# ygtxr1997/MSML

Measured on AMD Instinct MI355X. Metric: images/sec (112x112) ires50-MSML+PartialFC training step, higher is better.
Workload: dtype bf16; 1 GPU; iresnet50-MSML (OSB r18 + FM x4) + 85742-id ArcFace PartialFC, 112x112, batch 256/GPU, fwd+bwd+clip+SGD; global_batch=256, parallelism=dp1+class-parallel head, launch=eager, weight gradients + OSB on side streams

## Files before the change

include/msml_hip.h:

```cpp
#ifndef MSML_HIP_H
#define MSML_HIP_H

#include <stddef.h>
#include <stdint.h>

#ifdef __cplusplus
extern "C" {
#endif

#define MSML_ABI_VERSION 1

enum { MSML_F32 = 0, MSML_BF16 = 1, MSML_BF16X3 = 2 };

enum {
  MSML_OK = 0,
  MSML_ERR_SHAPE = -1,
  MSML_ERR_DTYPE = -2,
  MSML_ERR_LAUNCH = -3,
  MSML_ERR_UNSUPPORTED = -4,
  MSML_ERR_WORKSPACE = -5
};

enum { MSML_ACT_TANH = 0, MSML_ACT_SIGMOID = 1 };
enum { MSML_ARITH_ADD = 0, MSML_ARITH_SUB = 1, MSML_ARITH_MUL = 2, MSML_ARITH_DIV = 3 };

int msml_version(void);
const char* msml_last_error(void);
long msml_stream_capture_id(void* stream);
int msml_stream_wait_stream(void* waiter, void* src);

int msml_nchw_to_nhwc(const float* src, void* dst, int N, int C, int H, int W, int Cp,
                      int dtype, void* stream);
int msml_nhwc_to_nchw(const void* src, float* dst, int N, int C, int H, int W, int Cp,
                      int dtype, void* stream);

int msml_pack_weight(const float* w, void* dst, int A, int B, int R, int S, int transpose,
                     int C1, int C1p, int C2, int C2p, int KOp, int dtype, void* stream);

int msml_fm_fuse_fwd(const void* x, const void* yf, void* z, long n, int act, int arith,
                     int dtype, void* stream);
int msml_fm_fuse_bwd(const void* dz, const void* x, const void* yf, void* dx, void* dyf,
                     long n, int act, int arith, int dtype, void* stream);

int msml_fm_act_fwd(const void* x, void* m, long n, int act, int dtype, void* stream);
int msml_fm_act_bwd(const void* dm, const void* x, void* dx, long n, int act, int dtype, void* stream);
int msml_mul_fwd(const void* a, const void* b, void* out, long n, int dtype, void* stream);
int msml_mul_bwd(const void* g, const void* a, const void* b, void* da, void* db, long n, int dtype,
                 void* stream);
int msml_axpb(const void* x, void* y, long n, float a, float b, int dtype, void* stream);
int msml_mse_fwd(const void* a, const void* b, long n, double count, float* loss, double* workspace,
                 long ws_doubles, int dtype, void* stream);
int msml_mse_bwd(const void* a, const void* b, const float* g, double count, void* da, void* db, long n,
                 int dtype, void* stream);
int msml_dropout(const void* x, void* y, long n, float p, long seed, int dtype, void* stream);
int msml_dropout_dev(const void* x, void* y, long n, float p, const long* seed, int dtype, void* stream);

int msml_conv_tile_m(int coutp);
int msml_conv_tile_n(int coutp);
int msml_conv2d(const void* in0, int c0p, const void* in1, int c1p, const void* wp, int kop,
                const float* bias, void* out, int coutp, float* stats, int N, int H, int W,
                int P, int Q, int R, int S, int stride, int pad_h, int pad_w, int transposed,
                int in_dtype, int out_dtype, void* stream);

int msml_conv2d_acc(const void* in0, int c0p, const void* in1, int c1p, const void* wp, int kop,
                    const float* bias, void* out, int coutp, double* acc, int N, int H, int W,
                    int P, int Q, int R, int S, int stride, int pad_h, int pad_w, int transposed,
                    int in_dtype, int out_dtype, void* stream);

long msml_conv_wgrad_workspace(int up, int vp, int N, int P, int Q, int R, int S);
int msml_conv_wgrad(const void* u, int up, const void* v, int vp, float* dw, int A, int Breal,
                    int Btot, int boff, int N, int H, int W, int P, int Q, int R, int S,
                    int stride, int pad_h, int pad_w, int accumulate, void* workspace,
                    long ws_bytes, int dtype, void* stream);

int msml_conv_wgrad_group_max(int up, int vp, int A, int Breal, int N, int H, int W, int P, int Q, int R, int S,
                              int stride, int pad_h, int pad_w);
int msml_conv_wgrad_group(const void* const* u, const void* const* v, float* const* dw, int group, int up, int vp,
                          int A, int Breal, int Btot, int boff, int N, int H, int W, int P, int Q, int R, int S,
                          int stride, int pad_h, int pad_w, int accumulate, void* workspace, long ws_bytes, int dtype,
                          void* stream);

int msml_conv_wgrad_kernel_is_n32(int up, int vp, int N, int H, int W, int P, int Q, int R, int S, int stride,
                                  int pad_h, int pad_w);

int msml_bn_stats_rows(long M, int C);
int msml_bn_stats(const void* x, long M, int C, float* partial, int dtype, void* stream);
int msml_bn_finalize(const float* partial, int rows, int C, double count, const float* gamma,
                     const float* beta, float* running_mean, float* running_var, float momentum,
                     float eps, float* scale, float* shift, float* save_mean, float* save_invstd,
                     void* stream);
int msml_bn_act_fwd(const void* x, const float* scale, const float* shift, const float* alpha,
                    const void* residual, int res_first, void* y, long M, int C, int dtype,
                    void* stream);
int msml_bn_act_fwd_stats_rows(long M, int C);
int msml_bn_act_fwd_stats(const void* x, const float* scale, const float* shift, const float* alpha,
                          const void* residual, int res_first, void* y, long M, int C,
                          float* stats, int dtype, void* stream);
int msml_bn_fin_act_fwd(const double* acc, double count, const float* gamma, const float* beta,
                        float* running_mean, float* running_var, float momentum, float eps, float* scale,
                        float* shift, float* save_mean, float* save_invstd, const void* x,
                        const float* alpha, const void* residual, int res_first, void* y, long M, int C,
                        double* acc_out, int dtype, void* stream);
int msml_bn_stats_acc(const void* x, long M, int C, double* acc, int dtype, void* stream);
int msml_conv2d_bnbwd_acc(const void* in0, int c0p, const void* wp, int kop, void* out, int coutp, int N,
                          int H, int W, int P, int Q, int R, int S, int stride, int pad_h, int pad_w,
                          int transposed, const void* bn_x, const float* bn_scale, const float* bn_shift,
                          const float* bn_alpha, const float* bn_mean, const float* bn_invstd, double* acc,
                          void* stream);
int msml_bn_fin_bwd_apply(const void* dy, const void* x, const float* scale, const float* shift,
                          const float* alpha, const float* save_mean, const float* save_invstd,
                          const double* acc, const void* residual_first, const void* add, int add_h,
                          int add_w, void* dx, void* dres, float* dgamma, float* dbeta, float* dalpha,
                          int accumulate, long M, int C, const void* next_x, const float* next_mean,
                          const float* next_invstd, double* next_acc, int dtype, void* stream);
int msml_bn_act_bwd_acc(const void* dy, const void* x, const float* scale, const float* shift,
                        const float* alpha, const float* save_mean, const float* save_invstd,
                        const void* residual_first, const void* add, void* dx, void* dres, float* dgamma,
                        float* dbeta, float* dalpha, int accumulate, long M, int C, double* acc, int dtype,
                        void* stream);
int msml_bn_act_bwd(const void* dy, const void* x, const float* scale, const float* shift,
                    const float* alpha, const float* save_mean, const float* save_invstd,
                    const void* residual_first, void* dx, void* dres, float* dgamma, float* dbeta,
                    float* dalpha, int accumulate, long M, int C, float* workspace, long ws_floats,
                    int dtype, void* stream);
int msml_bias_grad(const void* dy, long M, int Cp, int Creal, float* db, int accumulate,
                   float* workspace, long ws_floats, int dtype, void* stream);
int msml_add(const void* a, const void* b, void* out, long n, int dtype, void* stream);

int msml_dap_fwd(const void* x, float* seg, unsigned char* mask, int N, int H, int W, int Cp,
                 int dtype, void* stream);
int msml_dap_bwd(const float* dseg, void* dx, int N, int H, int W, int Cp, int dtype, void* stream);
int msml_seg_consensus_loss(const float* logit, const long* msk, int N, int H, int W, float alpha,
                            float beta, float* loss, float* dlogit, float* workspace,
                            long ws_floats, void* stream);
int msml_seg_consensus_loss_r(const float* logit, const long* msk, int N, int H, int W, float alpha, float beta,
                              int reduce_pixel_all, int reduce_pixel_kl_all, float* loss, float* dlogit,
                              float* workspace, long ws_floats, void* stream);

int msml_rownorm_fwd(const float* w, int R, int Rp, int E, void* dst, int ld, float* inv_norm,
                     int dtype, void* stream);
int msml_rownorm_bwd(const float* w, const float* inv_norm, const float* dy, int ldy, int R, int E,
                     float* dw, int accumulate, void* stream);
int msml_gather_target(const float* cosm, int ld, const long* label, int N, float* out,
                       void* stream);
int msml_margin_fwd(float* cosm, const long* label, int N, int C, int ld, int kind, float s,
                    float m, float a, float k, void* stream);
int msml_margin_bwd(const float* dlogit, int ldg, const long* label, const float* cos_t, int N,
                    int C, void* dcos, int ldo, int kind, float s, float m, float a, float k,
                    int dtype, void* stream);
int msml_pfc_rowstats(const float* cosm, int ld, int N, int C, const long* label, int kind, float s,
                      float m, float a, float k, float* rowmax, float* rowsum, void* stream);
int msml_pfc_grad(const float* cosm, int ld, int N, int C, const long* label, int kind, float s,
                  float m, float a, float k, const float* gmax, const float* gsum, float eps_ls,
                  float inv_n, void* dcos, int ldo, float* ptarget, int dtype, void* stream);
int msml_sgd_momentum(float* w, const float* grad, float* mom, long n, float lr, float mu, float wd,
                      int first_step, const float* clip_coef, void* stream);
int msml_grad_norm_clip(const float* grad, long n, float max_norm, float* out2, float* workspace,
                        long ws_floats, void* stream);
int msml_sgd_momentum_dev(float* w, const float* grad, float* mom, long n, const float* lr, float mu, float wd,
                          const float* coef, void* stream);
int msml_grad_norm_clip_scaled(const float* grad, long n, float max_norm, float scale, float* out2, float* workspace,
                               long ws_floats, void* stream);

long msml_gemm_splitk_workspace(int M, int coutp, int K);
int msml_gemm_splitk(const void* a, int M, int K, const void* wp, int kop, float* out, int coutp,
                     void* workspace, long ws_bytes, int dtype, void* stream);

int msml_pack_weights_batched(const long* table, int count, int dtype, void* stream);
int msml_pack_tiles(int A, int B, int R, int S);
int msml_pack_weights_tiled(const long* table, const int* tile_prefix, int count, int total_tiles,
                            int dtype, void* stream);

int msml_transpose(const void* src, int R, int C, int ld_s, void* dst, int ld_d, int dtype,
                   void* stream);

int msml_conv2d_fused(const void* in0, int c0p, const void* in1, int c1p, const void* wp, int kop,
                      const float* scale, const float* shift, const float* alpha,
                      const void* residual, int res_first, void* out, int coutp, int N, int H,
                      int W, int P, int Q, int R, int S, int stride, int pad_h, int pad_w,
                      int transposed, void* stream);

int msml_conv2d_x3(const void* in0, int c0p, const void* in1, int c1p, const void* wp, int kop,
                   const float* scale, const float* shift, const float* alpha, const void* residual,
                   int res_first, void* out, int coutp, int N, int H, int W, int P, int Q, int R, int S,
                   int stride, int pad_h, int pad_w, int transposed, void* stream);
int msml_conv2d_x3_border(const void* in0, int c0p, const void* wp, int kop, const float* scale,
                          const float* shift9, const float* alpha, const void* residual, int res_first,
                          void* out, int coutp, int N, int H, int W, void* stream);
int msml_x3_bn_act_fwd(const void* x, const float* scale, const float* shift, const float* alpha,
                       const void* residual, int res_first, void* y, long M, int C, void* stream);
int msml_x3_fm_fuse_fwd(const void* x, const void* yf, void* z, long M, int C, int act, int arith,
                        void* stream);
int msml_x3_add(const void* a, const void* b, void* out, long M, int C, void* stream);
int msml_x3_from_f32(const float* src, void* dst, long M, int C, void* stream);
int msml_x3_to_f32(const void* src, float* dst, long M, int C, void* stream);

int msml_pair_sqdist(const float* emb, int n_pairs, int E, double* dist, void* stream);
int msml_pair_sqdist_f64(const double* emb, int n_pairs, int E, double* dist, void* stream);
int msml_pair_hist(const double* dist, const unsigned char* same, int n_pairs, const double* thr, int nthr,
                   int nfolds, int* hist, void* stream);

int msml_occ_draw(long seed, long offset, int N, int H, int W, int mode, int lo, int hi, int flip, int* desc,
                  void* stream);
int msml_occ_apply(const unsigned char* src, const int* desc, float* img, long* msk, float* ori, int N, int H,
                   int W, int light, void* stream);

int msml_occ_draw_tex(long seed, long offset, int N, int H, int W, int mode, int lo, int hi, int flip,
                      const int* meta, int nsets, int* desc, void* stream);
int msml_occ_resize(const unsigned char* atlas, const int* meta, const int* dir, const int* rtab, const int* desc,
                    unsigned char* patch, long patch_stride, int N, int lds_bytes, void* stream);
int msml_occ_apply_tex(const unsigned char* src, const int* desc, const unsigned char* patch, long patch_stride,
                       float* img, long* msk, float* ori, int N, int H, int W, int light, void* stream);

int msml_occ_draw_out(long seed, long offset, int N, int H, int W, int out_h, int out_w, int mode, int lo, int hi,
                      int flip, const int* meta, int nsets, int* desc, void* stream);
int msml_occ_apply_out(const unsigned char* src, const int* desc, const unsigned char* patch, long patch_stride,
                       const int* tabw, const int* tabh, float* img, long* msk, float* ori, int N, int H, int W,
                       int out_h, int out_w, int gray, int norm, int light, void* stream);

int msml_deconv4_bwd_data(const void* dy, const void* wp0, const void* wp1, void* dx0, void* dx1, int N, int H,
                          void* stream);

int msml_conv2d_bnbwd_rows(int coutp, int N, int P, int Q);
int msml_conv2d_bnbwd(const void* in0, int c0p, const void* wp, int kop, void* out, int coutp,
                      int N, int H, int W, int P, int Q, int R, int S, int stride, int pad_h,
                      int pad_w, int transposed, const void* bn_x, const float* bn_scale,
                      const float* bn_shift, const float* bn_alpha, const float* bn_mean,
                      const float* bn_invstd, float* partial, int rows_cap, int* rows_used,
                      void* stream);
int msml_bn_act_bwd_apply(const void* dy, const void* x, const float* scale, const float* shift,
                          const float* alpha, const float* save_mean, const float* save_invstd,
                          const float* partial, int rows, const void* add, void* dx,
                          float* dgamma, float* dbeta, float* dalpha, int accumulate, long M,
                          int C, float* coef_ws, int dtype, void* stream);

int msml_bn_act_bwd_apply_s2(const void* dy, const void* x, const float* scale, const float* shift,
                             const float* alpha, const float* save_mean, const float* save_invstd,
                             const float* partial, int rows, const void* add, int H, int W, void* dx,
                             float* dgamma, float* dbeta, float* dalpha, int accumulate, long M,
                             int C, float* coef_ws, int dtype, void* stream);
int msml_bn_act_bwd_apply_next_s2(const void* dy, const void* x, const float* scale,
                                  const float* shift, const float* alpha, const float* save_mean,
                                  const float* save_invstd, const float* partial, int rows,
                                  const void* add, int H, int W, void* dx, float* dgamma, float* dbeta,
                                  float* dalpha, int accumulate, long M, int C, float* coef_ws,
                                  const void* next_x, const float* next_mean,
                                  const float* next_invstd, float* next_partial, int dtype,
                                  void* stream);

int msml_conv2d_bnin_applies(int c0p, int coutp, int N, int H, int W, int P, int Q, int R, int S,
                             int stride, int pad_h, int pad_w, int want_stats);
int msml_conv2d_bnin(const void* in0, int c0p, const float* in_scale, const float* in_shift,
                     const float* in_alpha, const void* wp, int kop, void* out, int coutp,
                     float* stats, int N, int H, int W, int P, int Q, int R, int S, int stride,
                     int pad_h, int pad_w, void* stream);
int msml_conv_wgrad_bnin_applies(int up, int vp, int A, int Breal, int N, int H, int W, int P, int Q,
                                 int R, int S, int stride, int pad_h, int pad_w);
int msml_conv_wgrad_bnin(const void* u, int up, const void* v, int vp, const float* x_scale,
                         const float* x_shift, const float* x_alpha, float* dw, int A, int Breal,
                         int Btot, int boff, int N, int H, int W, int P, int Q, int R, int S,
                         int stride, int pad_h, int pad_w, int accumulate, void* workspace,
                         long ws_bytes, void* stream);

#define MSML_KERNEL_MFM 2
const char* msml_conv2d_kernel(int c0p, int c1p, int coutp, int N, int H, int W, int P, int Q,
                               int R, int S, int stride, int pad_h, int pad_w, int transposed,
                               int in_dtype, int out_dtype, int want_stats);

int msml_stem_im2col(const float* x, void* out, int N, int C, int H, int W, int P, int Q, int R,
                     int S, int stride, int pad, int KP, int dtype, void* stream);

int msml_bn_act_bwd_apply_rows(long M, int C);
int msml_bn_act_bwd_apply_next(const void* dy, const void* x, const float* scale, const float* shift,
                               const float* alpha, const float* save_mean, const float* save_invstd,
                               const float* partial, int rows, const void* add, void* dx,
                               float* dgamma, float* dbeta, float* dalpha, int accumulate, long M,
                               int C, float* coef_ws, const void* next_x, const float* next_mean,
                               const float* next_invstd, float* next_partial, int dtype, void* stream);

int msml_conv2d_bnin_acc_applies(int c0p, int coutp, int N, int H, int W, int P, int Q, int R, int S, int stride,
                                 int pad_h, int pad_w);
int msml_conv2d_bnin_acc(const void* in0, int c0p, const double* acc_in, double count, const float* gamma,
                         const float* beta, float* running_mean, float* running_var, float momentum, float eps,
                         float* coef_out, const float* in_alpha, void* act_out, const void* wp, int kop, void* out,
                         int coutp, double* acc_out, int N, int H, int W, int P, int Q, int R, int S, int stride,
                         int pad_h, int pad_w, void* stream);

int msml_iblock_fwd_tables(int* nptr, int* nint, int* nflt);
int msml_iblock_fwd(const void* const* ptrs, const int* ints, const float* flts, void* stream);

int msml_probe_mfma(const void* seed, float* out, int wgs, int iters, void* stream);
int msml_probe_mfma_lds(const void* seed, float* out, int wgs, int iters, void* stream);


int msml_conv2d_mfm(const void* in0, int c0p, const void* wp, int kop, const float* bias, void* out, int coutp,
                    const void* residual, unsigned char* sel, int N, int H, int W, int P, int Q, int R, int S,
                    int stride, int pad_h, int pad_w, int dtype, void* stream);

int msml_mfm_bwd(const void* dy, const unsigned char* sel, void* dz, long M, int cp, int C, int czp, int dtype,
                 void* stream);

int msml_pool2_fwd(const void* x, void* y, int N, int H, int W, int cp, int dtype, void* stream);

int msml_pool2_bwd(const void* dy, const void* x, void* dx, int N, int H, int W, int cp, int dtype, void* stream);

int msml_template_pool(const float* feats, long n_rows, long ld, int E, int flip, const float* faceness,
                       const int* order, const int* media_start, const int* tmpl_media_start, const int* launch,
                       int n_templates, double* out, void* stream);
int msml_template_pair_score(const double* tn, int n_templates, int E, const int* r1, const int* r2, long n_pairs,
                             double* score, void* stream);
int msml_roc_blocks(int n);
int msml_roc_block_counts(const double* sorted, const unsigned char* label, int n, int* blk, void* stream);
int msml_roc_points(const double* sorted, const unsigned char* label, int n, const int* off, int* tps, int* fps,
                    void* stream);
int msml_roc_reduce_blocks(int n_points);
int msml_roc_reduce(const int* tps, const int* fps, int n_points, const double* target, int n_targets,
                    unsigned char* keep, unsigned long long* part, void* stream);
int msml_pair_cosdist(const float* emb, int n_pairs, int E, double* dist, void* stream);
int msml_pair_cosdist_f64(const double* emb, int n_pairs, int E, double* dist, void* stream);
int msml_rank_count(const double* sorted, int n, const double* q, int m, int strict, int* out, void* stream);

#ifdef __cplusplus
}
#endif
#endif
```

msml_amd/blocks.py:

```python
import os

import torch

from . import ops
from . import _lib
from ._lib import BF16, call
from .ops import cpad


TAP = None
FAULT = os.environ.get("MSML_FAULT", "")


def _bn_pack(bn):
    return (bn.weight, bn.bias, bn.running_mean, bn.running_var, 0.1 if bn.momentum is None else bn.momentum,
            bn.eps, bn)


def _bn_coef(x, stats, bnp):
    assert not _is_acc(stats), "accumulator-mode statistics go through _bn_fin_apply"
    c = x.shape[-1]
    m = x.numel() // c
    coef = torch.empty(4, c, dtype=torch.float32, device=x.device)
    if stats is None:
        rows = ops.bn_stats_rows(m, c)
        stats = torch.empty(rows, 2, c, dtype=torch.float32, device=x.device)
        with ops.PROFILE.rec("bn_stats", 0.0, x.numel() * x.element_size()):
            call("msml_bn_stats", x, m, c, stats, BF16)
    k = ops.rows4(coef)
    call("msml_bn_finalize", stats, stats.shape[0], c, float(m), bnp[0], bnp[1], bnp[2], bnp[3], bnp[4], bnp[5],
         k[0], k[1], k[2], k[3])
    ops.bn_counter(bnp[6])
    return coef


def _bn_apply(x, coef, alpha, residual, emit_stats=False, res_first=0):
    c = x.shape[-1]
    m = x.numel() // c
    y = torch.empty_like(x)
    coef = ops.rows4(coef)
    with ops.PROFILE.rec("bn_act_fwd", 0.0, x.numel() * x.element_size() * (3 if residual is not None else 2)):
        if emit_stats:
            ystats = torch.empty(_lib.value("msml_bn_act_fwd_stats_rows", m, c), 2, c, dtype=torch.float32,
                                 device=x.device)
            call("msml_bn_act_fwd_stats", x, coef[0], coef[1], alpha, residual, 0, y, m, c, ystats, BF16)
            return y, ystats
        call("msml_bn_act_fwd", x, coef[0], coef[1], alpha, residual, res_first, y, m, c, BF16)
    return y


def _bn_fin_apply(x, acc, bnp, alpha, residual, emit_stats=False, res_first=0):
    c = x.shape[-1]
    m = x.numel() // c
    coef = torch.empty(4, c, dtype=torch.float32, device=x.device)
    y = torch.empty_like(x)
    yacc = ops.stats_acc(c, x.device) if emit_stats else None
    k = ops.rows4(coef)
    with ops.PROFILE.rec("bn_act_fwd", 0.0, x.numel() * x.element_size() * (3 if residual is not None else 2)):
        call("msml_bn_fin_act_fwd", acc, float(m), bnp[0], bnp[1], bnp[2], bnp[3], bnp[4], bnp[5], k[0], k[1],
             k[2], k[3], x, alpha, residual, res_first, y, m, c, yacc, BF16)
    ops.bn_counter(bnp[6])
    if emit_stats:
        return y, coef, yacc
    return y, coef


def _is_acc(stats):
    return stats is not None and stats.dtype == torch.float64


def _own_stats(x, stats):
    c = x.shape[-1]
    if stats is None and ops.acc_applies(c, BF16):
        stats = ops.stats_acc(c, x.device)
        with ops.PROFILE.rec("bn_stats", 0.0, x.numel() * x.element_size()):
            call("msml_bn_stats_acc", x, x.numel() // c, c, stats, BF16)
    return stats


def _bn_fwd(x, stats, bnp, alpha, residual, emit_stats=False):
    stats = _own_stats(x, stats)
    if _is_acc(stats):
        return _bn_fin_apply(x, stats, bnp, alpha, residual, emit_stats)
    coef = _bn_coef(x, stats, bnp)
    if emit_stats:
        y, ystats = _bn_apply(x, coef, alpha, residual, True)
        return y, coef, ystats
    return _bn_apply(x, coef, alpha, residual), coef


def _conv_pack(cm):
    w = cm.weight
    return (w, tuple(w.shape), cm.stride[0], cm.padding[0], cm.padding[1])


def _conv_fwd(x, cp):
    w, (cout, cin, r, s), stride, ph, pw = cp
    wp = ops.PACKS.get(w, False, 0, cout, 0, cin, cin, 0, BF16)
    return ops.conv2d(x, None, wp, None, cpad(cout), r, s, stride, ph, pw, False, want_stats=True,
                      real=(cin, cout))


def _bn_conv_fwd(x, stats, bnp, alpha, cp):
    if not (ops.FUSE_BN_IN and stats is None):
        stats = _own_stats(x, stats)
    if _is_acc(stats):
        w, (cout, cin, r, s), stride, ph, pw = cp
        n, h, wd, cp_in = x.shape
        if ph == pw and ops.bnin_acc_applies(n, h, wd, cp_in, cpad(cout), r, s, stride, ph):
            wp = ops.PACKS.get(w, False, 0, cout, 0, cin, cin, 0, BF16)
            o, coef, y, st = ops.conv2d_bnin_acc(x, stats, bnp, alpha, wp, cpad(cout), real=(cin, cout))
            ops.bn_counter(bnp[6])
            return o, coef, y, st
        o, coef = _bn_fin_apply(x, stats, bnp, alpha, None)
        y, st = _conv_fwd(o, cp)
        return o, coef, y, st
    coef = _bn_coef(x, stats, bnp)
    w, (cout, cin, r, s), stride, ph, pw = cp
    n, h, wd, cp_in = x.shape
    if r == 3 and s == 3 and stride == 1 and ph == 1 and pw == 1 and \
            ops.bnin_applies(n, h, wd, cp_in, cpad(cout), cout, cin):
        wp = ops.PACKS.get(w, False, 0, cout, 0, cin, cin, 0, BF16)
        y, st = ops.conv2d_bnin(x, coef, alpha, wp, cpad(cout), real=(cin, cout))
        return None, coef, y, st
    o = _bn_apply(x, coef, alpha, None)
    y, st = _conv_fwd(o, cp)
    return o, coef, y, st


def _wgrad(dy, x, cp, xin=None):
    wparam, (cout, cin, r, s), stride, ph, pw = cp
    inplace = ops.inplace(wparam)
    dw = wparam.grad.view(wparam.shape) if inplace else torch.empty_like(wparam)
    side = ops.WGRAD_STREAM if inplace else None
    if side is not None:
        _lib.stream_wait_current(side)
        dy.record_stream(side)
        x.record_stream(side)
        if xin is not None:
            xin[0].record_stream(side)
    if xin is not None:
        ops.conv_wgrad_bnin(dy, x, xin[0], xin[1], dw, cout, cin, cin, 0, accumulate=inplace, stream=side)
    elif inplace and r == 3 and s == 3 and stride == 1 and ph == 1 and pw == 1:
        ops.conv_wgrad_queued(dy, x, dw, cout, cin, cin, 0, side, wparam)
        return None
    else:
        ops.conv_wgrad(dy, x, dw, cout, cin, cin, 0, r, s, stride, ph, pw, accumulate=inplace, stream=side)
    if inplace:
        ops.grad_ready(wparam)
        return None
    return dw


def _dgrad(dy, cp, h, w, bn_x=None, coef=None, alpha=None):
    wparam, (cout, cin, r, s), stride, ph, pw = cp
    wp = ops.PACKS.get(wparam, True, 0, cout, 0, cin, cout, 0, BF16)
    if bn_x is not None and ops.FUSE_BN_BWD:
        got = ops.conv_dgrad_bnbwd(dy, wp, cpad(cin), r, s, stride, ph, pw, h, w, bn_x, coef, alpha,
                                   real=(cout, cin))
        if got is not None:
            return got
    dx, _ = ops.conv2d(dy, None, wp, None, cpad(cin), r, s, stride, ph, pw, True, p=h, q=w, real=(cout, cin))
    return dx, None


def _dgrad_plus(dy, cp, h, w, other):
    wparam, (cout, cin, r, s), stride, ph, pw = cp
    cinp = cpad(cin)
    if stride != 1 or other.shape[-1] != cinp:
        dx, _ = _dgrad(dy, cp, h, w)
        call("msml_add", dx, other, dx, dx.numel(), BF16)
        return dx
    wp = ops.PACKS.get(wparam, True, 0, cout, 0, cin, cout, 0, BF16)
    unit = ops.unit_coef(cinp, dy.device)
    n, p, q, c0p = dy.shape
    out = torch.empty(n, h, w, cinp, dtype=torch.bfloat16, device=dy.device)
    name = "conv_igemm"
    if ops.PROFILE.on:
        name = ops.conv_label("T+add", c0p, 0, cinp, n, p, q, h, w, r, s, stride, ph, pw, 1, BF16, BF16, False)
    with ops.PROFILE.rec(name, 2.0 * n * p * q * cout * cin * r * s):
        call("msml_conv2d_fused", dy, c0p, None, 0, wp, wp.shape[0], unit[0], unit[1], None, other, 0, out, cinp,
             n, p, q, h, w, r, s, stride, ph, pw, 1)
    return out


def _dgrad_1x1_compact(dy, cp):
    wparam, (cout, cin, _, _), _, _, _ = cp
    wp = ops.PACKS.get(wparam, True, 0, cout, 0, cin, cout, 0, BF16)
    dxc, _ = ops.conv2d(dy, None, wp, None, cpad(cin), 1, 1, 1, 0, 0, True, p=dy.shape[1], q=dy.shape[2],
                        real=(cout, cin))
    return dxc


class _ParamGrads:

    def __init__(self, params, c, dev):
        self.params = params
        self.want = [p is not None and p.requires_grad for p in params]
        self.inplace = all((not w) or ops.inplace(p) for w, p in zip(self.want, params))
        if self.inplace:
            self.tg = [p.grad if w else None for w, p in zip(self.want, params)]
        else:
            pg = torch.empty(3, c, dtype=torch.float32, device=dev)
            self.tg = [pg[i] if p is not None else None for i, p in enumerate(params)]

    def done(self):
        if self.inplace:
            ops.grad_ready(*[p for w, p in zip(self.want, self.params) if w])

    def out(self, i):
        return self.tg[i] if (self.want[i] and not self.inplace) else None


def _bn_bwd(dy, x, coef, alpha, pgr, partial=None, add=None, nxt=None, add_s2=False):
    c = x.shape[-1]
    m = x.numel() // c
    dx = torch.empty_like(x)
    coef = ops.rows4(coef)
    if nxt:
        nxt = (nxt[0], ops.rows4(nxt[1])) + tuple(nxt[2:])
    s2 = (add, x.shape[1], x.shape[2]) if add_s2 else (add,)
    sfx = "_s2" if add_s2 else ""
    if partial is None and ops.acc_applies(c, BF16):
        assert not add_s2, "a compact stride-2 `add` needs the producer-side sums (docstring)"
        with ops.PROFILE.rec("bn_act_bwd", 0.0, x.numel() * x.element_size() * 5):
            call("msml_bn_act_bwd_acc", dy, x, coef[0], coef[1], alpha, coef[2], coef[3], None, add, dx, None,
                 pgr.tg[0], pgr.tg[1], pgr.tg[2], int(pgr.inplace), m, c, ops.stats_acc(c, x.device, 3), BF16)
    elif partial is None:
        rows = ops.bn_stats_rows(m, c)
        ws = ops.workspace((rows * 3 * c + 2 * c) * 4, x.device)
        with ops.PROFILE.rec("bn_act_bwd", 0.0, x.numel() * x.element_size() * 5):
            call("msml_bn_act_bwd", dy, x, coef[0], coef[1], alpha, coef[2], coef[3], None, dx, None,
                 pgr.tg[0], pgr.tg[1], pgr.tg[2], int(pgr.inplace), m, c, ws, ws.numel() // 4, BF16)
        if add is not None:
            call("msml_add", dx, add, dx, dx.numel(), BF16)
    elif partial.dtype == torch.float64:
        ah, aw = (x.shape[1], x.shape[2]) if add_s2 else (0, 0)
        if nxt is not None and 256 % (c // 8) == 0:
            nacc = ops.stats_acc(c, x.device, 3)
            with ops.PROFILE.rec("bn_act_bwd_apply", 0.0, x.numel() * x.element_size() * (5 if add is not None else 4)):
                call("msml_bn_fin_bwd_apply", dy, x, coef[0], coef[1], alpha, coef[2], coef[3], partial, None, add, ah, aw,
                     dx, None, pgr.tg[0], pgr.tg[1], pgr.tg[2], int(pgr.inplace), m, c, nxt[0], nxt[1][2], nxt[1][3],
                     nacc, BF16)
            pgr.done()
            return dx, nacc
        with ops.PROFILE.rec("bn_act_bwd_apply", 0.0, x.numel() * x.element_size() * (4 if add is not None else 3)):
            call("msml_bn_fin_bwd_apply", dy, x, coef[0], coef[1], alpha, coef[2], coef[3], partial, None, add, ah, aw,
                 dx, None, pgr.tg[0], pgr.tg[1], pgr.tg[2], int(pgr.inplace), m, c, None, None, None, None, BF16)
    else:
        cw = torch.empty(98 * c, dtype=torch.float32, device=x.device)
        if nxt is not None and 256 % (c // 8) == 0:
            npart = torch.empty(_lib.value("msml_bn_act_bwd_apply_rows", m, c), 3, c, dtype=torch.float32,
                                device=x.device)
            with ops.PROFILE.rec("bn_act_bwd_apply", 0.0, x.numel() * x.element_size() * (5 if add is not None else 4)):
                call("msml_bn_act_bwd_apply_next" + sfx, dy, x, coef[0], coef[1], alpha, coef[2], coef[3], partial,
                     partial.shape[0], *s2, dx, pgr.tg[0], pgr.tg[1], pgr.tg[2], int(pgr.inplace), m, c, cw,
                     nxt[0], nxt[1][2], nxt[1][3], npart, BF16)
            pgr.done()
            return dx, npart
        with ops.PROFILE.rec("bn_act_bwd_apply", 0.0, x.numel() * x.element_size() * (4 if add is not None else 3)):
            call("msml_bn_act_bwd_apply" + sfx, dy, x, coef[0], coef[1], alpha, coef[2], coef[3], partial,
                 partial.shape[0], *s2, dx, pgr.tg[0], pgr.tg[1], pgr.tg[2], int(pgr.inplace), m, c, cw, BF16)
    pgr.done()
    if nxt is not None:
        return dx, None
    return dx


def _block_pack(blk):
    ds = blk.downsample
    return {
        "bn1": _bn_pack(blk.bn1), "bn2": _bn_pack(blk.bn2), "bn3": _bn_pack(blk.bn3),
        "c1": _conv_pack(blk.conv1), "c2": _conv_pack(blk.conv2), "alpha": blk.prelu.weight,
        "ds": None if ds is None else (_conv_pack(ds[0]), _bn_pack(ds[1])),
        "emit_stats": bool(getattr(blk, "emit_stats", False)),
    }


(_IB_X, _IB_XACC, _IB_BN1_G, _IB_BN1_B, _IB_BN1_RM, _IB_BN1_RV, _IB_COEF1, _IB_O1, _IB_WP1, _IB_C1, _IB_ACC1,
 _IB_BN2_G, _IB_BN2_B, _IB_BN2_RM, _IB_BN2_RV, _IB_COEF2, _IB_ALPHA, _IB_O2, _IB_WP2, _IB_C2, _IB_ACC2,
 _IB_WPD, _IB_D, _IB_ACCD, _IB_BND_G, _IB_BND_B, _IB_BND_RM, _IB_BND_RV, _IB_COEFD, _IB_IDN,
 _IB_BN3_G, _IB_BN3_B, _IB_BN3_RM, _IB_BN3_RV, _IB_COEF3, _IB_OUT, _IB_ACC_OUT, _IB_NPTR) = range(38)
(_II_N, _II_H, _II_W, _II_CINP, _II_COUTP, _II_KOP1, _II_KOP2, _II_KOPD, _II_STRIDE, _II_P, _II_Q, _II_HAS_DS,
 _II_DS_STRIDE, _II_NINT) = range(14)
_IF_NFLT = 8
_TABLES_OK = []


def _tables_checked():
    if not _TABLES_OK:
        import ctypes
        a, b, c = ctypes.c_int(), ctypes.c_int(), ctypes.c_int()
        call("msml_iblock_fwd_tables", ctypes.byref(a), ctypes.byref(b), ctypes.byref(c))
        if (a.value, b.value, c.value) != (_IB_NPTR, _II_NINT, _IF_NFLT):
            raise RuntimeError("msml_iblock_fwd: table layout of the library (%d, %d, %d) differs from blocks.py"
                               % (a.value, b.value, c.value))
        _TABLES_OK.append(True)
    return True


def _iblock_fwd_applies(x, bp):
    if not (ops.BLOCK_C_ENTRY and ops.ACC_STATS and not ops.PROFILE.on and not ops.FUSE_BN_IN and x.dtype == torch.bfloat16):
        return False
    cout = cpad(bp["c1"][1][0])
    return ops.acc_applies(x.shape[-1], BF16) and ops.acc_applies(cout, BF16) and x.shape[-1] == bp["c1"][1][1]


def _iblock_fwd_fast(x, bp, xstats):
    import ctypes
    _tables_checked()
    tab = bp.get("_fwd_tab")
    if tab is None:
        tab = bp["_fwd_tab"] = ((ctypes.c_void_p * _IB_NPTR)(), (ctypes.c_int * _II_NINT)(), (ctypes.c_float * _IF_NFLT)())
    pt, it, ft = tab
    dev = x.device
    n, h, w, cinp = x.shape
    bn1, bn2, bn3, ds = bp["bn1"], bp["bn2"], bp["bn3"], bp["ds"]
    w1, (cout, cin, _, _), _, _, _ = bp["c1"]
    w2, _, stride, _, _ = bp["c2"]
    coutp = cpad(cout)
    p_, q_ = ops.conv_out_size(h, 3, stride, 1, False), ops.conv_out_size(w, 3, stride, 1, False)
    if xstats is None:
        xstats = _own_stats(x, None)
    bf = torch.bfloat16
    o1 = torch.empty_like(x)
    c1 = torch.empty(n, h, w, coutp, dtype=bf, device=dev)
    o2 = torch.empty_like(c1)
    c2 = torch.empty(n, p_, q_, coutp, dtype=bf, device=dev)
    out = torch.empty_like(c2)
    k1 = torch.empty(4, cinp, dtype=torch.float32, device=dev)
    k2 = torch.empty(4, coutp, dtype=torch.float32, device=dev)
    k3 = torch.empty(4, coutp, dtype=torch.float32, device=dev)
    acc1, acc2 = ops.stats_acc(coutp, dev), ops.stats_acc(coutp, dev)
    wp1 = ops.PACKS.get(w1, False, 0, cout, 0, cin, cin, 0, BF16)
    wp2 = ops.PACKS.get(w2, False, 0, cout, 0, cout, cout, 0, BF16)
    emit = bp["emit_stats"] and 256 % (coutp // 8) == 0
    ostats = ops.stats_acc(coutp, dev) if emit else None
    pt[_IB_X], pt[_IB_XACC] = x.data_ptr(), xstats.data_ptr()
    pt[_IB_BN1_G], pt[_IB_BN1_B], pt[_IB_BN1_RM], pt[_IB_BN1_RV] = (bn1[0].data_ptr(), bn1[1].data_ptr(),
                                                                    bn1[2].data_ptr(), bn1[3].data_ptr())
    pt[_IB_COEF1], pt[_IB_O1], pt[_IB_WP1], pt[_IB_C1], pt[_IB_ACC1] = (k1.data_ptr(), o1.data_ptr(), wp1.data_ptr(),
                                                                       c1.data_ptr(), acc1.data_ptr())
    pt[_IB_BN2_G], pt[_IB_BN2_B], pt[_IB_BN2_RM], pt[_IB_BN2_RV] = (bn2[0].data_ptr(), bn2[1].data_ptr(),
                                                                    bn2[2].data_ptr(), bn2[3].data_ptr())
    pt[_IB_COEF2], pt[_IB_ALPHA], pt[_IB_O2], pt[_IB_WP2], pt[_IB_C2], pt[_IB_ACC2] = (
        k2.data_ptr(), bp["alpha"].data_ptr(), o2.data_ptr(), wp2.data_ptr(), c2.data_ptr(), acc2.data_ptr())
    d = kd = None
    it[_II_HAS_DS] = 0
    if ds is not None:
        wd, (_, _, dr, dsz), dstride, dph, dpw = ds[0]
        if dr != 1 or dsz != 1 or dph != 0 or dpw != 0:
            return None
        dbn = ds[1]
        d = torch.empty_like(c2)
        idn = torch.empty_like(c2)
        kd = torch.empty(4, coutp, dtype=torch.float32, device=dev)
        accd = ops.stats_acc(coutp, dev)
        wpd = ops.PACKS.get(wd, False, 0, cout, 0, cin, cin, 0, BF16)
        pt[_IB_WPD], pt[_IB_D], pt[_IB_ACCD] = wpd.data_ptr(), d.data_ptr(), accd.data_ptr()
        pt[_IB_BND_G], pt[_IB_BND_B], pt[_IB_BND_RM], pt[_IB_BND_RV] = (dbn[0].data_ptr(), dbn[1].data_ptr(),
                                                                        dbn[2].data_ptr(), dbn[3].data_ptr())
        pt[_IB_COEFD], pt[_IB_IDN] = kd.data_ptr(), idn.data_ptr()
        it[_II_HAS_DS], it[_II_KOPD], it[_II_DS_STRIDE] = 1, wpd.shape[0], dstride
        ft[6], ft[7] = dbn[4], dbn[5]
    pt[_IB_BN3_G], pt[_IB_BN3_B], pt[_IB_BN3_RM], pt[_IB_BN3_RV] = (bn3[0].data_ptr(), bn3[1].data_ptr(),
                                                                    bn3[2].data_ptr(), bn3[3].data_ptr())
    pt[_IB_COEF3], pt[_IB_OUT] = k3.data_ptr(), out.data_ptr()
    pt[_IB_ACC_OUT] = ostats.data_ptr() if emit else None
    (it[_II_N], it[_II_H], it[_II_W], it[_II_CINP], it[_II_COUTP], it[_II_KOP1], it[_II_KOP2], it[_II_STRIDE], it[_II_P],
     it[_II_Q]) = n, h, w, cinp, coutp, wp1.shape[0], wp2.shape[0], stride, p_, q_
    ft[0], ft[1], ft[2], ft[3], ft[4], ft[5] = bn1[4], bn1[5], bn2[4], bn2[5], bn3[4], bn3[5]
    call("msml_iblock_fwd", pt, it, ft)
    for b in ((bn1, bn2, bn3) if ds is None else (bn1, bn2, ds[1], bn3)):
        ops.bn_counter(b[6])
    return o1, c1, o2, c2, d, k1, k2, k3, kd, out, ostats


class _IBlock(torch.autograd.Function):
    @staticmethod
    def forward(ctx, x, bp, xstats, pc2, pk3, *params):
        if _iblock_fwd_applies(x, bp):
            fast = _iblock_fwd_fast(x, bp, xstats)
            if fast is not None:
                o1, c1, o2, c2, d, k1, k2, k3, kd, out, ostats = fast
                if ostats is None:
                    ostats = out.new_empty(0)
                ctx.bp = bp
                ctx.set_materialize_grads(False)
                bp["_last_bn3"] = (c2, k3) if bp["emit_stats"] else None
                ctx.save_for_backward(x, o1, c1, o2, c2, d, k1, k2, k3, kd, pc2, pk3)
                ctx.mark_non_differentiable(ostats)
                return out, ostats
        ds = bp["ds"]
        o1, k1, c1, st1 = _bn_conv_fwd(x, xstats, bp["bn1"], None, bp["c1"])
        o2, k2, c2, st2 = _bn_conv_fwd(c1, st1, bp["bn2"], bp["alpha"], bp["c2"])
        if ds is not None:
            d, std = _conv_fwd(x, ds[0])
            idn, kd = _bn_fwd(d, std, ds[1], None, None)
        else:
            d, kd, idn = None, None, x
        if bp["emit_stats"] and 256 % (c2.shape[-1] // 8) == 0:
            out, k3, ostats = _bn_fwd(c2, st2, bp["bn3"], None, idn, emit_stats=True)
        else:
            out, k3 = _bn_fwd(c2, st2, bp["bn3"], None, idn)
            ostats = out.new_empty(0)
        ctx.bp = bp
        ctx.set_materialize_grads(False)
        bp["_last_bn3"] = (c2, k3) if bp["emit_stats"] else None
        ctx.save_for_backward(x, o1, c1, o2, c2, d, k1, k2, k3, kd, pc2, pk3)
        ctx.mark_non_differentiable(ostats)
        return out, ostats

    @staticmethod
    def backward(ctx, dout, _dstats):
        x, o1, c1, o2, c2, d, k1, k2, k3, kd, pc2, pk3 = ctx.saved_tensors
        bp = ctx.bp
        ds = bp["ds"]
        dev = x.device
        dout = dout.contiguous()
        n, h, w, _ = x.shape
        bn1, bn2, bn3, alpha = bp["bn1"], bp["bn2"], bp["bn3"], bp["alpha"]
        g3 = _ParamGrads((bn3[0], bn3[1], None), c2.shape[-1], dev)
        part3 = dout.__dict__.pop("_msml_bn3_partial", None) if bp["emit_stats"] else None
        if part3 is not None:
            ops.COUNTERS["bn3_partial_hits"] += 1
        dc2 = _bn_bwd(dout, c2, k3, None, g3, part3)
        dw2 = _wgrad(dc2, o2, bp["c2"]) if o2 is not None else _wgrad(dc2, c1, bp["c2"], (k2, alpha))
        do2, part2 = _dgrad(dc2, bp["c2"], c1.shape[1], c1.shape[2], c1, k2, alpha)
        g2 = _ParamGrads((bn2[0], bn2[1], alpha), c1.shape[-1], dev)
        dc1 = _bn_bwd(do2, c1, k2, alpha, g2, part2)
        dw1 = _wgrad(dc1, o1, bp["c1"]) if o1 is not None else _wgrad(dc1, x, bp["c1"], (k1, None))
        do1, part1 = _dgrad(dc1, bp["c1"], h, w, x, k1, None)
        dwd, gd = None, None
        if ds is not None:
            gd = _ParamGrads((ds[1][0], ds[1][1], None), d.shape[-1], dev)
            dd = _bn_bwd(dout, d, kd, None, gd)
            dwd = _wgrad(dd, x, ds[0])
            (_, (_, _, dr, dsz), dstride, dph, dpw) = ds[0]
            join_s2 = (ops.SPARSE_DOWNSAMPLE_GRAD and part1 is not None and dr == 1 and dsz == 1 and dstride == 2
                       and dph == 0 and dpw == 0 and n * h * w < (1 << 24))
            if join_s2:
                join = _dgrad_1x1_compact(dd, ds[0])
            else:
                join, _ = _dgrad(dd, ds[0], h, w)
        else:
            join, join_s2 = (None if FAULT == "skip_join" else dout), False
        g1 = _ParamGrads((bn1[0], bn1[1], None), x.shape[-1], dev)
        if pc2 is not None and part1 is not None and ops.FUSE_BN_BWD:
            dx, pprev = _bn_bwd(do1, x, k1, None, g1, part1, add=join, nxt=(pc2, pk3), add_s2=join_s2)
            if pprev is not None:
                dx._msml_bn3_partial = pprev
        else:
            dx = _bn_bwd(do1, x, k1, None, g1, part1, add=join, add_s2=join_s2)
        if TAP is not None:
            TAP("iblock", bp, {"x": x, "dout": dout, "dx": dx, "k1": k1, "k2": k2, "k3": k3, "kd": kd})
        grads = [dw1, dw2] + ([dwd] if ds is not None else [])
        grads += [g1.out(0), g1.out(1), g2.out(0), g2.out(1), g2.out(2), g3.out(0), g3.out(1)]
        if ds is not None:
            grads += [gd.out(0), gd.out(1)]
        return (dx, None, None, None, None) + tuple(grads)


def iblock(blk, x):
    bp = blk.__dict__.get("_msml_pack")
    if bp is None or bp["bn1"][2] is not blk.bn1._buffers["running_mean"]:
        bp = _block_pack(blk)
        ds = blk.downsample
        params = [blk.conv1.weight, blk.conv2.weight] + ([ds[0].weight] if ds is not None else [])
        params += [blk.bn1.weight, blk.bn1.bias, blk.bn2.weight, blk.bn2.bias, blk.prelu.weight,
                   blk.bn3.weight, blk.bn3.bias]
        if ds is not None:
            params += [ds[1].weight, ds[1].bias]
        bp["params"] = tuple(params)
        blk.__dict__["_msml_pack"] = bp
    xd = x.__dict__ if hasattr(x, "__dict__") else {}
    xstats, prev = xd.get("_msml_stats"), xd.get("_msml_bn3")
    out, ostats = _IBlock.apply(x, bp, xstats, prev[0] if prev else None, prev[1] if prev else None, *bp["params"])
    last = bp.pop("_last_bn3", None)
    if ostats.numel():
        out._msml_stats = ostats
        out._msml_bn3 = last
    return out


def _bottle_pack(blk):
    return {
        "bn1": _bn_pack(blk.bn1), "bn2": _bn_pack(blk.bn2), "bn3": _bn_pack(blk.bn3),
        "c1": _conv_pack(blk.conv1), "c2": _conv_pack(blk.conv2), "c3": _conv_pack(blk.conv3),
        "a1": blk.prelu1.weight, "a2": blk.prelu2.weight, "a3": blk.prelu3.weight,
    }


class _Bottle(torch.autograd.Function):
    @staticmethod
    def forward(ctx, x, bp, *params):
        c1, st1 = _conv_fwd(x, bp["c1"])
        o1, k1 = _bn_fwd(c1, st1, bp["bn1"], bp["a1"], None)
        c2, st2 = _conv_fwd(o1, bp["c2"])
        o2, k2 = _bn_fwd(c2, st2, bp["bn2"], bp["a2"], None)
        c3, st3 = _conv_fwd(o2, bp["c3"])
        if _is_acc(st3):
            out, k3 = _bn_fin_apply(c3, st3, bp["bn3"], bp["a3"], x, res_first=1)
        else:
            k3 = _bn_coef(c3, st3, bp["bn3"])
            out = _bn_apply(c3, k3, bp["a3"], x, res_first=1)
        ctx.bp = bp
        ctx.set_materialize_grads(False)
        ctx.save_for_backward(x, c1, o1, c2, o2, c3, k1, k2, k3)
        return out

    @staticmethod
    def backward(ctx, dout):
        x, c1, o1, c2, o2, c3, k1, k2, k3 = ctx.saved_tensors
        bp = ctx.bp
        dev = x.device
        dout = dout.contiguous()
        n, h, w, _ = x.shape
        bn1, bn2, bn3 = bp["bn1"], bp["bn2"], bp["bn3"]
        g3 = _ParamGrads((bn3[0], bn3[1], bp["a3"]), c3.shape[-1], dev)
        c = c3.shape[-1]
        m = c3.numel() // c
        dc3, dres = torch.empty_like(c3), torch.empty_like(x)
        r3 = ops.rows4(k3)
        with ops.PROFILE.rec("bn_act_bwd", 0.0, c3.numel() * c3.element_size() * 7):
            if ops.acc_applies(c, BF16):
                call("msml_bn_act_bwd_acc", dout, c3, r3[0], r3[1], bp["a3"], r3[2], r3[3], x, None, dc3, dres,
                     g3.tg[0], g3.tg[1], g3.tg[2], int(g3.inplace), m, c, ops.stats_acc(c, dev, 3), BF16)
            else:
                rows = ops.bn_stats_rows(m, c)
                ws = ops.workspace((rows * 3 * c + 2 * c) * 4, dev)
                call("msml_bn_act_bwd", dout, c3, r3[0], r3[1], bp["a3"], r3[2], r3[3], x, dc3, dres,
                     g3.tg[0], g3.tg[1], g3.tg[2], int(g3.inplace), m, c, ws, ws.numel() // 4, BF16)
        g3.done()
        dw3 = _wgrad(dc3, o2, bp["c3"])
        do2, part2 = _dgrad(dc3, bp["c3"], h, w, c2, k2, bp["a2"])
        g2 = _ParamGrads((bn2[0], bn2[1], bp["a2"]), c2.shape[-1], dev)
        dc2 = _bn_bwd(do2, c2, k2, bp["a2"], g2, part2)
        dw2 = _wgrad(dc2, o1, bp["c2"])
        do1, part1 = _dgrad(dc2, bp["c2"], h, w, c1, k1, bp["a1"])
        g1 = _ParamGrads((bn1[0], bn1[1], bp["a1"]), c1.shape[-1], dev)
        dc1 = _bn_bwd(do1, c1, k1, bp["a1"], g1, part1)
        dw1 = _wgrad(dc1, x, bp["c1"])
        dx = _dgrad_plus(dc1, bp["c1"], h, w, dres)
        if TAP is not None:
            TAP("bottle", bp, {"x": x, "dout": dout, "dx": dx, "k1": k1, "k2": k2, "k3": k3})
        return (dx, None, dw1, dw2, dw3, g1.out(0), g1.out(1), g1.out(2), g2.out(0), g2.out(1), g2.out(2),
                g3.out(0), g3.out(1), g3.out(2))


def bottleneck(blk, x):
    bp = blk.__dict__.get("_msml_pack")
    if bp is None or bp["bn1"][2] is not blk.bn1._buffers["running_mean"]:
        bp = _bottle_pack(blk)
        bp["params"] = (blk.conv1.weight, blk.conv2.weight, blk.conv3.weight,
                        blk.bn1.weight, blk.bn1.bias, blk.prelu1.weight,
                        blk.bn2.weight, blk.bn2.bias, blk.prelu2.weight,
                        blk.bn3.weight, blk.bn3.bias, blk.prelu3.weight)
        blk.__dict__["_msml_pack"] = bp
    return _Bottle.apply(x, bp, *bp["params"])
```

msml_amd/csrc/bn.hip:

```cpp
#include <stdlib.h>

#include "common.h"

#define RED_ROWS_MAX 1024

template <int NQ, bool PIPE, typename L, typename F>
__device__ __forceinline__ void slab_reduce(long M, int C, float* __restrict__ partial, L ld, F f, int acc_mode = 0) {
  extern __shared__ __attribute__((aligned(16))) char smem_raw[];
  float* red = reinterpret_cast<float*>(smem_raw);
  const int C8 = C / 8;
  const int PY = 256 / C8 > 0 ? 256 / C8 : 1;
  MSML_LDS_REGION(red, PY * NQ * C * 4);
  const int t = threadIdx.x;
  const int cx = t % C8, py = t / C8;
  float q[NQ][8];
#pragma unroll
  for (int a = 0; a < NQ; a++)
#pragma unroll
    for (int j = 0; j < 8; j++) q[a][j] = 0.f;
  const long per = (M + gridDim.x - 1) / gridDim.x;
  const long beg = blockIdx.x * per;
  long end = beg + per;
  if (end > M) end = M;
  if (py < PY) {
    long pix = beg + py;
    if (PIPE)
    for (; pix + 3 * PY < end; pix += 4 * PY) {
      auto d0 = ld(pix, cx), d1 = ld(pix + PY, cx), d2 = ld(pix + 2 * PY, cx), d3 = ld(pix + 3 * PY, cx);
      f(d0, q);
      f(d1, q);
      f(d2, q);
      f(d3, q);
    }
    for (; pix < end; pix += PY) f(ld(pix, cx), q);
  }
  if (py < PY) {
#pragma unroll
    for (int a = 0; a < NQ; a++)
#pragma unroll
      for (int j = 0; j < 8; j++) red[(py * NQ + a) * C + cx * 8 + j] = q[a][j];
  }
  __syncthreads();
  for (int i = t; i < NQ * C; i += blockDim.x) {
    float s = 0.f;
    for (int y = 0; y < PY; y++) s += red[y * NQ * C + i];
    if (acc_mode)
      unsafeAtomicAdd(reinterpret_cast<double*>(partial) + (long)(blockIdx.x & (MSML_ACC_ROWS - 1)) * NQ * C + i, (double)s);
    else
      partial[(long)blockIdx.x * NQ * C + i] = s;
  }
}

static inline int red_rows(long M, int C) {
  int py = 256 / (C / 8) > 0 ? 256 / (C / 8) : 1;
  static const long ppt = getenv("MSML_RED_PPT") ? atol(getenv("MSML_RED_PPT")) : 16;
  long rows = (M + (long)py * ppt - 1) / ((long)py * ppt);
  if (rows < 1) rows = 1;
  if (rows > RED_ROWS_MAX) rows = RED_ROWS_MAX;
  return (int)rows;
}
static inline size_t red_lds(int NQ, int C) {
  int py = 256 / (C / 8) > 0 ? 256 / (C / 8) : 1;
  return (size_t)py * NQ * C * sizeof(float);
}

#define RED_PIPE_MAX_ROWS 512
template <typename T, bool PIPE>
__global__ void __launch_bounds__(256) k_bn_stats(const T* __restrict__ x, long M, int C,
                                                  float* __restrict__ partial, int acc_mode) {
  slab_reduce<2, PIPE>(M, C, partial, [&](long pix, int c8) { return load8<T>(x + pix * C + c8 * 8); },
                 [&](const Vec8& v, float(&q)[2][8]) {
#pragma unroll
    for (int j = 0; j < 8; j++) {
      q[0][j] += v.v[j];
      q[1][j] += v.v[j] * v.v[j];
    }
  }, acc_mode);
}

extern "C" int msml_bn_stats_rows(long M, int C) { return red_rows(M, C); }

extern "C" int msml_bn_stats(const void* x, long M, int C, float* partial, int dtype, void* stream) {
  MSML_CHECK(x && partial && M > 0 && C > 0 && C % 8 == 0 && C <= 2048, MSML_ERR_SHAPE,
             "bn_stats: bad shape M=%ld C=%d", M, C);
  int rows = red_rows(M, C);
  MSML_DISPATCH_DTYPE(dtype, "bn_stats",
                      if (rows <= RED_PIPE_MAX_ROWS)
                        (k_bn_stats<DT, true>)<<<rows, 256, red_lds(2, C), (hipStream_t)stream>>>((const DT*)x, M, C, partial, msml_tl_stats_acc);
                      else
                        (k_bn_stats<DT, false>)<<<rows, 256, red_lds(2, C), (hipStream_t)stream>>>((const DT*)x, M, C, partial, msml_tl_stats_acc);)
  MSML_LAUNCH_OK("bn_stats");
  return MSML_OK;
}

extern "C" int msml_bn_stats_acc(const void* x, long M, int C, double* acc, int dtype, void* stream) {
  MSML_CHECK(acc, MSML_ERR_SHAPE, "bn_stats_acc: null accumulator");
  msml_tl_stats_acc = 1;
  const int rc = msml_bn_stats(x, M, C, reinterpret_cast<float*>(acc), dtype, stream);
  msml_tl_stats_acc = 0;
  return rc;
}

#define FIN_CPB 8
#define FIN_LANES (1024 / FIN_CPB)
template <int NQ>
__device__ __forceinline__ void fin_reduce(const float* __restrict__ partial, int rows, int C, int c,
                                           bool cok, double (&out)[NQ]) {
  __shared__ double red[FIN_LANES][NQ][FIN_CPB + 1];
  __shared__ double red2[16][NQ][FIN_CPB + 1];
  const int cx = threadIdx.x & (FIN_CPB - 1), ry = threadIdx.x / FIN_CPB;
  double acc[NQ];
#pragma unroll
  for (int q = 0; q < NQ; q++) acc[q] = 0.0;
  if (cok) {
    double a1[NQ], a2[NQ], a3[NQ];
#pragma unroll
    for (int q = 0; q < NQ; q++) a1[q] = a2[q] = a3[q] = 0.0;
    int r = ry;
    for (; r + 3 * FIN_LANES < rows; r += 4 * FIN_LANES)
#pragma unroll
      for (int q = 0; q < NQ; q++) {
        acc[q] += (double)partial[((long)r * NQ + q) * C + c];
        a1[q] += (double)partial[((long)(r + FIN_LANES) * NQ + q) * C + c];
        a2[q] += (double)partial[((long)(r + 2 * FIN_LANES) * NQ + q) * C + c];
        a3[q] += (double)partial[((long)(r + 3 * FIN_LANES) * NQ + q) * C + c];
      }
    for (; r < rows; r += FIN_LANES)
#pragma unroll
      for (int q = 0; q < NQ; q++) acc[q] += (double)partial[((long)r * NQ + q) * C + c];
#pragma unroll
    for (int q = 0; q < NQ; q++) acc[q] = (acc[q] + a1[q]) + (a2[q] + a3[q]);
  }
#pragma unroll
  for (int q = 0; q < NQ; q++) red[ry][q][cx] = acc[q];
  __syncthreads();
  if (ry < 16) {
#pragma unroll
    for (int q = 0; q < NQ; q++) {
      double s = 0.0;
#pragma unroll
      for (int y = 0; y < FIN_LANES / 16; y++) s += red[ry * (FIN_LANES / 16) + y][q][cx];
      red2[ry][q][cx] = s;
    }
  }
  __syncthreads();
#pragma unroll
  for (int q = 0; q < NQ; q++) {
    double s = 0.0;
    if (ry == 0)
#pragma unroll
      for (int y = 0; y < 16; y++) s += red2[y][q][cx];
    out[q] = s;
  }
}

__global__ void __launch_bounds__(1024) k_bn_finalize(const float* __restrict__ partial, int rows, int C, double count,
                              const float* __restrict__ gamma, const float* __restrict__ beta,
                              float* __restrict__ rmean, float* __restrict__ rvar, float momentum,
                              float eps, float* __restrict__ scale, float* __restrict__ shift,
                              float* __restrict__ save_mean, float* __restrict__ save_invstd) {
  const int c = blockIdx.x * FIN_CPB + (threadIdx.x & (FIN_CPB - 1));
  const bool cok = c < C;
  float mean = 0.f, invstd = 1.f;
  if (rows > 0) {
    double s[2];
    fin_reduce<2>(partial, rows, C, c, cok, s);
    if (threadIdx.x >= FIN_CPB || !cok) return;
    double m = s[0] / count;
    double var = s[1] / count - m * m;
    if (var < 0.0) var = 0.0;
    mean = (float)m;
    invstd = (float)(1.0 / sqrt(var + (double)eps));
    if (rmean) {
      double unbiased = count > 1.0 ? var * count / (count - 1.0) : var;
      rmean[c] = (1.f - momentum) * rmean[c] + momentum * mean;
      rvar[c] = (1.f - momentum) * rvar[c] + momentum * (float)unbiased;
    }
  } else {
    if (threadIdx.x >= FIN_CPB || !cok) return;
    mean = rmean[c];
    invstd = 1.0f / sqrtf(rvar[c] + eps);
  }
  float g = gamma ? gamma[c] : 1.f, b = beta ? beta[c] : 0.f;
  scale[c] = g * invstd;
  shift[c] = b - mean * g * invstd;
  if (save_mean) {
    save_mean[c] = mean;
    save_invstd[c] = invstd;
  }
}

extern "C" int msml_bn_finalize(const float* partial, int rows, int C, double count,
                                const float* gamma, const float* beta, float* running_mean,
                                float* running_var, float momentum, float eps, float* scale,
                                float* shift, float* save_mean, float* save_invstd, void* stream) {
  MSML_CHECK(C > 0 && scale && shift && rows >= 0, MSML_ERR_SHAPE, "bn_finalize: bad args");
  MSML_CHECK(rows > 0 ? (partial && count > 0) : (running_mean && running_var), MSML_ERR_SHAPE,
             "bn_finalize: train needs partials, eval needs running stats");
  k_bn_finalize<<<cdiv(C, FIN_CPB), 1024, 0, (hipStream_t)stream>>>(
      partial, rows, C, count, gamma, beta, running_mean, running_var, momentum, eps, scale, shift,
      save_mean, save_invstd);
  MSML_LAUNCH_OK("bn_finalize");
  return MSML_OK;
}

struct Coef8 {
  float v[8];
};
__device__ __forceinline__ Coef8 ldc8(const float* p, int c0, float dflt) {
  Coef8 r;
  if (p) {
    f32x4 a = *reinterpret_cast<const f32x4*>(p + c0);
    f32x4 b = *reinterpret_cast<const f32x4*>(p + c0 + 4);
#pragma unroll
    for (int i = 0; i < 4; i++) { r.v[i] = a[i]; r.v[4 + i] = b[i]; }
  } else {
#pragma unroll
    for (int i = 0; i < 8; i++) r.v[i] = dflt;
  }
  return r;
}

template <typename T, bool STATS>
__global__ void __launch_bounds__(256) k_bn_act_fwd(const T* __restrict__ x, const float* __restrict__ scale,
                                                    const float* __restrict__ shift,
                                                    const float* __restrict__ alpha,
                                                    const T* __restrict__ residual, int res_first,
                                                    T* __restrict__ y, long n8, int C8, float* __restrict__ stats) {
  const long tid = blockIdx.x * (long)blockDim.x + threadIdx.x;
  const int c0 = (int)(tid % C8) * 8;
  const Coef8 sc = ldc8(scale, c0, 1.f), sh = ldc8(shift, c0, 0.f), al = ldc8(alpha, c0, 1.f);
  float q1[8], q2[8];
#pragma unroll
  for (int j = 0; j < 8; j++) q1[j] = q2[j] = 0.f;
  for (long i = tid; i < n8; i += (long)gridDim.x * blockDim.x) {
    Vec8 v = load8<T>(x + i * 8);
    Vec8 r;
    if (residual) r = load8<T>(residual + i * 8);
#pragma unroll
    for (int j = 0; j < 8; j++) {
      float z = v.v[j] * sc.v[j] + sh.v[j];
      if (residual && res_first) z += r.v[j];
      if (alpha) z = z > 0.f ? z : z * al.v[j];
      if (residual && !res_first) z += r.v[j];
      v.v[j] = z;
    }
    store8<T>(y + i * 8, v);
    if (STATS) {
      const Vec8 vr = round8<T>(v);
#pragma unroll
      for (int j = 0; j < 8; j++) {
        q1[j] += vr.v[j];
        q2[j] += vr.v[j] * vr.v[j];
      }
    }
  }
  if (STATS) {
    __shared__ float red[2][256][9];
    const int t = threadIdx.x, C = C8 * 8;
#pragma unroll
    for (int j = 0; j < 8; j++) {
      red[0][t][j] = q1[j];
      red[1][t][j] = q2[j];
    }
    __syncthreads();
    for (int i = t; i < 2 * C; i += 256) {
      const int which = i / C, c = i % C, cx = c >> 3, j = c & 7;
      float sum = 0.f;
      for (int k = cx; k < 256; k += C8) sum += red[which][k][j];
      stats[((long)blockIdx.x * 2 + which) * C + c] = sum;
    }
  }
}

static inline int ew_grid(long n8) {
  static const long cap = getenv("MSML_EW_GRID") ? atol(getenv("MSML_EW_GRID")) : 768;
  long b = (n8 + 255) / 256;
  return (int)(b < cap ? b : cap);
}
static inline int ew_grid_c(long n8, int C8) {
  int g = ew_grid(n8);
  if (C8 > 256) {
    int m = C8 / 256;
    g = (g + m - 1) / m * m;
  }
  return g;
}

extern "C" int msml_bn_act_fwd(const void* x, const float* scale, const float* shift,
                               const float* alpha, const void* residual, int res_first, void* y,
                               long M, int C, int dtype, void* stream) {
  MSML_CHECK(x && y && scale && shift && M > 0 && C > 0 && C % 8 == 0, MSML_ERR_SHAPE,
             "bn_act_fwd: bad shape M=%ld C=%d", M, C);
  MSML_CHECK(256 % (C / 8) == 0 || (C / 8) % 256 == 0, MSML_ERR_UNSUPPORTED,
             "bn_act_fwd: C/8 = %d must divide 256 or be a multiple of it", C / 8);
  long n8 = M * (C / 8);
  MSML_DISPATCH_DTYPE(dtype, "bn_act_fwd",
                      (k_bn_act_fwd<DT, false>)<<<ew_grid_c(n8, C / 8), 256, 0, (hipStream_t)stream>>>(
                          (const DT*)x, scale, shift, alpha, (const DT*)residual, res_first, (DT*)y, n8,
                          C / 8, nullptr);)
  MSML_LAUNCH_OK("bn_act_fwd");
  return MSML_OK;
}

extern "C" int msml_bn_act_fwd_stats_rows(long M, int C) { return ew_grid_c(M * (C / 8), C / 8); }

extern "C" int msml_bn_act_fwd_stats(const void* x, const float* scale, const float* shift, const float* alpha,
                                     const void* residual, int res_first, void* y, long M, int C,
                                     float* stats, int dtype, void* stream) {
  MSML_CHECK(x && y && scale && shift && stats && M > 0 && C > 0 && C % 8 == 0, MSML_ERR_SHAPE,
             "bn_act_fwd_stats: bad shape M=%ld C=%d", M, C);
  MSML_CHECK(256 % (C / 8) == 0, MSML_ERR_UNSUPPORTED, "bn_act_fwd_stats: C/8 = %d must divide 256", C / 8);
  long n8 = M * (C / 8);
  MSML_DISPATCH_DTYPE(dtype, "bn_act_fwd_stats",
                      (k_bn_act_fwd<DT, true>)<<<ew_grid_c(n8, C / 8), 256, 0, (hipStream_t)stream>>>(
                          (const DT*)x, scale, shift, alpha, (const DT*)residual, res_first, (DT*)y, n8,
                          C / 8, stats);)
  MSML_LAUNCH_OK("bn_act_fwd_stats");
  return MSML_OK;
}

template <typename T, bool STATS>
__global__ void __launch_bounds__(256) k_bn_fin_act_fwd(const double* __restrict__ acc, double count,
                                                        const float* __restrict__ gamma, const float* __restrict__ beta,
                                                        float* __restrict__ rmean, float* __restrict__ rvar, float momentum,
                                                        float eps, float* __restrict__ scale, float* __restrict__ shift,
                                                        float* __restrict__ save_mean, float* __restrict__ save_invstd,
                                                        const T* __restrict__ x, const float* __restrict__ alpha,
                                                        const T* __restrict__ residual, int res_first,
                                                        T* __restrict__ y, long n8, int C8, double* __restrict__ acc_out) {
  extern __shared__ float cs[];
  const int C = C8 * 8, t = threadIdx.x;
  MSML_LDS_REGION(cs, 2 * C * 4);
  for (int c = t; c < C; c += 256) {
    double s = 0.0, ss = 0.0;
#pragma unroll
    for (int r = 0; r < MSML_ACC_ROWS; r++) {
      s += acc[(r * 2 + 0) * C + c];
      ss += acc[(r * 2 + 1) * C + c];
    }
    const double m = s / count;
    double var = ss / count - m * m;
    if (var < 0.0) var = 0.0;
    const float mean = (float)m;
    const float invstd = (float)(1.0 / sqrt(var + (double)eps));
    const float g = gamma ? gamma[c] : 1.f, b = beta ? beta[c] : 0.f;
    const float sc = g * invstd, sh = b - mean * g * invstd;
    cs[c] = sc;
    cs[C + c] = sh;
    if (blockIdx.x == 0) {
      scale[c] = sc;
      shift[c] = sh;
      save_mean[c] = mean;
      save_invstd[c] = invstd;
      if (rmean) {
        const double unbiased = count > 1.0 ? var * count / (count - 1.0) : var;
        rmean[c] = (1.f - momentum) * rmean[c] + momentum * mean;
        rvar[c] = (1.f - momentum) * rvar[c] + momentum * (float)unbiased;
      }
    }
  }
  __syncthreads();
  const long tid = blockIdx.x * (long)blockDim.x + t;
  const int c0 = (int)(tid % C8) * 8;
  Coef8 sc, sh;
#pragma unroll
  for (int j = 0; j < 8; j++) {
    sc.v[j] = cs[c0 + j];
    sh.v[j] = cs[C + c0 + j];
  }
  const Coef8 al = ldc8(alpha, c0, 1.f);
  float q1[8], q2[8];
#pragma unroll
  for (int j = 0; j < 8; j++) q1[j] = q2[j] = 0.f;
  for (long i = tid; i < n8; i += (long)gridDim.x * blockDim.x) {
    Vec8 v = load8<T>(x + i * 8);
    Vec8 r;
    if (residual) r = load8<T>(residual + i * 8);
#pragma unroll
    for (int j = 0; j < 8; j++) {
      float z = v.v[j] * sc.v[j] + sh.v[j];
      if (residual && res_first) z += r.v[j];
      if (alpha) z = z > 0.f ? z : z * al.v[j];
      if (residual && !res_first) z += r.v[j];
      v.v[j] = z;
    }
    store8<T>(y + i * 8, v);
    if (STATS) {
      const Vec8 vr = round8<T>(v);
#pragma unroll
      for (int j = 0; j < 8; j++) {
        q1[j] += vr.v[j];
        q2[j] += vr.v[j] * vr.v[j];
      }
    }
  }
  if (STATS) {
    __shared__ float red[2][256][9];
#pragma unroll
    for (int j = 0; j < 8; j++) {
      red[0][t][j] = q1[j];
      red[1][t][j] = q2[j];
    }
    __syncthreads();
    for (int i = t; i < 2 * C; i += 256) {
      const int which = i / C, c = i % C, cx = c >> 3, j = c & 7;
      float sum = 0.f;
      for (int k = cx; k < 256; k += C8) sum += red[which][k][j];
      stats_emit(reinterpret_cast<float*>(acc_out), 1, blockIdx.x, which, C, c, sum);
    }
  }
}

extern "C" int msml_bn_fin_act_fwd(const double* acc, double count, const float* gamma, const float* beta,
                                   float* running_mean, float* running_var, float momentum, float eps, float* scale,
                                   float* shift, float* save_mean, float* save_invstd, const void* x,
                                   const float* alpha, const void* residual, int res_first, void* y, long M, int C,
                                   double* acc_out, int dtype, void* stream) {
  MSML_CHECK(acc && x && y && scale && shift && save_mean && save_invstd && M > 0 && C > 0 && C % 8 == 0 && count > 0,
             MSML_ERR_SHAPE, "bn_fin_act_fwd: bad arguments M=%ld C=%d", M, C);
  MSML_CHECK(256 % (C / 8) == 0, MSML_ERR_UNSUPPORTED, "bn_fin_act_fwd: C/8 = %d must divide 256", C / 8);
  const long n8 = M * (C / 8);
  const size_t lds = (size_t)2 * C * sizeof(float);
  hipStream_t st = (hipStream_t)stream;
  if (acc_out) {
    MSML_DISPATCH_DTYPE(dtype, "bn_fin_act_fwd",
                        (k_bn_fin_act_fwd<DT, true>)<<<ew_grid_c(n8, C / 8), 256, lds, st>>>(
                            acc, count, gamma, beta, running_mean, running_var, momentum, eps, scale, shift, save_mean,
                            save_invstd, (const DT*)x, alpha, (const DT*)residual, res_first, (DT*)y, n8, C / 8, acc_out);)
  } else {
    MSML_DISPATCH_DTYPE(dtype, "bn_fin_act_fwd",
                        (k_bn_fin_act_fwd<DT, false>)<<<ew_grid_c(n8, C / 8), 256, lds, st>>>(
                            acc, count, gamma, beta, running_mean, running_var, momentum, eps, scale, shift, save_mean,
                            save_invstd, (const DT*)x, alpha, (const DT*)residual, res_first, (DT*)y, n8, C / 8, nullptr);)
  }
  MSML_LAUNCH_OK("bn_fin_act_fwd");
  return MSML_OK;
}

template <typename T, bool PIPE>
__global__ void __launch_bounds__(256) k_bn_bwd_reduce(const T* __restrict__ dy, const T* __restrict__ x,
                                                       const float* __restrict__ scale,
                                                       const float* __restrict__ shift,
                                                       const float* __restrict__ alpha,
                                                       const float* __restrict__ mean,
                                                       const float* __restrict__ invstd,
                                                       const T* __restrict__ res, long M, int C,
                                                       float* __restrict__ partial, int acc_mode) {
  const int c0h = (threadIdx.x % (C / 8)) * 8;
  const Coef8 sc = ldc8(scale, c0h, 1.f), sh = ldc8(shift, c0h, 0.f), al = ldc8(alpha, c0h, 1.f);
  const Coef8 mu = ldc8(mean, c0h, 0.f), is = ldc8(invstd, c0h, 1.f);
  struct Px {
    Vec8 g, v, rr;
  };
  slab_reduce<3, PIPE>(M, C, partial, [&](long pix, int c8) {
    Px d;
    d.g = load8<T>(dy + pix * C + c8 * 8);
    d.v = load8<T>(x + pix * C + c8 * 8);
    if (res) d.rr = load8<T>(res + pix * C + c8 * 8);
    return d;
  }, [&](const Px& d, float(&q)[3][8]) {
    const Vec8 &g = d.g, &v = d.v, &rr = d.rr;
#pragma unroll
    for (int j = 0; j < 8; j++) {
      float gg = g.v[j];
      if (alpha) {
        float z = v.v[j] * sc.v[j] + sh.v[j];
        if (res) z += rr.v[j];
        if (z <= 0.f) {
          q[2][j] += gg * z;
          gg *= al.v[j];
        }
      }
      float xh = (v.v[j] - mu.v[j]) * is.v[j];
      q[0][j] += gg;
      q[1][j] += gg * xh;
    }
  }, acc_mode);
}

#define FOLD_ROWS 32
#define FOLD_MIN_ROWS 512
template <int NQ>
__global__ void __launch_bounds__(1024) k_fold_rows(const float* __restrict__ partial, int rows, int C,
                                                    float* __restrict__ out) {
  const int c = blockIdx.x * FIN_CPB + (threadIdx.x & (FIN_CPB - 1));
  const bool cok = c < C;
  const int chunk = (rows + FOLD_ROWS - 1) / FOLD_ROWS;
  const int r0 = blockIdx.y * chunk;
  int nr = rows - r0;
  if (nr > chunk) nr = chunk;
  if (nr < 0) nr = 0;
  double s[NQ];
  fin_reduce<NQ>(partial + (long)r0 * NQ * C, nr, C, c, cok, s);
  if (threadIdx.x >= FIN_CPB || !cok) return;
#pragma unroll
  for (int q = 0; q < NQ; q++) out[((long)blockIdx.y * NQ + q) * C + c] = (float)s[q];
}

__global__ void __launch_bounds__(1024) k_bn_bwd_finalize(const float* __restrict__ partial, int rows, int C, double count,
                                  float* __restrict__ dgamma, float* __restrict__ dbeta,
                                  float* __restrict__ dalpha, float* __restrict__ coef, int accumulate) {
  const int c = blockIdx.x * FIN_CPB + (threadIdx.x & (FIN_CPB - 1));
  const bool cok = c < C;
  double s[3];
  fin_reduce<3>(partial, rows, C, c, cok, s);
  if (threadIdx.x >= FIN_CPB || !cok) return;
  if (dbeta) dbeta[c] = (accumulate ? dbeta[c] : 0.f) + (float)s[0];
  if (dgamma) dgamma[c] = (accumulate ? dgamma[c] : 0.f) + (float)s[1];
  if (dalpha) dalpha[c] = (accumulate ? dalpha[c] : 0.f) + (float)s[2];
  coef[c] = (float)(s[0] / count);
  coef[C + c] = (float)(s[1] / count);
}

template <typename T, bool NEXT, bool ADD_S2 = false>
__global__ void __launch_bounds__(256) k_bn_bwd_apply(const T* __restrict__ dy, const T* __restrict__ x,
                                                      const float* __restrict__ scale,
                                                      const float* __restrict__ shift,
                                                      const float* __restrict__ alpha,
                                                      const float* __restrict__ mean,
                                                      const float* __restrict__ invstd,
                                                      const float* __restrict__ coef,
                                                      const T* __restrict__ res, const T* __restrict__ add,
                                                      T* __restrict__ dx, T* __restrict__ dres, long n8,
                                                      int C8, const T* __restrict__ nx,
                                                      const float* __restrict__ nmean,
                                                      const float* __restrict__ ninvstd,
                                                      float* __restrict__ npartial, int aH, int aW) {
  const int C = C8 * 8;
  const long tid = blockIdx.x * (long)blockDim.x + threadIdx.x;
  const int c0 = (int)(tid % C8) * 8;
  const Coef8 sc = ldc8(scale, c0, 1.f), sh = ldc8(shift, c0, 0.f), al = ldc8(alpha, c0, 1.f);
  const Coef8 mu = ldc8(mean, c0, 0.f), is = ldc8(invstd, c0, 1.f);
  const Coef8 k1 = ldc8(coef, c0, 0.f), k2 = ldc8(coef + C, c0, 0.f);
  const float rcpW = ADD_S2 ? 1.0f / (float)aW : 0.f, rcpH = ADD_S2 ? 1.0f / (float)aH : 0.f;
  const int aPw = (aW + 1) >> 1, aPh = (aH + 1) >> 1;
  const Coef8 nmu = ldc8(NEXT ? nmean : nullptr, c0, 0.f), nis = ldc8(NEXT ? ninvstd : nullptr, c0, 1.f);
  float nq0[8], nq1[8];
#pragma unroll
  for (int j = 0; j < 8; j++) nq0[j] = nq1[j] = 0.f;
  for (long i = tid; i < n8; i += (long)gridDim.x * blockDim.x) {
    Vec8 g = load8<T>(dy + i * 8);
    Vec8 v = load8<T>(x + i * 8);
    Vec8 rr, ad;
    if (res) rr = load8<T>(res + i * 8);
    bool has_add = add != nullptr;
    if (ADD_S2) {
      const int pix = (int)(i / C8);
      int row = (int)((float)pix * rcpW), xx = pix - row * aW;
      if (xx < 0) { row--; xx += aW; } else if (xx >= aW) { row++; xx -= aW; }
      int nn = (int)((float)row * rcpH), yy = row - nn * aH;
      if (yy < 0) { nn--; yy += aH; } else if (yy >= aH) { nn++; yy -= aH; }
      has_add = !((xx | yy) & 1);
      if (has_add) ad = load8<T>(add + (((long)nn * aPh + (yy >> 1)) * aPw + (xx >> 1)) * C + c0);
    } else if (add) {
      ad = load8<T>(add + i * 8);
    }
#pragma unroll
    for (int j = 0; j < 8; j++) {
      float gg = g.v[j];
      if (alpha) {
        float z = v.v[j] * sc.v[j] + sh.v[j];
        if (res) z += rr.v[j];
        if (z <= 0.f) gg *= al.v[j];
      }
      float xh = (v.v[j] - mu.v[j]) * is.v[j];
      v.v[j] = sc.v[j] * (gg - k1.v[j] - xh * k2.v[j]);
      if (has_add) v.v[j] += ad.v[j];
      g.v[j] = gg;
    }
    store8<T>(dx + i * 8, v);
    if (dres) store8<T>(dres + i * 8, g);
    if (NEXT) {
      const Vec8 o = round8<T>(v), xn = load8<T>(nx + i * 8);
#pragma unroll
      for (int j = 0; j < 8; j++) {
        nq0[j] += o.v[j];
        nq1[j] += o.v[j] * ((xn.v[j] - nmu.v[j]) * nis.v[j]);
      }
    }
  }
  if (NEXT) {
    __shared__ float red[2][256][9];
    const int t = threadIdx.x;
#pragma unroll
    for (int j = 0; j < 8; j++) {
      red[0][t][j] = nq0[j];
      red[1][t][j] = nq1[j];
    }
    __syncthreads();
    for (int i = t; i < 3 * C; i += 256) {
      const int q = i / C, c = i % C, cx = c >> 3, j = c & 7;
      float sum = 0.f;
      if (q < 2)
        for (int k = cx; k < 256; k += C8) sum += red[q][k][j];
      npartial[((long)blockIdx.x * 3 + q) * C + c] = sum;
    }
  }
}

extern "C" int msml_bn_act_bwd(const void* dy, const void* x, const float* scale, const float* shift,
                               const float* alpha, const float* save_mean, const float* save_invstd,
                               const void* residual_first, void* dx, void* dres, float* dgamma,
                               float* dbeta, float* dalpha, int accumulate, long M, int C,
                               float* workspace, long ws_floats, int dtype, void* stream) {
  MSML_CHECK(dy && x && dx && scale && shift && save_mean && save_invstd && workspace && M > 0 &&
                 C > 0 && C % 8 == 0 && C <= 2048,
             MSML_ERR_SHAPE, "bn_act_bwd: bad args M=%ld C=%d", M, C);
  MSML_CHECK(256 % (C / 8) == 0, MSML_ERR_UNSUPPORTED, "bn_act_bwd: C/8 = %d must divide 256", C / 8);
  int rows = red_rows(M, C);
  long need = (long)rows * 3 * C + 2 * C;
  MSML_CHECK(ws_floats >= need, MSML_ERR_WORKSPACE, "bn_act_bwd: workspace %ld < %ld floats", ws_floats, need);
  float* partial = workspace;
  float* coef = workspace + (long)rows * 3 * C;
  hipStream_t st = (hipStream_t)stream;
  long n8 = M * (C / 8);
  MSML_DISPATCH_DTYPE(
      dtype, "bn_act_bwd",
      if (rows <= RED_PIPE_MAX_ROWS)
        (k_bn_bwd_reduce<DT, true>)<<<rows, 256, red_lds(3, C), st>>>((const DT*)dy, (const DT*)x, scale, shift, alpha,
                                                                      save_mean, save_invstd,
                                                                      (const DT*)residual_first, M, C, partial, 0);
      else
        (k_bn_bwd_reduce<DT, false>)<<<rows, 256, red_lds(3, C), st>>>((const DT*)dy, (const DT*)x, scale, shift, alpha,
                                                                       save_mean, save_invstd,
                                                                       (const DT*)residual_first, M, C, partial, 0);
      MSML_LAUNCH_OK("bn_bwd_reduce");
      k_bn_bwd_finalize<<<cdiv(C, FIN_CPB), 1024, 0, st>>>(partial, rows, C, (double)M, dgamma, dbeta, dalpha, coef, accumulate);
      MSML_LAUNCH_OK("bn_bwd_finalize");
      (k_bn_bwd_apply<DT, false>)<<<ew_grid_c(n8, C / 8), 256, 0, st>>>(
          (const DT*)dy, (const DT*)x, scale, shift, alpha, save_mean, save_invstd, coef,
          (const DT*)residual_first, (const DT*)nullptr, (DT*)dx, (DT*)dres, n8, C / 8, (const DT*)nullptr,
          nullptr, nullptr, nullptr, 0, 0);)
  MSML_LAUNCH_OK("bn_bwd_apply");
  return MSML_OK;
}

template <typename T, bool NEXT, bool ADD_S2>
__global__ void __launch_bounds__(256) k_bn_fin_bwd_apply(const T* __restrict__ dy, const T* __restrict__ x,
                                                          const float* __restrict__ scale, const float* __restrict__ shift,
                                                          const float* __restrict__ alpha, const float* __restrict__ mean,
                                                          const float* __restrict__ invstd, const double* __restrict__ acc,
                                                          double count, float* __restrict__ dgamma,
                                                          float* __restrict__ dbeta, float* __restrict__ dalpha,
                                                          int accumulate, const T* __restrict__ res,
                                                          const T* __restrict__ add, T* __restrict__ dx,
                                                          T* __restrict__ dres, long n8, int C8,
                                                          const T* __restrict__ nx, const float* __restrict__ nmean,
                                                          const float* __restrict__ ninvstd, double* __restrict__ nacc,
                                                          int aH, int aW) {
  extern __shared__ float ck[];
  const int C = C8 * 8, t = threadIdx.x;
  MSML_LDS_REGION(ck, 2 * C * 4);
  for (int c = t; c < C; c += 256) {
    double s0 = 0.0, s1 = 0.0, s2 = 0.0;
#pragma unroll
    for (int r = 0; r < MSML_ACC_ROWS; r++) {
      s0 += acc[(r * 3 + 0) * C + c];
      s1 += acc[(r * 3 + 1) * C + c];
      s2 += acc[(r * 3 + 2) * C + c];
    }
    ck[c] = (float)(s0 / count);
    ck[C + c] = (float)(s1 / count);
    if (blockIdx.x == 0) {
      if (dbeta) dbeta[c] = (accumulate ? dbeta[c] : 0.f) + (float)s0;
      if (dgamma) dgamma[c] = (accumulate ? dgamma[c] : 0.f) + (float)s1;
      if (dalpha) dalpha[c] = (accumulate ? dalpha[c] : 0.f) + (float)s2;
    }
  }
  __syncthreads();
  const long tid = blockIdx.x * (long)blockDim.x + t;
  const int c0 = (int)(tid % C8) * 8;
  const Coef8 sc = ldc8(scale, c0, 1.f), sh = ldc8(shift, c0, 0.f), al = ldc8(alpha, c0, 1.f);
  const Coef8 mu = ldc8(mean, c0, 0.f), is = ldc8(invstd, c0, 1.f);
  Coef8 k1, k2;
#pragma unroll
  for (int j = 0; j < 8; j++) {
    k1.v[j] = ck[c0 + j];
    k2.v[j] = ck[C + c0 + j];
  }
  const float rcpW = ADD_S2 ? 1.0f / (float)aW : 0.f, rcpH = ADD_S2 ? 1.0f / (float)aH : 0.f;
  const int aPw = (aW + 1) >> 1, aPh = (aH + 1) >> 1;
  const Coef8 nmu = ldc8(NEXT ? nmean : nullptr, c0, 0.f), nis = ldc8(NEXT ? ninvstd : nullptr, c0, 1.f);
  float nq0[8], nq1[8];
#pragma unroll
  for (int j = 0; j < 8; j++) nq0[j] = nq1[j] = 0.f;
  for (long i = tid; i < n8; i += (long)gridDim.x * blockDim.x) {
    Vec8 g = load8<T>(dy + i * 8);
    Vec8 v = load8<T>(x + i * 8);
    Vec8 rr, ad;
    if (res) rr = load8<T>(res + i * 8);
    bool has_add = add != nullptr;
    if (ADD_S2) {
      const int pix = (int)(i / C8);
      int row = (int)((float)pix * rcpW), xx = pix - row * aW;
      if (xx < 0) { row--; xx += aW; } else if (xx >= aW) { row++; xx -= aW; }
      int nn = (int)((float)row * rcpH), yy = row - nn * aH;
      if (yy < 0) { nn--; yy += aH; } else if (yy >= aH) { nn++; yy -= aH; }
      has_add = !((xx | yy) & 1);
      if (has_add) ad = load8<T>(add + (((long)nn * aPh + (yy >> 1)) * aPw + (xx >> 1)) * C + c0);
    } else if (add) {
      ad = load8<T>(add + i * 8);
    }
#pragma unroll
    for (int j = 0; j < 8; j++) {
      float gg = g.v[j];
      if (alpha) {
        float z = v.v[j] * sc.v[j] + sh.v[j];
        if (res) z += rr.v[j];
        if (z <= 0.f) gg *= al.v[j];
      }
      float xh = (v.v[j] - mu.v[j]) * is.v[j];
      v.v[j] = sc.v[j] * (gg - k1.v[j] - xh * k2.v[j]);
      if (has_add) v.v[j] += ad.v[j];
      g.v[j] = gg;
    }
    store8<T>(dx + i * 8, v);
    if (dres) store8<T>(dres + i * 8, g);
    if (NEXT) {
      const Vec8 o = round8<T>(v), xn = load8<T>(nx + i * 8);
#pragma unroll
      for (int j = 0; j < 8; j++) {
        const float gn = o.v[j];
        nq0[j] += gn;
        nq1[j] += gn * ((xn.v[j] - nmu.v[j]) * nis.v[j]);
      }
    }
  }
  if (NEXT) {
    __shared__ float red[2][256][9];
#pragma unroll
    for (int j = 0; j < 8; j++) {
      red[0][t][j] = nq0[j];
      red[1][t][j] = nq1[j];
    }
    __syncthreads();
    for (int i = t; i < 2 * C; i += 256) {
      const int q = i / C, c = i % C, cx = c >> 3, j = c & 7;
      float sum = 0.f;
      for (int k = cx; k < 256; k += C8) sum += red[q][k][j];
      bnb_emit(reinterpret_cast<float*>(nacc), 1, blockIdx.x, q, C, c, sum);
    }
  }
}

extern "C" int msml_bn_fin_bwd_apply(const void* dy, const void* x, const float* scale, const float* shift,
                                     const float* alpha, const float* save_mean, const float* save_invstd,
                                     const double* acc, const void* residual_first, const void* add, int add_h,
                                     int add_w, void* dx, void* dres, float* dgamma, float* dbeta, float* dalpha,
                                     int accumulate, long M, int C, const void* next_x, const float* next_mean,
                                     const float* next_invstd, double* next_acc, int dtype, void* stream) {
  MSML_CHECK(dy && x && dx && scale && shift && save_mean && save_invstd && acc && M > 0 && C > 0 && C % 8 == 0,
             MSML_ERR_SHAPE, "bn_fin_bwd_apply: bad args M=%ld C=%d", M, C);
  MSML_CHECK(256 % (C / 8) == 0, MSML_ERR_UNSUPPORTED, "bn_fin_bwd_apply: C/8 = %d must divide 256", C / 8);
  const bool s2 = add_h > 0;
  MSML_CHECK(!s2 || (add && add_w > 0 && M % ((long)add_h * add_w) == 0 && M < (1L << 24)), MSML_ERR_SHAPE,
             "bn_fin_bwd_apply: stride-2 add needs M = N*H*W < 2^24 (M=%ld H=%d W=%d)", M, add_h, add_w);
  MSML_CHECK(!next_acc || (next_x && next_mean && next_invstd), MSML_ERR_SHAPE, "bn_fin_bwd_apply: next_* incomplete");
  hipStream_t st = (hipStream_t)stream;
  const long n8 = M * (C / 8);
  const size_t lds = (size_t)2 * C * sizeof(float);
#define BN_FIN_LAUNCH(NEXT_, S2_)                                                                                   \
  (k_bn_fin_bwd_apply<DT, NEXT_, S2_>)<<<ew_grid_c(n8, C / 8), 256, lds, st>>>(                                     \
      (const DT*)dy, (const DT*)x, scale, shift, alpha, save_mean, save_invstd, acc, (double)M, dgamma, dbeta, dalpha, \
      accumulate, (const DT*)residual_first, (const DT*)add, (DT*)dx, (DT*)dres, n8, C / 8, (const DT*)next_x,      \
      next_mean, next_invstd, next_acc, add_h, add_w);
  MSML_DISPATCH_DTYPE(dtype, "bn_fin_bwd_apply",
                      if (next_acc) { if (s2) { BN_FIN_LAUNCH(true, true) } else { BN_FIN_LAUNCH(true, false) } }
                      else { if (s2) { BN_FIN_LAUNCH(false, true) } else { BN_FIN_LAUNCH(false, false) } })
#undef BN_FIN_LAUNCH
  MSML_LAUNCH_OK("bn_fin_bwd_apply");
  return MSML_OK;
}

extern "C" int msml_bn_act_bwd_acc(const void* dy, const void* x, const float* scale, const float* shift,
                                   const float* alpha, const float* save_mean, const float* save_invstd,
                                   const void* residual_first, const void* add, void* dx, void* dres, float* dgamma,
                                   float* dbeta, float* dalpha, int accumulate, long M, int C, double* acc, int dtype,
                                   void* stream) {
  MSML_CHECK(dy && x && dx && scale && shift && save_mean && save_invstd && acc && M > 0 && C > 0 && C % 8 == 0 &&
                 C <= 2048, MSML_ERR_SHAPE, "bn_act_bwd_acc: bad args M=%ld C=%d", M, C);
  MSML_CHECK(256 % (C / 8) == 0, MSML_ERR_UNSUPPORTED, "bn_act_bwd_acc: C/8 = %d must divide 256", C / 8);
  const int rows = red_rows(M, C);
  hipStream_t st = (hipStream_t)stream;
  MSML_DISPATCH_DTYPE(
      dtype, "bn_act_bwd_acc",
      if (rows <= RED_PIPE_MAX_ROWS)
        (k_bn_bwd_reduce<DT, true>)<<<rows, 256, red_lds(3, C), st>>>((const DT*)dy, (const DT*)x, scale, shift, alpha,
                                                                      save_mean, save_invstd, (const DT*)residual_first,
                                                                      M, C, reinterpret_cast<float*>(acc), 1);
      else
        (k_bn_bwd_reduce<DT, false>)<<<rows, 256, red_lds(3, C), st>>>((const DT*)dy, (const DT*)x, scale, shift, alpha,
                                                                       save_mean, save_invstd, (const DT*)residual_first,
                                                                       M, C, reinterpret_cast<float*>(acc), 1);)
  MSML_LAUNCH_OK("bn_bwd_reduce(acc)");
  return msml_bn_fin_bwd_apply(dy, x, scale, shift, alpha, save_mean, save_invstd, acc, residual_first, add, 0, 0,
                               dx, dres, dgamma, dbeta, dalpha, accumulate, M, C, nullptr, nullptr, nullptr, nullptr,
                               dtype, stream);
}

static int bn_bwd_apply_impl(const void* dy, const void* x, const float* scale, const float* shift,
                             const float* alpha, const float* save_mean, const float* save_invstd,
                             const float* partial, int rows, const void* add, void* dx, float* dgamma,
                             float* dbeta, float* dalpha, int accumulate, long M, int C, float* coef_ws,
                             const void* next_x, const float* next_mean, const float* next_invstd,
                             float* next_partial, int dtype, void* stream, int add_h = 0, int add_w = 0) {
  MSML_CHECK(dy && x && dx && scale && shift && save_mean && save_invstd && partial && coef_ws && rows > 0 &&
                 M > 0 && C > 0 && C % 8 == 0 && C <= 2048,
             MSML_ERR_SHAPE, "bn_act_bwd_apply: bad args M=%ld C=%d rows=%d", M, C, rows);
  MSML_CHECK(256 % (C / 8) == 0, MSML_ERR_UNSUPPORTED, "bn_act_bwd_apply: C/8 = %d must divide 256", C / 8);
  const bool s2 = add_h > 0;
  MSML_CHECK(!s2 || (add && add_w > 0 && M % ((long)add_h * add_w) == 0 && M < (1L << 24)), MSML_ERR_SHAPE,
             "bn_act_bwd_apply: stride-2 add needs M = N*H*W < 2^24 (M=%ld H=%d W=%d)", M, add_h, add_w);
  hipStream_t st = (hipStream_t)stream;
  long n8 = M * (C / 8);
  if (rows > FOLD_MIN_ROWS) {
    float* folded = coef_ws + 2 * C;
    k_fold_rows<3><<<dim3(cdiv(C, FIN_CPB), FOLD_ROWS), 1024, 0, st>>>(partial, rows, C, folded);
    MSML_LAUNCH_OK("bn_bwd_fold");
    partial = folded;
    rows = FOLD_ROWS;
  }
  k_bn_bwd_finalize<<<cdiv(C, FIN_CPB), 1024, 0, st>>>(partial, rows, C, (double)M, dgamma, dbeta, dalpha, coef_ws, accumulate);
  MSML_LAUNCH_OK("bn_bwd_finalize");
#define BN_APPLY_LAUNCH(NEXT_, S2_, NX, NM, NI, NP)                                                          \
  (k_bn_bwd_apply<DT, NEXT_, S2_>)<<<ew_grid_c(n8, C / 8), 256, 0, st>>>(                                    \
      (const DT*)dy, (const DT*)x, scale, shift, alpha, save_mean, save_invstd, coef_ws, (const DT*)nullptr, \
      (const DT*)add, (DT*)dx, (DT*)nullptr, n8, C / 8, (const DT*)(NX), NM, NI, NP, add_h, add_w);
  if (next_partial) {
    MSML_CHECK(next_x && next_mean && next_invstd && 256 % (C / 8) == 0, MSML_ERR_SHAPE,
               "bn_act_bwd_apply_next: bad args C=%d", C);
    MSML_DISPATCH_DTYPE(dtype, "bn_act_bwd_apply_next",
                        if (s2) { BN_APPLY_LAUNCH(true, true, next_x, next_mean, next_invstd, next_partial) }
                        else { BN_APPLY_LAUNCH(true, false, next_x, next_mean, next_invstd, next_partial) })
  } else {
    MSML_DISPATCH_DTYPE(dtype, "bn_act_bwd_apply",
                        if (s2) { BN_APPLY_LAUNCH(false, true, nullptr, nullptr, nullptr, nullptr) }
                        else { BN_APPLY_LAUNCH(false, false, nullptr, nullptr, nullptr, nullptr) })
  }
#undef BN_APPLY_LAUNCH
  MSML_LAUNCH_OK("bn_bwd_apply");
  return MSML_OK;
}

extern "C" int msml_bn_act_bwd_apply(const void* dy, const void* x, const float* scale, const float* shift,
                                     const float* alpha, const float* save_mean, const float* save_invstd,
                                     const float* partial, int rows, const void* add, void* dx,
                                     float* dgamma, float* dbeta, float* dalpha, int accumulate, long M,
                                     int C, float* coef_ws, int dtype, void* stream) {
  return bn_bwd_apply_impl(dy, x, scale, shift, alpha, save_mean, save_invstd, partial, rows, add, dx, dgamma,
                           dbeta, dalpha, accumulate, M, C, coef_ws, nullptr, nullptr, nullptr, nullptr, dtype,
                           stream);
}

extern "C" int msml_bn_act_bwd_apply_rows(long M, int C) { return ew_grid_c(M * (C / 8), C / 8); }

extern "C" int msml_bn_act_bwd_apply_next(const void* dy, const void* x, const float* scale, const float* shift,
                                          const float* alpha, const float* save_mean, const float* save_invstd,
                                          const float* partial, int rows, const void* add, void* dx,
                                          float* dgamma, float* dbeta, float* dalpha, int accumulate, long M,
                                          int C, float* coef_ws, const void* next_x, const float* next_mean,
                                          const float* next_invstd, float* next_partial, int dtype,
                                          void* stream) {
  MSML_CHECK(next_partial, MSML_ERR_SHAPE, "bn_act_bwd_apply_next: next_partial is null");
  return bn_bwd_apply_impl(dy, x, scale, shift, alpha, save_mean, save_invstd, partial, rows, add, dx, dgamma,
                           dbeta, dalpha, accumulate, M, C, coef_ws, next_x, next_mean, next_invstd,
                           next_partial, dtype, stream);
}

extern "C" int msml_bn_act_bwd_apply_s2(const void* dy, const void* x, const float* scale, const float* shift,
                                        const float* alpha, const float* save_mean, const float* save_invstd,
                                        const float* partial, int rows, const void* add, int H, int W, void* dx,
                                        float* dgamma, float* dbeta, float* dalpha, int accumulate, long M,
                                        int C, float* coef_ws, int dtype, void* stream) {
  MSML_CHECK(add && H > 0 && W > 0, MSML_ERR_SHAPE, "bn_act_bwd_apply_s2: bad add H=%d W=%d", H, W);
  return bn_bwd_apply_impl(dy, x, scale, shift, alpha, save_mean, save_invstd, partial, rows, add, dx, dgamma,
                           dbeta, dalpha, accumulate, M, C, coef_ws, nullptr, nullptr, nullptr, nullptr, dtype,
                           stream, H, W);
}

extern "C" int msml_bn_act_bwd_apply_next_s2(const void* dy, const void* x, const float* scale,
                                             const float* shift, const float* alpha, const float* save_mean,
                                             const float* save_invstd, const float* partial, int rows,
                                             const void* add, int H, int W, void* dx, float* dgamma, float* dbeta,
                                             float* dalpha, int accumulate, long M, int C, float* coef_ws,
                                             const void* next_x, const float* next_mean,
                                             const float* next_invstd, float* next_partial, int dtype,
                                             void* stream) {
  MSML_CHECK(add && H > 0 && W > 0 && next_partial, MSML_ERR_SHAPE, "bn_act_bwd_apply_next_s2: bad args");
  return bn_bwd_apply_impl(dy, x, scale, shift, alpha, save_mean, save_invstd, partial, rows, add, dx, dgamma,
                           dbeta, dalpha, accumulate, M, C, coef_ws, next_x, next_mean, next_invstd,
                           next_partial, dtype, stream, H, W);
}

__global__ void __launch_bounds__(1024) k_colsum_finalize(const float* __restrict__ partial, int rows, int C,
                                                          int stride_q, float* __restrict__ out, int Creal,
                                                          int accumulate) {
  constexpr int CS_LANES = 32;
  __shared__ double red[CS_LANES][33];
  const int cx = threadIdx.x & 31, ry = threadIdx.x >> 5;
  const int c = blockIdx.x * 32 + cx;
  double acc = 0.0;
  if (c < Creal)
    for (int r = ry; r < rows; r += CS_LANES) acc += (double)partial[(long)r * stride_q * C + c];
  red[ry][cx] = acc;
  __syncthreads();
  if (ry == 0 && c < Creal) {
    double s = 0.0;
    for (int y = 0; y < CS_LANES; y++) s += red[y][cx];
    out[c] = (accumulate ? out[c] : 0.f) + (float)s;
  }
}

extern "C" int msml_bias_grad(const void* dy, long M, int Cp, int Creal, float* db, int accumulate,
                              float* workspace, long ws_floats, int dtype, void* stream) {
  MSML_CHECK(dy && db && workspace && M > 0 && Cp > 0 && Cp % 8 == 0 && Cp <= 2048 && Creal <= Cp, MSML_ERR_SHAPE,
             "bias_grad: bad args");
  int rows = red_rows(M, Cp);
  MSML_CHECK(ws_floats >= (long)rows * 2 * Cp, MSML_ERR_WORKSPACE, "bias_grad: workspace too small");
  hipStream_t st = (hipStream_t)stream;
  MSML_DISPATCH_DTYPE(dtype, "bias_grad",
                      if (rows <= RED_PIPE_MAX_ROWS)
                        (k_bn_stats<DT, true>)<<<rows, 256, red_lds(2, Cp), st>>>((const DT*)dy, M, Cp, workspace, 0);
                      else
                        (k_bn_stats<DT, false>)<<<rows, 256, red_lds(2, Cp), st>>>((const DT*)dy, M, Cp, workspace, 0);)
  MSML_LAUNCH_OK("bias_grad");
  k_colsum_finalize<<<cdiv(Creal, 32), 1024, 0, st>>>(workspace, rows, Cp, 2, db, Creal, accumulate);
  MSML_LAUNCH_OK("bias_grad_finalize");
  return MSML_OK;
}

template <typename T>
__global__ void __launch_bounds__(256) k_add(const T* __restrict__ a, const T* __restrict__ b,
                                             T* __restrict__ o, long n8) {
  for (long i = blockIdx.x * (long)blockDim.x + threadIdx.x; i < n8;
       i += (long)gridDim.x * blockDim.x) {
    Vec8 x = load8<T>(a + i * 8), y = load8<T>(b + i * 8);
#pragma unroll
    for (int j = 0; j < 8; j++) x.v[j] += y.v[j];
    store8<T>(o + i * 8, x);
  }
}

extern "C" int msml_add(const void* a, const void* b, void* out, long n, int dtype, void* stream) {
  MSML_CHECK(a && b && out && n > 0 && n % 8 == 0, MSML_ERR_SHAPE, "add: n=%ld", n);
  MSML_DISPATCH_DTYPE(dtype, "add",
                      k_add<DT><<<ew_grid(n / 8), 256, 0, (hipStream_t)stream>>>(
                          (const DT*)a, (const DT*)b, (DT*)out, n / 8);)
  MSML_LAUNCH_OK("add");
  return MSML_OK;
}
```

msml_amd/functional.py:

```python
import os
import torch

from . import _lib, ops
from ._lib import BF16, DTYPE_OF, F32, TORCH_DTYPE, call
from .ops import cpad


class _ToNHWC(torch.autograd.Function):

    @staticmethod
    def forward(ctx, x, dtype):
        return ops.to_nhwc(x.float(), dtype)

    @staticmethod
    def backward(ctx, g):
        return None, None


def to_nhwc(x, dtype):
    return _ToNHWC.apply(x, dtype)


def _slice_w(w, deconv, off, n):
    if deconv:
        return w[off:off + n]
    return w[:, off:off + n].contiguous()


class _Conv(torch.autograd.Function):

    @staticmethod
    def forward(ctx, x0, x1, weight, bias, cfg, wp):
        deconv = cfg["deconv"]
        c0, c1 = cfg["c0"], cfg["c1"]
        cout = cfg["cout"]
        r, s = weight.shape[2], weight.shape[3]
        dtype = DTYPE_OF[x0.dtype]
        if wp is None:
            wp = ops.PACKS.get(weight, deconv, 0, weight.shape[0], 0, weight.shape[1], c0, c1, dtype)
        bp = None
        if bias is not None:
            bp = ops.padded_bias(bias, cpad(cout))
        y, stats = ops.conv2d(x0, x1, wp, bp, cpad(cout), r, s, cfg["stride"], cfg["pad_h"],
                              cfg["pad_w"], deconv, out_dtype=cfg.get("out_dtype"),
                              want_stats=cfg.get("want_stats", False), real=(c0 + c1, cout))
        ctx.cfg = cfg
        ctx.set_materialize_grads(False)
        ctx.has_bias = bias is not None
        ctx.wparam = cfg.get("grad_param", weight)
        ctx.wobj = weight
        ctx.bparam = bias
        ctx.save_for_backward(x0, x1, weight)
        if stats is None:
            stats = x0.new_empty(0)
        ctx.mark_non_differentiable(stats)
        return y, stats

    @staticmethod
    def backward(ctx, dy, _dstats):
        return _Conv._bwd(ctx, dy, ctx.needs_input_grad)

    @staticmethod
    def _bwd(ctx, dy, need):
        x0, x1, weight = ctx.saved_tensors
        cfg = ctx.cfg
        if dy is None:
            return None, None, None, None, None, None
        deconv, c0, c1, cout = cfg["deconv"], cfg["c0"], cfg["c1"], cfg["cout"]
        stride, ph, pw = cfg["stride"], cfg["pad_h"], cfg["pad_w"]
        r, s = weight.shape[2], weight.shape[3]
        dy = dy.contiguous()
        if DTYPE_OF[dy.dtype] != DTYPE_OF[x0.dtype]:
            dy = dy.to(x0.dtype)
        dtype = DTYPE_OF[x0.dtype]
        w = weight.detach()
        n, h, wd, _ = x0.shape
        grads = [None, None]
        if (deconv and x1 is not None and need[0] and need[1] and dtype == BF16
                and r == 4 and s == 4 and stride == 2 and ph == 1 and pw == 1 and x0.shape[3] == 32 and x1.shape[3] == 32
                and dy.shape[3] == 32 and h == wd and h in (14, 28, 56)):
            wp0 = ops.PACKS.get(w, False, 0, c0, 0, cout, cout, 0, dtype, owner=ctx.wobj)
            wp1 = ops.PACKS.get(w, False, c0, c1, 0, cout, cout, 0, dtype, owner=ctx.wobj)
            g0, g1 = torch.empty_like(x0), torch.empty_like(x1)
            name = "conv_igemm"
            if ops.PROFILE.on:
                name = "conv N c32+0->32+32 %dx%d k4x4 s2 n%d [k_deconv4_bwd<both segments>]" % (2 * h, 2 * h, n)
            with ops.PROFILE.rec(name, 2.0 * n * h * wd * (c0 + c1) * cout * 16):
                rc = _lib.try_call("msml_deconv4_bwd_data", dy, wp0, wp1, g0, g1, n, h)
            if rc == 0:
                grads = [g0, g1]
        for i, (x, off, ci) in enumerate(((x0, 0, c0), (x1, c0, c1))):
            if grads[i] is not None:
                continue
            if x is None or not need[i]:
                continue
            if deconv:
                wp = ops.PACKS.get(w, False, off, ci, 0, cout, cout, 0, dtype, owner=ctx.wobj)
                grads[i], _ = ops.conv2d(dy, None, wp, None, cpad(ci), r, s, stride, ph, pw, False,
                                         p=h, q=wd, real=(cout, ci))
            else:
                wp = ops.PACKS.get(w, True, 0, cout, off, ci, cout, 0, dtype, owner=ctx.wobj)
                grads[i], _ = ops.conv2d(dy, None, wp, None, cpad(ci), r, s, stride, ph, pw, True,
                                         p=h, q=wd, real=(cout, ci))
        dw = None
        if need[2]:
            inplace = ops.inplace(ctx.wparam)
            dw = ctx.wparam.grad.view(w.shape) if inplace else torch.empty_like(w)
            side = ops.WGRAD_STREAM if inplace else None
            if side is not None:
                _lib.stream_wait_current(side)
                dy.record_stream(side)
                for xs in (x0, x1):
                    if xs is not None:
                        xs.record_stream(side)
            for x, off, ci in ((x0, 0, c0), (x1, c0, c1)):
                if x is None:
                    continue
                if deconv:
                    ops.conv_wgrad(x, dy, dw[off:off + ci], ci, cout, cout, 0, r, s, stride, ph, pw,
                                   accumulate=inplace, stream=side)
                else:
                    ops.conv_wgrad(dy, x, dw, cout, ci, c0 + c1, off, r, s, stride, ph, pw,
                                   accumulate=inplace, stream=side)
            if inplace:
                dw = None
                ops.grad_ready(ctx.wparam)
        db = None
        if ctx.has_bias and need[3]:
            m = dy.numel() // dy.shape[-1]
            cp = dy.shape[-1]
            rows = ops.bn_stats_rows(m, cp)
            wsb = ops.workspace(rows * 2 * cp * 4, dy.device)
            binplace = ops.inplace(ctx.bparam)
            db = ctx.bparam.grad if binplace else torch.empty(cout, dtype=torch.float32, device=dy.device)
            call("msml_bias_grad", dy, m, cp, cout, db, int(binplace), wsb, wsb.numel() // 4, dtype)
            if binplace:
                db = None
                ops.grad_ready(ctx.bparam)
        return grads[0], grads[1], dw, db, None, None


def conv(x0, x1, weight, bias, cfg, wp=None):
    y, stats = _Conv.apply(x0, x1, weight, bias, cfg, wp)
    return y, (stats if stats.numel() else None)


FAULT = ""


class _ConvTee(torch.autograd.Function):

    @staticmethod
    def forward(ctx, x0, x1, weight, bias, cfg, wp):
        y, stats = _Conv.forward(ctx, x0, x1, weight, bias, cfg, wp)
        ctx.mark_non_differentiable(stats)
        return y, stats, x0.view_as(x0)

    @staticmethod
    def backward(ctx, dy, _dstats, dtee):
        cfg = ctx.cfg
        x0, x1, weight = ctx.saved_tensors
        if FAULT == "skip_tee":
            dtee = None
        fused = None
        if (dy is not None and dtee is not None and ctx.needs_input_grad[0] and not cfg["deconv"] and cfg["stride"] == 1
                and dy.dtype == torch.bfloat16 and dtee.dtype == torch.bfloat16 and dtee.shape == x0.shape):
            c0, cout = cfg["c0"], cfg["cout"]
            r, s = weight.shape[2], weight.shape[3]
            dyc = dy.contiguous()
            wp = ops.PACKS.get(weight.detach(), True, 0, cout, 0, c0, cout, 0, BF16, owner=ctx.wobj)
            n, h, wd, c0p = x0.shape
            unit = _unit_coef(c0p, dy.device)
            fused = torch.empty_like(x0)
            name = "conv_igemm"
            if ops.PROFILE.on:
                name = ops.conv_label("T+add", dyc.shape[3], 0, c0p, n, dyc.shape[1], dyc.shape[2], h, wd, r, s, 1,
                                      cfg["pad_h"], cfg["pad_w"], 1, BF16, BF16, False)
            with ops.PROFILE.rec(name, 2.0 * n * h * wd * cout * c0 * r * s):
                call("msml_conv2d_fused", dyc, dyc.shape[3], None, 0, wp, wp.shape[0], unit[0], unit[1], None,
                     dtee.contiguous(), 0, fused, c0p, n, dyc.shape[1], dyc.shape[2], h, wd, r, s, 1, cfg["pad_h"],
                     cfg["pad_w"], 1)
        if fused is not None:
            g = _Conv._bwd(ctx, dy, (False,) + tuple(ctx.needs_input_grad[1:]))
            return (fused,) + tuple(g[1:])
        g = _Conv._bwd(ctx, dy, ctx.needs_input_grad)
        if dtee is not None and g[0] is not None:
            g0 = torch.empty_like(g[0])
            call("msml_add", g[0], dtee.contiguous(), g0, g0.numel(), DTYPE_OF[g0.dtype])
            return (g0,) + tuple(g[1:])
        return ((dtee if g[0] is None else g[0]),) + tuple(g[1:])


def _unit_coef(cp, device):
    return ops.unit_coef(cp, device)


def conv_tee(x0, x1, weight, bias, cfg, wp=None):
    y, stats, x0b = _ConvTee.apply(x0, x1, weight, bias, cfg, wp)
    return y, (stats if stats.numel() else None), x0b


class _BnAct(torch.autograd.Function):

    @staticmethod
    def forward(ctx, x, stats, gamma, beta, alpha, residual, rmean, rvar, training, momentum, eps,
                res_first, emit=False):
        c = x.shape[-1]
        m = x.numel() // c
        dtype = DTYPE_OF[x.dtype]
        dev = x.device
        coef = torch.empty(4, c, dtype=torch.float32, device=dev)
        if training and stats is None and ops.acc_applies(c, dtype):
            stats = ops.stats_acc(c, dev)
            with ops.PROFILE.rec("bn_stats", 0.0, x.numel() * x.element_size()):
                call("msml_bn_stats_acc", x, m, c, stats, dtype)
        if training and stats is not None and stats.dtype == torch.float64:
            y = torch.empty_like(x)
            yacc = ops.stats_acc(c, dev) if emit else None
            with ops.PROFILE.rec("bn_act_fwd", 0.0, x.numel() * x.element_size() * (3 if residual is not None else 2)):
                call("msml_bn_fin_act_fwd", stats, float(m), gamma, beta, rmean, rvar, momentum, eps, coef[0], coef[1],
                     coef[2], coef[3], x, alpha, residual, int(res_first), y, m, c, yacc, dtype)
            ctx.training = training
            ctx.has = (gamma is not None, beta is not None, alpha is not None, residual is not None)
            ctx.res_first = bool(res_first) and residual is not None and alpha is not None
            ctx.params = (gamma, beta, alpha)
            ctx.save_for_backward(x, coef, alpha, residual if ctx.res_first else None)
            if emit:
                ctx.mark_non_differentiable(yacc)
                return y, yacc
            return y
        if training:
            if stats is None:
                rows = ops.bn_stats_rows(m, c)
                stats = torch.empty(rows, 2, c, dtype=torch.float32, device=dev)
                with ops.PROFILE.rec("bn_stats", 0.0, x.numel() * x.element_size()):
                    call("msml_bn_stats", x, m, c, stats, dtype)
            call("msml_bn_finalize", stats, stats.shape[0], c, float(m), gamma, beta, rmean, rvar,
                 momentum, eps, coef[0], coef[1], coef[2], coef[3])
        else:
            call("msml_bn_finalize", None, 0, c, 0.0, gamma, beta, rmean, rvar, momentum, eps,
                 coef[0], coef[1], coef[2], coef[3])
        y = torch.empty_like(x)
        with ops.PROFILE.rec("bn_act_fwd", 0.0, x.numel() * x.element_size() * (3 if residual is not None else 2)):
            call("msml_bn_act_fwd", x, coef[0], coef[1], alpha, residual, int(res_first), y, m, c, dtype)
        ctx.training = training
        ctx.has = (gamma is not None, beta is not None, alpha is not None, residual is not None)
        ctx.res_first = bool(res_first) and residual is not None and alpha is not None
        ctx.params = (gamma, beta, alpha)
        ctx.save_for_backward(x, coef, alpha, residual if ctx.res_first else None)
        return y

    @staticmethod
    def backward(ctx, dy, *_dacc):
        x, coef, alpha, res = ctx.saved_tensors
        if not ctx.training:
            raise RuntimeError("msml_amd: backward through eval-mode BatchNorm is not supported")
        c = x.shape[-1]
        m = x.numel() // c
        dtype = DTYPE_OF[x.dtype]
        dy = dy.contiguous()
        dx = torch.empty_like(x)
        pg = torch.empty(3, c, dtype=torch.float32, device=x.device)
        rows = ops.bn_stats_rows(m, c)
        need = (rows * 3 * c + 2 * c) * 4
        ws = ops.workspace(need, x.device)
        dres = torch.empty_like(x) if ctx.res_first else None
        has_g, has_b, has_a, has_r = ctx.has
        gamma, beta, alpha_p = ctx.params
        want = (has_g and ctx.needs_input_grad[2], has_b and ctx.needs_input_grad[3],
                has_a and ctx.needs_input_grad[4])
        inplace = all((not w) or ops.inplace(prm) for w, prm in zip(want, (gamma, beta, alpha_p)))
        if inplace:
            tg = [prm.grad if w else None for w, prm in zip(want, (gamma, beta, alpha_p))]
        else:
            tg = [pg[0], pg[1], pg[2] if alpha is not None else None]
        with ops.PROFILE.rec("bn_act_bwd", 0.0, x.numel() * x.element_size() * (5 + (3 if ctx.res_first else 0))):
            if ops.acc_applies(c, dtype):
                call("msml_bn_act_bwd_acc", dy, x, coef[0], coef[1], alpha, coef[2], coef[3], res, None, dx, dres,
                     tg[0], tg[1], tg[2], int(inplace), m, c, ops.stats_acc(c, x.device, 3), dtype)
            else:
                call("msml_bn_act_bwd", dy, x, coef[0], coef[1], alpha, coef[2], coef[3], res, dx, dres,
                     tg[0], tg[1], tg[2], int(inplace), m, c, ws, ws.numel() // 4, dtype)
        if ctx.res_first:
            dy = dres
        if inplace:
            ops.grad_ready(*[prm for w, prm in zip(want, (gamma, beta, alpha_p)) if w])
        return (dx, None,
                pg[0] if want[0] and not inplace else None,
                pg[1] if want[1] and not inplace else None,
                pg[2] if want[2] and not inplace else None,
                dy if has_r else None, None, None, None, None, None, None, None)


def bn_act(x, stats, bn, prelu=None, residual=None, res_first=False, emit_stats=False):
    if isinstance(x, SplitT):
        return bn_act_x3(x, bn, prelu, residual, res_first)
    training = bn.training
    if training:
        ops.bn_counter(bn)
    c = x.shape[-1]
    if bn.num_features != c:
        return _bn_act_padded(x, stats, bn, prelu, residual, res_first, training)
    emit = bool(emit_stats and training and ops.EMIT_STEM_STATS and x.dtype == torch.bfloat16 and ops.acc_applies(c, BF16)
                and (stats is None or stats.dtype == torch.float64) and 256 % (c // 8) == 0)
    out = _BnAct.apply(x, stats, bn.weight, bn.bias, prelu.weight if prelu is not None else None,
                       residual, bn.running_mean, bn.running_var, training,
                       0.1 if bn.momentum is None else bn.momentum, bn.eps, res_first, emit)
    if emit:
        y, yacc = out
        y._msml_stats = yacc
        return y
    return out


def _bn_act_padded(x, stats, bn, prelu, residual, res_first, training):
    import torch.nn.functional as F
    c, cr = x.shape[-1], bn.num_features
    assert cr < c and bn.weight is not None
    pad = (0, c - cr)
    rm = F.pad(bn.running_mean, pad)
    rv = F.pad(bn.running_var, pad, value=1.0)
    out = _BnAct.apply(x, stats, F.pad(bn.weight, pad), F.pad(bn.bias, pad),
                       F.pad(prelu.weight, pad) if prelu is not None else None, residual, rm, rv, training,
                       0.1 if bn.momentum is None else bn.momentum, bn.eps, res_first, False)
    if training:
        with torch.no_grad():
            bn.running_mean.copy_(rm[:cr])
            bn.running_var.copy_(rv[:cr])
    return out


class _FmFuse(torch.autograd.Function):
    @staticmethod
    def forward(ctx, x, yf, act, arith):
        z = torch.empty_like(yf)
        with ops.PROFILE.rec("fm_fuse_fwd", 0.0, 3 * x.numel() * x.element_size()):
            call("msml_fm_fuse_fwd", x, yf, z, x.numel(), act, arith, DTYPE_OF[x.dtype])
        ctx.save_for_backward(x, yf)
        ctx.mode = (act, arith)
        return z

    @staticmethod
    def backward(ctx, dz):
        x, yf = ctx.saved_tensors
        dz = dz.contiguous()
        dx, dyf = torch.empty_like(x), torch.empty_like(yf)
        with ops.PROFILE.rec("fm_fuse_bwd", 0.0, 5 * x.numel() * x.element_size()):
            call("msml_fm_fuse_bwd", dz, x, yf, dx, dyf, x.numel(), ctx.mode[0], ctx.mode[1],
                 DTYPE_OF[x.dtype])
        return dx, dyf, None, None


ACTS = {"tanh": 0, "sigmoid": 1}
ARITHS = {"add": 0, "sub": 1, "mul": 2, "div": 3}


def fm_fuse(x, yf, act, arith):
    if isinstance(x, SplitT):
        return fm_fuse_x3(x, yf, act, arith)
    return _FmFuse.apply(x, yf, ACTS[act], ARITHS[arith])


class _Add(torch.autograd.Function):
    @staticmethod
    def forward(ctx, a, b):
        out = torch.empty_like(a)
        call("msml_add", a, b, out, a.numel(), DTYPE_OF[a.dtype])
        return out

    @staticmethod
    def backward(ctx, g):
        return g, g


def add(a, b):
    if isinstance(a, SplitT):
        return add_x3(a, b)
    return _Add.apply(a, b)


class _FanOut2(torch.autograd.Function):

    @staticmethod
    def forward(ctx, x):
        return x.view_as(x), x.view_as(x)

    @staticmethod
    def backward(ctx, ga, gb):
        if ga is None or gb is None:
            return ga if gb is None else gb
        ga, gb = ga.contiguous(), gb.contiguous()
        out = torch.empty_like(ga)
        call("msml_add", ga, gb, out, out.numel(), DTYPE_OF[ga.dtype])
        return out


def fanout2(x):
    if (torch.is_grad_enabled() and isinstance(x, torch.Tensor) and x.requires_grad and x.is_cuda
            and x.dtype in DTYPE_OF):
        a, b = _FanOut2.apply(x)
        if "_msml_stats" in x.__dict__:
            a.__dict__["_msml_stats"] = x.__dict__["_msml_stats"]
        return a, b
    return x, x


class _Dap(torch.autograd.Function):

    @staticmethod
    def forward(ctx, x):
        n, h, w, cp = x.shape
        seg = torch.empty(n, 2, h, w, dtype=torch.float32, device=x.device)
        call("msml_dap_fwd", x, seg, None, n, h, w, cp, DTYPE_OF[x.dtype])
        ctx.meta = (x.shape, x.dtype)
        return seg

    @staticmethod
    def backward(ctx, dseg):
        shape, dt = ctx.meta
        dx = torch.empty(shape, dtype=dt, device=dseg.device)
        dseg = dseg.contiguous().float()
        dseg.record_stream(_lib.current_stream())
        call("msml_dap_bwd", dseg, dx, shape[0], shape[1], shape[2], shape[3], DTYPE_OF[dt])
        return dx


def dap(x):
    if isinstance(x, SplitT):
        x = x3_to_f32(x)
    return _Dap.apply(x)


def mask_index(final_seg):
    n, _, h, w = final_seg.shape
    a, b = final_seg[:, 0], final_seg[:, 1]
    return (b > a).to(torch.uint8)


class _ToVec(torch.autograd.Function):

    @staticmethod
    def forward(ctx, x, c):
        ctx.meta = (x.shape, x.dtype)
        return x.reshape(x.shape[0], -1)[:, :c].float()

    @staticmethod
    def backward(ctx, g):
        shape, dt = ctx.meta
        out = torch.zeros(shape, dtype=dt, device=g.device)
        out.reshape(shape[0], -1)[:, :g.shape[1]] = g.to(dt)
        return out, None


def to_vec(x, c):
    return _ToVec.apply(x, c)


class _SegLoss(torch.autograd.Function):

    @staticmethod
    def forward(ctx, logit, msk, alpha, beta, mean_all=False, kl_all=False):
        n, c, h, w = logit.shape
        assert c == 2
        logit = logit.contiguous().float()
        msk = msk.to(device=logit.device, dtype=torch.int64).contiguous()
        loss = torch.empty(1, dtype=torch.float32, device=logit.device)
        dlogit = torch.empty_like(logit)
        ws = torch.empty(20 * n, dtype=torch.float32, device=logit.device)
        call("msml_seg_consensus_loss_r", logit, msk, n, h, w, alpha, beta, int(mean_all), int(kl_all), loss, dlogit, ws,
             ws.numel())
        ctx.save_for_backward(dlogit)
        return loss[0]

    @staticmethod
    def backward(ctx, g):
        (dlogit,) = ctx.saved_tensors
        return dlogit * g, None, None, None, None, None


def seg_consensus_loss(logit, msk, alpha=10.0, beta=5.0, reduce_pixel="idx", reduce_pixel_kl="idx"):
    return _SegLoss.apply(logit, msk, alpha, beta, reduce_pixel == "all", reduce_pixel_kl == "all")


HEAD_KIND = {"arc": 0, "cos": 1}


class _CosMarginHead(torch.autograd.Function):

    @staticmethod
    def forward(ctx, emb, weight, label, kind, s, m, a, k, dtype):
        b, e = emb.shape
        c = weight.shape[0]
        dev = emb.device
        tdt = TORCH_DTYPE[dtype]
        cp = cpad(c)
        kop = (cp + ops.tile_n(cp) - 1) // ops.tile_n(cp) * ops.tile_n(cp)
        xn = torch.empty(b, 1, 1, e, dtype=tdt, device=dev)
        inv_x = torch.empty(b, dtype=torch.float32, device=dev)
        call("msml_rownorm_fwd", emb.detach().contiguous(), b, b, e, xn, e, inv_x, dtype)
        wn = torch.empty(kop, e, dtype=tdt, device=dev)
        inv_w = torch.empty(c, dtype=torch.float32, device=dev)
        call("msml_rownorm_fwd", weight.detach(), c, kop, e, wn, e, inv_w, dtype)
        cosm, _ = ops.conv2d(xn, None, wn, None, cp, 1, 1, 1, 0, 0, False, out_dtype=F32)
        cosm = cosm.reshape(b, cp)
        label = label.to(device=dev, dtype=torch.int64).contiguous()
        cos_t = torch.empty(b, dtype=torch.float32, device=dev)
        call("msml_gather_target", cosm, cp, label, b, cos_t)
        call("msml_margin_fwd", cosm, label, b, c, cp, kind, s, m, a, k)
        ctx.save_for_backward(emb, weight, label, xn, wn, inv_x, inv_w, cos_t)
        ctx.prm = (kind, s, m, a, k, dtype)
        return cosm[:, :c]

    @staticmethod
    def backward(ctx, dlogit):
        emb, weight, label, xn, wn, inv_x, inv_w, cos_t = ctx.saved_tensors
        kind, s, m, a, k, dtype = ctx.prm
        b, e = emb.shape
        c = weight.shape[0]
        dev = emb.device
        tdt = TORCH_DTYPE[dtype]
        cp = cpad(c)
        dlogit = dlogit.contiguous().float()
        dcos = torch.empty(b, 1, 1, cp, dtype=tdt, device=dev)
        call("msml_margin_bwd", dlogit, dlogit.shape[1], label, cos_t, b, c, dcos, cp, kind, s, m,
             a, k, dtype)
        demb = dw = None
        if ctx.needs_input_grad[0]:
            wnt = torch.empty(e, ops.kpad(cp), dtype=tdt, device=dev)
            call("msml_transpose", wn, c, e, e, wnt, ops.kpad(cp), dtype)
            dxn, _ = ops.conv2d(dcos, None, wnt, None, e, 1, 1, 1, 0, 0, False, out_dtype=F32)
            demb = torch.empty_like(emb)
            call("msml_rownorm_bwd", emb.detach().contiguous(), inv_x, dxn.reshape(b, e), e, b, e,
                 demb, 0)
        if ctx.needs_input_grad[1]:
            dwn = torch.empty(c, e, dtype=torch.float32, device=dev)
            ops.conv_wgrad(dcos, xn, dwn, c, e, e, 0, 1, 1, 1, 0, 0)
            dw = torch.empty_like(weight)
            call("msml_rownorm_bwd", weight.detach(), inv_w, dwn, e, c, e, dw, 0)
        return demb, dw, None, None, None, None, None, None, None


def cos_margin_head(emb, weight, label, kind, s, m, a, k, dtype):
    return _CosMarginHead.apply(emb, weight, label, HEAD_KIND[kind], s, m, a, k, dtype)


class _Linear(torch.autograd.Function):

    @staticmethod
    def forward(ctx, emb, weight, bias, dtype):
        b, e = emb.shape
        c = weight.shape[0]
        tdt = TORCH_DTYPE[dtype]
        x = emb.detach().to(tdt).reshape(b, 1, 1, e).contiguous()
        wp = ops.pack_weight(weight.detach().reshape(c, e, 1, 1), False, e, 0, dtype)
        bp = torch.zeros(cpad(c), dtype=torch.float32, device=emb.device)
        bp[:c] = bias.detach()
        y, _ = ops.conv2d(x, None, wp, bp, cpad(c), 1, 1, 1, 0, 0, False, out_dtype=F32)
        ctx.save_for_backward(x, weight)
        ctx.dtype = dtype
        return y.reshape(b, -1)[:, :c]

    @staticmethod
    def backward(ctx, dy):
        x, weight = ctx.saved_tensors
        dtype = ctx.dtype
        tdt = TORCH_DTYPE[dtype]
        b, e = x.shape[0], x.shape[3]
        c = weight.shape[0]
        cp = cpad(c)
        g = torch.zeros(b, 1, 1, cp, dtype=tdt, device=dy.device)
        g.reshape(b, cp)[:, :c] = dy.to(tdt)
        wt = ops.pack_weight(weight.detach().reshape(c, e, 1, 1), True, c, 0, dtype)
        dx, _ = ops.conv2d(g, None, wt, None, e, 1, 1, 1, 0, 0, False, out_dtype=F32)
        dw = torch.empty_like(weight)
        ops.conv_wgrad(g, x, dw, c, e, e, 0, 1, 1, 1, 0, 0)
        db = dy.float().sum(0)
        return dx.reshape(b, e), dw, db, None


def linear(emb, weight, bias, dtype):
    return _Linear.apply(emb, weight, bias, dtype)


class _Normalize(torch.autograd.Function):

    @staticmethod
    def forward(ctx, x):
        b, e = x.shape
        x = x.contiguous().float()
        y = torch.empty_like(x)
        inv = torch.empty(b, dtype=torch.float32, device=x.device)
        call("msml_rownorm_fwd", x, b, b, e, y, e, inv, F32)
        ctx.save_for_backward(x, inv)
        return y

    @staticmethod
    def backward(ctx, dy):
        x, inv = ctx.saved_tensors
        b, e = x.shape
        dx = torch.empty_like(x)
        call("msml_rownorm_bwd", x, inv, dy.contiguous().float(), e, b, e, dx, 0)
        return dx


def normalize(x):
    return _Normalize.apply(x)


class _FlatFc(torch.autograd.Function):

    @staticmethod
    def forward(ctx, x, weight, bias, grad_param):
        n, h, w, c = x.shape
# ... 694 lines not shown
```

msml_amd/ops.py:

```python
import ctypes
import os
import weakref

import torch

from . import _lib
from ._lib import BF16, DTYPE_OF, F32, TORCH_DTYPE, call, try_call


class _Profile:

    def __init__(self):
        self.on = False
        self.recs = []
        self.by_size = bool(os.environ.get("MSML_PROFILE_BY_SIZE"))

    def start(self):
        self.recs = []
        self.on = True

    def rec(self, name, flops=0.0, nbytes=0.0):
        if not self.on:
            return _NO_REC
        if nbytes and not flops and self.by_size:
# ... 52 lines not shown
def cpad(c):
    cp = (c + 31) // 32 * 32
    if 64 < cp < 256 and cp & (cp - 1):
        cp = 128 if cp < 128 else 256
    return cp


def kpad(k):
    return (k + 31) // 32 * 32


def tile_n(coutp):
    return 32 if coutp <= 32 else (64 if coutp <= 64 else 128)


def tile_m(coutp):
    return 256 if coutp <= 64 else 128


def to_nhwc(x, dtype, cp=None):
    n, c, h, w = x.shape
    cp = cp or cpad(c)
    out = torch.empty(n, h, w, cp, dtype=TORCH_DTYPE[dtype], device=x.device)
    call("msml_nchw_to_nhwc", x.contiguous(), out, n, c, h, w, cp, dtype)
    return out


def to_nchw(t, c):
    n, h, w, cp = t.shape
    out = torch.empty(n, c, h, w, dtype=torch.float32, device=t.device)
    call("msml_nhwc_to_nchw", t, out, n, c, h, w, cp, DTYPE_OF[t.dtype])
    return out


def pack_weight(w, transpose, c1, c2, dtype, stored=False):
    a, b, r, s = w.shape
    ko = b if transpose else a
    kop = (cpad(ko) + tile_n(cpad(ko)) - 1) // tile_n(cpad(ko)) * tile_n(cpad(ko))
    c1p, c2p = (c1, c2) if stored else (cpad(c1), cpad(c2) if c2 else 0)
    ktot = kpad(r * s * c1p) + (kpad(r * s * c2p) if c2 else 0)
    wp = torch.empty(kop, ktot, dtype=TORCH_DTYPE[dtype], device=w.device)
    call("msml_pack_weight", w.contiguous(), wp, a, b, r, s, int(transpose), c1, c1p, c2, c2p, kop,
         dtype)
    return wp


def bn_stats_rows(m, c):
    return _lib.value("msml_bn_stats_rows", m, c)


ACC_STATS = os.environ.get("MSML_NO_ACC_STATS") is None
ACC_ROWS = 8


class _AccArena:
    CHUNK = 1 << 20

    def __init__(self):
        self.chunks = {}

    def get(self, c, device, nq=2):
        n = ACC_ROWS * nq * c
        raw = _lib.raw_stream()
        cap = _lib.value("msml_stream_capture_id", raw) if torch.cuda.is_current_stream_capturing() else 0
        if cap < 0:
            raise RuntimeError("msml_stream_capture_id failed: %s" % _lib.load().msml_last_error().decode())
        key = (device.index, raw, cap != 0)
        ent = self.chunks.get(key)
        if ent is None or ent[1] + n > ent[0].numel() or ent[2] != cap:
            ent = [torch.zeros(max(self.CHUNK, n), dtype=torch.float64, device=device), 0, cap]
            self.chunks[key] = ent
        out = ent[0][ent[1]:ent[1] + n].view(ACC_ROWS, nq, c)
        ent[1] += n
        return out


ACC_ARENA = _AccArena()


def acc_applies(c, dtype):
    return ACC_STATS and dtype == BF16 and c % 8 == 0 and 256 % (c // 8) == 0


def stats_acc(c, device, nq=2):
    return ACC_ARENA.get(c, device, nq)


def rows4(t):
    assert t.dtype is torch.float32
    p = t.data_ptr()
    s = t.stride(0) * 4
    return (p, p + s, p + s + s, p + 3 * s)


_UNIT_COEF = {}


def unit_coef(cp, device):
    key = (cp, device)
    u = _UNIT_COEF.get(key)
    if u is None:
        if torch.cuda.is_current_stream_capturing():
            return (torch.ones(cp, dtype=torch.float32, device=device), torch.zeros(cp, dtype=torch.float32, device=device))
        u = _UNIT_COEF[key] = (torch.ones(cp, dtype=torch.float32).to(device), torch.zeros(cp, dtype=torch.float32).to(device))
        torch.cuda.current_stream(device).synchronize()
    return u


def conv_out_size(h, r, stride, pad, transposed, out_pad=0):
    if transposed:
        return (h - 1) * stride - 2 * pad + r + out_pad
    return (h + 2 * pad - r) // stride + 1


def stem_im2col(x, r, s, stride, pad, kp=32, dtype=BF16):
    n, c, h, w = x.shape
    p = conv_out_size(h, r, stride, pad, False)
    q = conv_out_size(w, s, stride, pad, False)
    out = torch.empty(n, p, q, kp, dtype=TORCH_DTYPE[dtype], device=x.device)
    with PROFILE.rec("stem_im2col", 0.0, x.numel() * 4 + out.numel() * out.element_size()):
        call("msml_stem_im2col", x.contiguous(), out, n, c, h, w, p, q, r, s, stride, pad, kp, dtype)
    return out


def conv_label(kind, c0p, c1p, coutp, n, h, w, p, q, r, s, stride, pad_h, pad_w, transposed, in_dtype, out_dtype,
               want_stats):
    kern = _lib.value("msml_conv2d_kernel", c0p, c1p, coutp, n, h, w, p, q, r, s, stride, pad_h, pad_w,
                      int(transposed), in_dtype, out_dtype, int(bool(want_stats))).decode()
    return "conv %s c%d+%d->%d %dx%d k%dx%d s%d n%d [%s]" % (kind, c0p, c1p, coutp, h, w, r, s, stride, n, kern)


def conv2d(x0, x1, wp, bias, coutp, r, s, stride, pad_h, pad_w, transposed, p=None, q=None,
           out_dtype=None, want_stats=False, real=None):
    n, h, w, c0p = x0.shape
    c1p = x1.shape[3] if x1 is not None else 0
    if p is None:
        p = conv_out_size(h, r, stride, pad_h, transposed)
        q = conv_out_size(w, s, stride, pad_w, transposed)
    in_dtype = DTYPE_OF[x0.dtype]
    out_dtype = in_dtype if out_dtype is None else out_dtype
    out = torch.empty(n, p, q, coutp, dtype=TORCH_DTYPE[out_dtype], device=x0.device)
    stats = None
    acc = want_stats and out_dtype == BF16 and acc_applies(coutp, in_dtype)
    if acc:
        stats = stats_acc(coutp, x0.device)
    elif want_stats:
        tiles = (n * p * q + tile_m(coutp) - 1) // tile_m(coutp)
        stats = torch.empty(tiles, 2, coutp, dtype=torch.float32, device=x0.device)
    cin, cout = real if real is not None else (c0p + c1p, coutp)
    pix = n * h * w if transposed else n * p * q
    name = "conv_igemm"
    if PROFILE.on:
        name = conv_label("T" if transposed else "N", c0p, c1p, coutp, n, h, w, p, q, r, s, stride, pad_h, pad_w,
                          transposed, in_dtype, out_dtype, want_stats)
    with PROFILE.rec(name, 2.0 * pix * cin * cout * r * s):
        call("msml_conv2d_acc" if acc else "msml_conv2d", x0, c0p, x1, c1p, wp, wp.shape[0], bias, out, coutp, stats,
             n, h, w, p, q, r, s, stride, pad_h, pad_w, int(transposed), in_dtype, out_dtype)
    return out, stats


FUSE_BN_IN = os.environ.get("MSML_FUSE_BN_IN") is not None
_BNIN_OK = {}


def bnin_applies(n, h, w, cin_p, cout_p, a_real, b_real):
    key = (n, h, w, cin_p, cout_p, a_real, b_real)
    ok = _BNIN_OK.get(key)
    if ok is None:
        ok = bool(FUSE_BN_IN and
                  _lib.value("msml_conv2d_bnin_applies", cin_p, cout_p, n, h, w, h, w, 3, 3, 1, 1, 1, 1) and
                  _lib.value("msml_conv_wgrad_bnin_applies", cout_p, cin_p, a_real, b_real, n, h, w, h, w,
                             3, 3, 1, 1, 1))
        _BNIN_OK[key] = ok
    return ok


BNIN_ACC = os.environ.get("MSML_NO_BNIN_ACC") is None
BNIN_ACC_MIN_C = int(os.environ.get("MSML_BNIN_ACC_MIN_C", "256"))
_BNIN_ACC_OK = {}


def bnin_acc_applies(n, h, w, cin_p, cout_p, r, s, stride, pad):
    key = (n, h, w, cin_p, cout_p, r, s, stride, pad)
    ok = _BNIN_ACC_OK.get(key)
    if ok is None:
        ok = False
        if BNIN_ACC and ACC_STATS and r == 3 and s == 3 and stride == 1 and pad == 1 and acc_applies(cin_p, BF16) and \
                acc_applies(cout_p, BF16):
            kind = _lib.value("msml_conv2d_bnin_acc_applies", cin_p, cout_p, n, h, w, h, w, 3, 3, 1, 1, 1)
            ok = (kind == 1 and cin_p >= BNIN_ACC_MIN_C) or kind == 3
        _BNIN_ACC_OK[key] = ok
    return ok


def conv2d_bnin_acc(x, acc_in, bnp, alpha, wp, coutp, real=None):
    n, h, w, c0p = x.shape
    act = torch.empty_like(x)
    out = torch.empty(n, h, w, coutp, dtype=torch.bfloat16, device=x.device)
    coef = torch.empty(4, c0p, dtype=torch.float32, device=x.device)
    acc_out = stats_acc(coutp, x.device)
    cin, cout = real if real is not None else (c0p, coutp)
    name = "conv_igemm"
    if PROFILE.on:
        name = conv_label("N+bn", c0p, 0, coutp, n, h, w, h, w, 3, 3, 1, 1, 1, 0, BF16, BF16, True)
    with PROFILE.rec(name, 2.0 * n * h * w * cin * cout * 9):
        call("msml_conv2d_bnin_acc", x, c0p, acc_in, float(n * h * w), bnp[0], bnp[1], bnp[2], bnp[3], bnp[4], bnp[5], coef,
             alpha, act, wp, wp.shape[0], out, coutp, acc_out, n, h, w, h, w, 3, 3, 1, 1, 1)
    return act, coef, out, acc_out


def conv2d_bnin(x, coef, alpha, wp, coutp, real=None):
    n, h, w, c0p = x.shape
    out = torch.empty(n, h, w, coutp, dtype=torch.bfloat16, device=x.device)
    tiles = (n * h * w + tile_m(coutp) - 1) // tile_m(coutp)
    stats = torch.empty(tiles, 2, coutp, dtype=torch.float32, device=x.device)
    cin, cout = real if real is not None else (c0p, coutp)
    name = "conv_igemm"
    if PROFILE.on:
        name = conv_label("N+bnin", c0p, 0, coutp, n, h, w, h, w, 3, 3, 1, 1, 1, 0, BF16, BF16, True)
    with PROFILE.rec(name, 2.0 * n * h * w * cin * cout * 9):
        coef = rows4(coef)
        call("msml_conv2d_bnin", x, c0p, coef[0], coef[1], alpha, wp, wp.shape[0], out, coutp, stats, n, h, w,
             h, w, 3, 3, 1, 1, 1)
    return out, stats


def conv_wgrad_bnin(u, v, coef, alpha, dw, a, breal, btot, boff, accumulate=False, stream=None):
    n, p, q, up = u.shape
    _, h, w, vp = v.shape
    key = (up, vp, n, p, q, 3, 3)
    need = _WGRAD_WS_NEED.get(key)
    if need is None:
        need = _WGRAD_WS_NEED[key] = _lib.value("msml_conv_wgrad_workspace", *key)
    raw = stream.cuda_stream if stream is not None else _lib.raw_stream()
    ws = workspace(need, u.device, "wgrad", stream)
    coef = rows4(coef)
    if PROFILE.on and stream is None:
        name = "wgrad+bnin u%d v%d %dx%d k3x3 s1 n%d" % (up, vp, p, q, n)
        with PROFILE.rec(name, 2.0 * n * p * q * a * breal * 9):
            call("msml_conv_wgrad_bnin", u, up, v, vp, coef[0], coef[1], alpha, dw, a, breal, btot, boff, n, h, w,
                 p, q, 3, 3, 1, 1, 1, int(accumulate), ws, ws.numel(), raw)
        return dw
    call("msml_conv_wgrad_bnin", u, up, v, vp, coef[0], coef[1], alpha, dw, a, breal, btot, boff, n, h, w,
         p, q, 3, 3, 1, 1, 1, int(accumulate), ws, ws.numel(), raw)
    return dw


def conv_dgrad_bnbwd(dy, wp, coutp, r, s, stride, pad_h, pad_w, p, q, bn_x, coef, alpha, real=None):
    n, h, w, c0p = dy.shape
    if dy.dtype != torch.bfloat16:
        return None
    out = torch.empty(n, p, q, coutp, dtype=torch.bfloat16, device=dy.device)
    cin, cout = real if real is not None else (c0p, coutp)
    coef = rows4(coef)
    name = "conv_igemm"
    if PROFILE.on:
        name = conv_label("T+bnb", c0p, 0, coutp, n, h, w, p, q, r, s, stride, pad_h, pad_w, 1, BF16, BF16, False)
    if acc_applies(coutp, BF16):
        acc = stats_acc(coutp, dy.device, 3)
        with PROFILE.rec(name, 2.0 * n * h * w * cin * cout * r * s):
            rc = try_call("msml_conv2d_bnbwd_acc", dy, c0p, wp, wp.shape[0], out, coutp, n, h, w, p, q, r, s, stride,
                          pad_h, pad_w, 1, bn_x, coef[0], coef[1], alpha, coef[2], coef[3], acc)
        return (out, acc) if rc == 0 else None
    cap = _lib.value("msml_conv2d_bnbwd_rows", coutp, n, p, q)
    partial = torch.empty(cap, 3, coutp, dtype=torch.float32, device=dy.device)
    used = ctypes.c_int(0)
    with PROFILE.rec(name, 2.0 * n * h * w * cin * cout * r * s):
        rc = try_call("msml_conv2d_bnbwd", dy, c0p, wp, wp.shape[0], out, coutp, n, h, w, p, q, r, s, stride,
                      pad_h, pad_w, 1, bn_x, coef[0], coef[1], alpha, coef[2], coef[3], partial, cap,
                      ctypes.byref(used))
    if rc != 0:
        return None
    return out, partial[:used.value]


_WS = {}


def workspace(nbytes, device, tag="main", stream=None):
    key = (device, tag, stream.cuda_stream if stream is not None else _lib.raw_stream())
    buf = _WS.get(key)
    if buf is None or buf.numel() < nbytes:
        if stream is not None:
            with torch.cuda.stream(stream):
                buf = torch.empty(max(nbytes, 1 << 20), dtype=torch.uint8, device=device)
        else:
            buf = torch.empty(max(nbytes, 1 << 20), dtype=torch.uint8, device=device)
        _WS[key] = buf
    return buf


WGRAD_STREAM = None
OSB_STREAM = None


BLOCK_FUNCTION = os.environ.get("MSML_NO_BLOCK_FUNCTION") is None
BOTTLE_FUNCTION = os.environ.get("MSML_NO_BOTTLE_FUNCTION") is None
FUSE_BN_BWD = os.environ.get("MSML_NO_FUSE_BN_BWD") is None
BLOCK_C_ENTRY = os.environ.get("MSML_BLOCK_C_ENTRY") is not None
EMIT_STEM_STATS = os.environ.get("MSML_NO_EMIT_STEM_STATS") is None
FM_TEE = os.environ.get("MSML_NO_FM_TEE") is None
GCM_TEE = os.environ.get("MSML_NO_GCM_TEE") is None
SPARSE_DOWNSAMPLE_GRAD = os.environ.get("MSML_NO_SPARSE_DOWNSAMPLE_GRAD") is None

COUNTERS = {"bn3_partial_hits": 0}

DEFER_BN_COUNTERS = False
_PENDING_COUNTERS = []


def bn_counter(bn):
    if bn.num_batches_tracked is None:
        return
    if DEFER_BN_COUNTERS:
        _PENDING_COUNTERS.append(bn.num_batches_tracked)
    else:
        bn.num_batches_tracked += 1


def flush_bn_counters():
    if _PENDING_COUNTERS:
        torch._foreach_add_(_PENDING_COUNTERS, 1)
        _PENDING_COUNTERS.clear()


def grad_ready(*params):
    for p in params:
        if p is not None:
            cb = getattr(p, "_msml_ready", None)
            if cb is not None:
                cb(p)


def wgrad_stream_join():
    wgrad_flush()
    if OSB_STREAM is None and WGRAD_STREAM is None:
        return
    cur = torch.cuda.current_stream()
    if OSB_STREAM is not None:
        cur.wait_stream(OSB_STREAM)
        if WGRAD_STREAM is not None:
            WGRAD_STREAM.wait_stream(OSB_STREAM)
    if WGRAD_STREAM is not None:
        cur.wait_stream(WGRAD_STREAM)


_WGRAD_WS_NEED = {}


def conv_wgrad(u, v, dw, a, breal, btot, boff, r, s, stride, pad_h, pad_w, accumulate=False, stream=None):
    n, p, q, up = u.shape
    _, h, w, vp = v.shape
    key = (up, vp, n, p, q, r, s)
    need = _WGRAD_WS_NEED.get(key)
    if need is None:
        need = _WGRAD_WS_NEED[key] = _lib.value("msml_conv_wgrad_workspace", *key)
    raw = stream.cuda_stream if stream is not None else _lib.raw_stream()
    ws = workspace(need, u.device, "wgrad", stream)
    name = "conv_wgrad"
    if PROFILE.on and stream is None:
        name = "wgrad u%d v%d %dx%d k%dx%d s%d n%d" % (up, vp, p, q, r, s, stride, n)
        with PROFILE.rec(name, 2.0 * n * p * q * a * breal * r * s):
            call("msml_conv_wgrad", u, up, v, vp, dw, a, breal, btot, boff, n, h, w, p, q, r, s, stride,
                 pad_h, pad_w, int(accumulate), ws, ws.numel(), DTYPE_OF[u.dtype], raw)
        return dw
    call("msml_conv_wgrad", u, up, v, vp, dw, a, breal, btot, boff, n, h, w, p, q, r, s, stride,
         pad_h, pad_w, int(accumulate), ws, ws.numel(), DTYPE_OF[u.dtype], raw)
    return dw


WGRAD_GROUP = int(os.environ.get("MSML_WGRAD_GROUP", "4"))
WGRAD_GROUP_MAX_HW = int(os.environ.get("MSML_WGRAD_GROUP_MAX_HW", "1000"))
_GROUP_MAX = {}


class _WgradQueue:
    def __init__(self):
        self.key = None
        self.items = []
        self.stream = None


_WQ = _WgradQueue()


def wgrad_drop():
    _WQ.items, _WQ.key, _WQ.stream = [], None, None


def wgrad_flush():
    q = _WQ
    if not q.items:
        return
    items, key, stream = q.items, q.key, q.stream
    q.items, q.key, q.stream = [], None, None
    up, vp, n, h, w, a, breal, btot, boff, raw = key
    if stream is None and raw != _lib.raw_stream():
        stream = torch.cuda.ExternalStream(raw)
    g = len(items)
    need = _WGRAD_WS_NEED.get((up, vp, n, h, w, 3, 3))
    if need is None:
        need = _WGRAD_WS_NEED[(up, vp, n, h, w, 3, 3)] = _lib.value("msml_conv_wgrad_workspace", up, vp, n, h, w, 3, 3)
    ws = workspace(need, items[0][0].device, "wgrad", stream)
    arr = ctypes.c_void_p * g
    us, vs, dws = arr(*[it[0].data_ptr() for it in items]), arr(*[it[1].data_ptr() for it in items]), \
        arr(*[it[2].data_ptr() for it in items])
    if g == 1:
        u, v, dw = items[0][:3]
        conv_wgrad(u, v, dw, a, breal, btot, boff, 3, 3, 1, 1, 1, accumulate=True, stream=stream)
    elif PROFILE.on and stream is None:
        with PROFILE.rec("wgrad u%d v%d %dx%d k3x3 s1 n%d x%d" % (up, vp, h, w, n, g), 2.0 * n * h * w * a * breal * 9 * g):
            call("msml_conv_wgrad_group", us, vs, dws, g, up, vp, a, breal, btot, boff, n, h, w, h, w, 3, 3, 1, 1, 1, 1,
                 ws, ws.numel(), BF16, raw)
    else:
        call("msml_conv_wgrad_group", us, vs, dws, g, up, vp, a, breal, btot, boff, n, h, w, h, w, 3, 3, 1, 1, 1, 1,
             ws, ws.numel(), BF16, raw)
    for it in items:
        if it[3] is not None:
            grad_ready(it[3])


def conv_wgrad_queued(u, v, dw, a, breal, btot, boff, stream, param):
    n, p, q, up = u.shape
    vp = v.shape[3]
    skey = (up, vp, n, p, q, a, breal, btot, boff)
    gmax = _GROUP_MAX.get(skey)
    if gmax is None:
        gmax = _GROUP_MAX[skey] = min(WGRAD_GROUP, _lib.value("msml_conv_wgrad_group_max", up, vp, a, breal, n, p, q, p, q,
                                                              3, 3, 1, 1, 1)) if WGRAD_GROUP > 1 else 1
    if gmax <= 1 or u.dtype != torch.bfloat16 or p > WGRAD_GROUP_MAX_HW:
        conv_wgrad(u, v, dw, a, breal, btot, boff, 3, 3, 1, 1, 1, accumulate=True, stream=stream)
        grad_ready(param)
        return
    wq = _WQ
    key = skey + (stream.cuda_stream if stream is not None else _lib.raw_stream(),)
    if wq.items and wq.key != key:
        wgrad_flush()
    if not wq.items:
        torch.autograd.Variable._execution_engine.queue_callback(wgrad_flush)
    wq.key, wq.stream = key, stream
    wq.items.append((u, v, dw, param))
    if len(wq.items) >= gmax:
        wgrad_flush()


def gemm_splitk(a, wp, coutp):
    m, k = a.shape
    need = _lib.value("msml_gemm_splitk_workspace", m, coutp, k)
    ws = workspace(need, a.device)
    out = torch.empty(m, coutp, dtype=torch.float32, device=a.device)
    with PROFILE.rec("gemm_splitk", 2.0 * m * k * coutp):
        call("msml_gemm_splitk", a, m, k, wp, wp.shape[0], out, coutp, ws, ws.numel(), DTYPE_OF[a.dtype])
    return out


class PackCache:

    def __init__(self):
        self.entries = {}
        self.stale_log = None
        self.table = None
        self.order = []
        self.last_epoch = -1

    def clear(self):
        self.__init__()

    @staticmethod
    def _stamp(w):
        return (w._version, WEIGHT_EPOCH, w.data_ptr())

    def _evict(self, key):
        def cb(_ref):
            self.entries.pop(key, None)
            self.table = None
        return cb

    def get(self, w, transpose, a_off, a_n, b_off, b_n, c1, c2, dtype, owner=None):
        own = w if owner is None else owner
        afull, bfull, r, s = w.shape
        key = (id(own), (afull, bfull, r, s), transpose, a_off, a_n, b_off, b_n, c1, c2, dtype)
        e = self.entries.get(key)
        if e is not None and e["ref"]() is not own:
            e = None
        if e is None:
            ko = b_n if transpose else a_n
            kop = (cpad(ko) + tile_n(cpad(ko)) - 1) // tile_n(cpad(ko)) * tile_n(cpad(ko))
            c1p, c2p = cpad(c1), cpad(c2) if c2 else 0
            ktot = kpad(r * s * c1p) + (kpad(r * s * c2p) if c2 else 0)
            dst = torch.zeros(kop, ktot, dtype=TORCH_DTYPE[dtype], device=w.device)
            desc = [0, dst.data_ptr(), afull, bfull, a_off, a_n, b_off, b_n, r, s, int(transpose), c1,
                    c1p, c2, c2p, kop]
            e = {"desc": desc, "dst": dst, "stamp": None, "ref": weakref.ref(own, self._evict(key))}
            self.entries[key] = e
            self.table = None
        st = self._stamp(own)
        if e["stamp"] != st:
            if self.stale_log is not None:
                self.stale_log.append((tuple(w.shape), transpose, e["stamp"], st))
            e["desc"][0] = own.data_ptr()
            t = torch.tensor([e["desc"]], dtype=torch.int64, device=w.device)
            call("msml_pack_weights_batched", t, 1, dtype)
            e["stamp"] = st
        return e["dst"]

    def refresh_if_stale(self):
        if self.entries and self.last_epoch != WEIGHT_EPOCH:
            self.refresh()

    def refresh(self):
        self.last_epoch = WEIGHT_EPOCH
        live = [(e, e["ref"]()) for e in list(self.entries.values())]
        live = [(e, w) for e, w in live if w is not None]
        if not live:
            return
        ents = [e for e, _ in live]
        ptrs = tuple(w.data_ptr() for _, w in live)
        dtype = DTYPE_OF[ents[0]["dst"].dtype]
        if self.table is None or self.order != ptrs:
            for e, w in live:
                e["desc"][0] = w.data_ptr()
            dev = ents[0]["dst"].device
            self.table = torch.tensor([e["desc"] for e in ents], dtype=torch.int64, device=dev)
            tiles = [_lib.value("msml_pack_tiles", e["desc"][5], e["desc"][7], e["desc"][8], e["desc"][9]) for e in ents]
            pre = [0]
            for n_ in tiles[:-1]:
                pre.append(pre[-1] + n_)
            self.total_tiles = pre[-1] + tiles[-1]
            tmap = [i for i, n_ in enumerate(tiles) for _ in range(n_)]
            self.prefix = torch.tensor(pre + [-1] + tmap, dtype=torch.int32, device=dev)
            self.order = ptrs
        if any(DTYPE_OF[e["dst"].dtype] != dtype for e in ents):
            for e in ents:
                e["stamp"] = None
            return
        if max(e["desc"][8] * e["desc"][9] for e in ents) <= 49:
            call("msml_pack_weights_tiled", self.table, self.prefix, len(ents), self.total_tiles, dtype)
        else:
            call("msml_pack_weights_batched", self.table, len(ents), dtype)
        for e, w in live:
            e["stamp"] = self._stamp(w)


WEIGHT_EPOCH = 0


def padded_bias(bias, cp):
    b = bias.detach()
    if b.numel() == cp and b.dtype == torch.float32 and b.is_contiguous():
        return b
    stamp = (bias._version, WEIGHT_EPOCH, bias.data_ptr(), cp)
    hit = getattr(bias, "_msml_bias_pad", None)
    if hit is None or hit[0] != stamp:
        buf = hit[1] if hit is not None and hit[1].numel() == cp and hit[1].device == b.device else \
            torch.zeros(cp, dtype=torch.float32, device=b.device)
        buf[:b.numel()].copy_(b)
        bias._msml_bias_pad = hit = (stamp, buf)
    return hit[1]
PACKS = PackCache()
```

Before: 8717 images/sec.

## Fuse downsample and bn3 backward into dual kernels and pass stem BN sums forward

```diff
diff --git a/include/msml_hip.h b/include/msml_hip.h
--- a/include/msml_hip.h
+++ b/include/msml_hip.h
@@ -118,6 +118,24 @@
                         const void* residual_first, const void* add, void* dx, void* dres, float* dgamma,
                         float* dbeta, float* dalpha, int accumulate, long M, int C, double* acc, int dtype,
                         void* stream);
+int msml_bn_fin_bwd_apply_next2(const void* dy, const void* x, const float* scale, const float* shift,
+                                const float* alpha, const float* save_mean, const float* save_invstd,
+                                const double* acc, const void* add, int add_h, int add_w, void* dx,
+                                float* dgamma, float* dbeta, float* dalpha, int accumulate, long M, int C,
+                                const void* next_x, const float* next_scale, const float* next_shift,
+                                const float* next_alpha, const float* next_mean, const float* next_invstd,
+                                double* next_acc, const void* next2_x, const float* next2_mean,
+                                const float* next2_invstd, double* next2_acc, int dtype, void* stream);
+int msml_bn_fin_bwd_apply_dual(const void* dy, const void* xa, const float* scale_a, const float* mean_a,
+                               const float* invstd_a, const double* acc_a, const void* xb, const float* scale_b,
+                               const float* mean_b, const float* invstd_b, const double* acc_b, void* dxa,
+                               void* dxb, float* dgamma_a, float* dbeta_a, float* dgamma_b, float* dbeta_b,
+                               int accumulate, long M, int C, int dtype, void* stream);
+int msml_bn_act_bwd_acc_dual(const void* dy, const void* xa, const float* scale_a, const float* mean_a,
+                             const float* invstd_a, double* acc_a, const void* xb, const float* scale_b,
+                             const float* mean_b, const float* invstd_b, double* acc_b, void* dxa, void* dxb,
+                             float* dgamma_a, float* dbeta_a, float* dgamma_b, float* dbeta_b, int accumulate,
+                             long M, int C, int dtype, void* stream);
 int msml_bn_act_bwd(const void* dy, const void* x, const float* scale, const float* shift,
                     const float* alpha, const float* save_mean, const float* save_invstd,
                     const void* residual_first, void* dx, void* dres, float* dgamma, float* dbeta,
diff --git a/msml_amd/blocks.py b/msml_amd/blocks.py
--- a/msml_amd/blocks.py
+++ b/msml_amd/blocks.py
@@ -217,8 +217,13 @@
     m = x.numel() // c
     dx = torch.empty_like(x)
     coef = ops.rows4(coef)
+    nal = nx2 = None
     if nxt:
-        nxt = (nxt[0], ops.rows4(nxt[1])) + tuple(nxt[2:])
+        nal = nxt[2] if len(nxt) > 2 else None
+        nx2 = (nxt[3], ops.rows4(nxt[4])) if len(nxt) > 4 and nxt[3] is not None and ops.DUAL_DS_BWD else None
+        nxt = (nxt[0], ops.rows4(nxt[1]))
+        if nal is not None and not (ops.STEM_BWD_SUMS and partial is not None and partial.dtype == torch.float64):
+            nxt = ()
     s2 = (add, x.shape[1], x.shape[2]) if add_s2 else (add,)
     sfx = "_s2" if add_s2 else ""
     if partial is None and ops.acc_applies(c, BF16):
@@ -236,8 +241,18 @@
             call("msml_add", dx, add, dx, dx.numel(), BF16)
     elif partial.dtype == torch.float64:
         ah, aw = (x.shape[1], x.shape[2]) if add_s2 else (0, 0)
-        if nxt is not None and 256 % (c // 8) == 0:
+        if nxt and 256 % (c // 8) == 0:
             nacc = ops.stats_acc(c, x.device, 3)
+            if nal is not None or nx2 is not None:
+                nacc2 = ops.stats_acc(c, x.device, 3) if nx2 is not None and nal is None else None
+                streams = (5 if add is not None else 4) + (1 if nacc2 is not None else 0)
+                with ops.PROFILE.rec("bn_act_bwd_apply", 0.0, x.numel() * x.element_size() * streams):
+                    call("msml_bn_fin_bwd_apply_next2", dy, x, coef[0], coef[1], alpha, coef[2], coef[3], partial, add, ah,
+                         aw, dx, pgr.tg[0], pgr.tg[1], pgr.tg[2], int(pgr.inplace), m, c, nxt[0], nxt[1][0], nxt[1][1], nal,
+                         nxt[1][2], nxt[1][3], nacc, *((nx2[0], nx2[1][2], nx2[1][3], nacc2) if nacc2 is not None
+                                                       else (None, None, None, None)), BF16)
+                pgr.done()
+                return dx, (nacc if nacc2 is None else (nacc, nacc2))
             with ops.PROFILE.rec("bn_act_bwd_apply", 0.0, x.numel() * x.element_size() * (5 if add is not None else 4)):
                 call("msml_bn_fin_bwd_apply", dy, x, coef[0], coef[1], alpha, coef[2], coef[3], partial, None, add, ah, aw,
                      dx, None, pgr.tg[0], pgr.tg[1], pgr.tg[2], int(pgr.inplace), m, c, nxt[0], nxt[1][2], nxt[1][3],
@@ -249,7 +264,7 @@
                  dx, None, pgr.tg[0], pgr.tg[1], pgr.tg[2], int(pgr.inplace), m, c, None, None, None, None, BF16)
     else:
         cw = torch.empty(98 * c, dtype=torch.float32, device=x.device)
-        if nxt is not None and 256 % (c // 8) == 0:
+        if nxt and 256 % (c // 8) == 0:
             npart = torch.empty(_lib.value("msml_bn_act_bwd_apply_rows", m, c), 3, c, dtype=torch.float32,
                                 device=x.device)
             with ops.PROFILE.rec("bn_act_bwd_apply", 0.0, x.numel() * x.element_size() * (5 if add is not None else 4)):
@@ -265,6 +280,26 @@
     if nxt is not None:
         return dx, None
     return dx
+
+
+def _bn_bwd_dual(dy, xa, ka, ga, acc_a, xb, kb, gb, acc_b):
+    c = xa.shape[-1]
+    m = xa.numel() // c
+    dxa, dxb = torch.empty_like(xa), torch.empty_like(xb)
+    ka, kb = ops.rows4(ka), ops.rows4(kb)
+    nbytes = xa.numel() * xa.element_size()
+    if acc_a is None:
+        acc_a, acc_b = ops.stats_acc(c, xa.device, 3), ops.stats_acc(c, xa.device, 3)
+        with ops.PROFILE.rec("bn_act_bwd", 0.0, nbytes * 8):
+            call("msml_bn_act_bwd_acc_dual", dy, xa, ka[0], ka[2], ka[3], acc_a, xb, kb[0], kb[2], kb[3], acc_b, dxa, dxb,
+                 ga.tg[0], ga.tg[1], gb.tg[0], gb.tg[1], int(ga.inplace), m, c, BF16)
+    else:
+        with ops.PROFILE.rec("bn_act_bwd_apply", 0.0, nbytes * 5):
+            call("msml_bn_fin_bwd_apply_dual", dy, xa, ka[0], ka[2], ka[3], acc_a, xb, kb[0], kb[2], kb[3], acc_b, dxa, dxb,
+                 ga.tg[0], ga.tg[1], gb.tg[0], gb.tg[1], int(ga.inplace), m, c, BF16)
+    ga.done()
+    gb.done()
+    return dxa, dxb
 
 
 def _block_pack(blk):
@@ -378,7 +413,7 @@
 
 class _IBlock(torch.autograd.Function):
     @staticmethod
-    def forward(ctx, x, bp, xstats, pc2, pk3, *params):
+    def forward(ctx, x, bp, xstats, pc2, pk3, pal, pd, pkd, *params):
         if _iblock_fwd_applies(x, bp):
             fast = _iblock_fwd_fast(x, bp, xstats)
             if fast is not None:
@@ -387,8 +422,8 @@
                     ostats = out.new_empty(0)
                 ctx.bp = bp
                 ctx.set_materialize_grads(False)
-                bp["_last_bn3"] = (c2, k3) if bp["emit_stats"] else None
-                ctx.save_for_backward(x, o1, c1, o2, c2, d, k1, k2, k3, kd, pc2, pk3)
+                bp["_last_bn3"] = (c2, k3, None, d, kd) if bp["emit_stats"] else None
+                ctx.save_for_backward(x, o1, c1, o2, c2, d, k1, k2, k3, kd, pc2, pk3, pal, pd, pkd)
                 ctx.mark_non_differentiable(ostats)
                 return out, ostats
         ds = bp["ds"]
@@ -406,14 +441,14 @@
             ostats = out.new_empty(0)
         ctx.bp = bp
         ctx.set_materialize_grads(False)
-        bp["_last_bn3"] = (c2, k3) if bp["emit_stats"] else None
-        ctx.save_for_backward(x, o1, c1, o2, c2, d, k1, k2, k3, kd, pc2, pk3)
+        bp["_last_bn3"] = (c2, k3, None, d, kd) if bp["emit_stats"] else None
+        ctx.save_for_backward(x, o1, c1, o2, c2, d, k1, k2, k3, kd, pc2, pk3, pal, pd, pkd)
         ctx.mark_non_differentiable(ostats)
         return out, ostats
 
     @staticmethod
     def backward(ctx, dout, _dstats):
-        x, o1, c1, o2, c2, d, k1, k2, k3, kd, pc2, pk3 = ctx.saved_tensors
+        x, o1, c1, o2, c2, d, k1, k2, k3, kd, pc2, pk3, pal, pd, pkd = ctx.saved_tensors
         bp = ctx.bp
         ds = bp["ds"]
         dev = x.device
@@ -422,19 +457,30 @@
         bn1, bn2, bn3, alpha = bp["bn1"], bp["bn2"], bp["bn3"], bp["alpha"]
         g3 = _ParamGrads((bn3[0], bn3[1], None), c2.shape[-1], dev)
         part3 = dout.__dict__.pop("_msml_bn3_partial", None) if bp["emit_stats"] else None
+        partd = None
+        if isinstance(part3, tuple):
+            part3, partd = part3
+            ops.COUNTERS["ds_partial_hits"] += 1
         if part3 is not None:
             ops.COUNTERS["bn3_partial_hits"] += 1
-        dc2 = _bn_bwd(dout, c2, k3, None, g3, part3)
+        dd = gd = None
+        if ds is not None:
+            gd = _ParamGrads((ds[1][0], ds[1][1], None), d.shape[-1], dev)
+        if (ds is not None and ops.DUAL_DS_BWD and ops.acc_applies(c2.shape[-1], BF16) and g3.inplace == gd.inplace
+                and (part3 is None) == (partd is None)):
+            dc2, dd = _bn_bwd_dual(dout, c2, k3, g3, part3, d, kd, gd, partd)
+        else:
+            dc2 = _bn_bwd(dout, c2, k3, None, g3, part3)
         dw2 = _wgrad(dc2, o2, bp["c2"]) if o2 is not None else _wgrad(dc2, c1, bp["c2"], (k2, alpha))
         do2, part2 = _dgrad(dc2, bp["c2"], c1.shape[1], c1.shape[2], c1, k2, alpha)
         g2 = _ParamGrads((bn2[0], bn2[1], alpha), c1.shape[-1], dev)
         dc1 = _bn_bwd(do2, c1, k2, alpha, g2, part2)
         dw1 = _wgrad(dc1, o1, bp["c1"]) if o1 is not None else _wgrad(dc1, x, bp["c1"], (k1, None))
         do1, part1 = _dgrad(dc1, bp["c1"], h, w, x, k1, None)
-        dwd, gd = None, None
+        dwd = None
         if ds is not None:
-            gd = _ParamGrads((ds[1][0], ds[1][1], None), d.shape[-1], dev)
-            dd = _bn_bwd(dout, d, kd, None, gd)
+            if dd is None:
+                dd = _bn_bwd(dout, d, kd, None, gd)
             dwd = _wgrad(dd, x, ds[0])
             (_, (_, _, dr, dsz), dstride, dph, dpw) = ds[0]
             join_s2 = (ops.SPARSE_DOWNSAMPLE_GRAD and part1 is not None and dr == 1 and dsz == 1 and dstride == 2
@@ -447,7 +493,7 @@
             join, join_s2 = (None if FAULT == "skip_join" else dout), False
         g1 = _ParamGrads((bn1[0], bn1[1], None), x.shape[-1], dev)
         if pc2 is not None and part1 is not None and ops.FUSE_BN_BWD:
-            dx, pprev = _bn_bwd(do1, x, k1, None, g1, part1, add=join, nxt=(pc2, pk3), add_s2=join_s2)
+            dx, pprev = _bn_bwd(do1, x, k1, None, g1, part1, add=join, nxt=(pc2, pk3, pal, pd, pkd), add_s2=join_s2)
             if pprev is not None:
                 dx._msml_bn3_partial = pprev
         else:
@@ -458,7 +504,7 @@
         grads += [g1.out(0), g1.out(1), g2.out(0), g2.out(1), g2.out(2), g3.out(0), g3.out(1)]
         if ds is not None:
             grads += [gd.out(0), gd.out(1)]
-        return (dx, None, None, None, None) + tuple(grads)
+        return (dx, None, None, None, None, None, None, None) + tuple(grads)
 
 
 def iblock(blk, x):
@@ -475,7 +521,7 @@
         blk.__dict__["_msml_pack"] = bp
     xd = x.__dict__ if hasattr(x, "__dict__") else {}
     xstats, prev = xd.get("_msml_stats"), xd.get("_msml_bn3")
-    out, ostats = _IBlock.apply(x, bp, xstats, prev[0] if prev else None, prev[1] if prev else None, *bp["params"])
+    out, ostats = _IBlock.apply(x, bp, xstats, *(prev if prev else (None,) * 5), *bp["params"])
     last = bp.pop("_last_bn3", None)
     if ostats.numel():
         out._msml_stats = ostats
diff --git a/msml_amd/csrc/bn.hip b/msml_amd/csrc/bn.hip
--- a/msml_amd/csrc/bn.hip
+++ b/msml_amd/csrc/bn.hip
@@ -5,7 +5,8 @@
 #define RED_ROWS_MAX 1024
 
 template <int NQ, bool PIPE, typename L, typename F>
-__device__ __forceinline__ void slab_reduce(long M, int C, float* __restrict__ partial, L ld, F f, int acc_mode = 0) {
+__device__ __forceinline__ void slab_reduce(long M, int C, float* __restrict__ partial, L ld, F f, int acc_mode = 0,
+                                            double* __restrict__ partial2 = nullptr) {
   extern __shared__ __attribute__((aligned(16))) char smem_raw[];
   float* red = reinterpret_cast<float*>(smem_raw);
   const int C8 = C / 8;
@@ -44,7 +45,12 @@
   for (int i = t; i < NQ * C; i += blockDim.x) {
     float s = 0.f;
     for (int y = 0; y < PY; y++) s += red[y * NQ * C + i];
-    if (acc_mode)
+    if (acc_mode == 2) {
+      const int a = i / C, c = i - a * C;
+      const long row = (long)(blockIdx.x & (MSML_ACC_ROWS - 1)) * 3 * C;
+      if (a != 2) unsafeAtomicAdd(reinterpret_cast<double*>(partial) + row + (long)a * C + c, (double)s);
+      if (a != 1) unsafeAtomicAdd(partial2 + row + (long)(a >> 1) * C + c, (double)s);
+    } else if (acc_mode)
       unsafeAtomicAdd(reinterpret_cast<double*>(partial) + (long)(blockIdx.x & (MSML_ACC_ROWS - 1)) * NQ * C + i, (double)s);
     else
       partial[(long)blockIdx.x * NQ * C + i] = s;
@@ -636,8 +642,14 @@
   return MSML_OK;
 }
 
-template <typename T, bool NEXT, bool ADD_S2>
-__global__ void __launch_bounds__(256) k_bn_fin_bwd_apply(const T* __restrict__ dy, const T* __restrict__ x,
+struct BnNextExtra {
+  const float *scale, *shift, *alpha;
+  const void* x2;
+  const float *mean2, *invstd2;
+  double* acc2;
+};
+template <typename T, int NEXT, bool ADD_S2>
+__global__ void __launch_bounds__(256) __attribute__((amdgpu_waves_per_eu(3))) k_bn_fin_bwd_apply(const T* __restrict__ dy, const T* __restrict__ x,
                                                           const float* __restrict__ scale, const float* __restrict__ shift,
                                                           const float* __restrict__ alpha, const float* __restrict__ mean,
                                                           const float* __restrict__ invstd, const double* __restrict__ acc,
@@ -648,7 +660,7 @@
                                                           T* __restrict__ dres, long n8, int C8,
                                                           const T* __restrict__ nx, const float* __restrict__ nmean,
                                                           const float* __restrict__ ninvstd, double* __restrict__ nacc,
-                                                          int aH, int aW) {
+                                                          int aH, int aW, BnNextExtra e) {
   extern __shared__ float ck[];
   const int C = C8 * 8, t = threadIdx.x;
   MSML_LDS_REGION(ck, 2 * C * 4);
@@ -682,13 +694,19 @@
   const float rcpW = ADD_S2 ? 1.0f / (float)aW : 0.f, rcpH = ADD_S2 ? 1.0f / (float)aH : 0.f;
   const int aPw = (aW + 1) >> 1, aPh = (aH + 1) >> 1;
   const Coef8 nmu = ldc8(NEXT ? nmean : nullptr, c0, 0.f), nis = ldc8(NEXT ? ninvstd : nullptr, c0, 1.f);
-  float nq0[8], nq1[8];
-#pragma unroll
-  for (int j = 0; j < 8; j++) nq0[j] = nq1[j] = 0.f;
+  const Coef8 nsc = ldc8(NEXT == 2 ? e.scale : nullptr, c0, 1.f), nsh = ldc8(NEXT == 2 ? e.shift : nullptr, c0, 0.f);
+  const Coef8 nal = ldc8(NEXT == 2 ? e.alpha : nullptr, c0, 1.f);
+  const Coef8 nmu2 = ldc8(NEXT == 3 ? e.mean2 : nullptr, c0, 0.f), nis2 = ldc8(NEXT == 3 ? e.invstd2 : nullptr, c0, 1.f);
+  const T* __restrict__ nx2 = reinterpret_cast<const T*>(e.x2);
+  float nq0[8], nq1[8], nq2[8];
+#pragma unroll
+  for (int j = 0; j < 8; j++) nq0[j] = nq1[j] = nq2[j] = 0.f;
   for (long i = tid; i < n8; i += (long)gridDim.x * blockDim.x) {
     Vec8 g = load8<T>(dy + i * 8);
     Vec8 v = load8<T>(x + i * 8);
-    Vec8 rr, ad;
+    Vec8 rr, ad, xn, xm;
+    if (NEXT >= 2) xn = load8<T>(nx + i * 8);
+    if (NEXT == 3) xm = load8<T>(nx2 + i * 8);
     if (res) rr = load8<T>(res + i * 8);
     bool has_add = add != nullptr;
     if (ADD_S2) {
@@ -718,45 +736,66 @@
     store8<T>(dx + i * 8, v);
     if (dres) store8<T>(dres + i * 8, g);
     if (NEXT) {
-      const Vec8 o = round8<T>(v), xn = load8<T>(nx + i * 8);
+      const Vec8 o = round8<T>(v);
+      if (NEXT == 1) xn = load8<T>(nx + i * 8);
 #pragma unroll
       for (int j = 0; j < 8; j++) {
-        const float gn = o.v[j];
+        float gn = o.v[j];
+        if (NEXT == 2) {
+          const float z = xn.v[j] * nsc.v[j] + nsh.v[j];
+          if (z <= 0.f) {
+            nq2[j] += gn * z;
+            gn *= nal.v[j];
+          }
+        }
         nq0[j] += gn;
         nq1[j] += gn * ((xn.v[j] - nmu.v[j]) * nis.v[j]);
+        if (NEXT == 3) nq2[j] += gn * ((xm.v[j] - nmu2.v[j]) * nis2.v[j]);
       }
     }
   }
   if (NEXT) {
-    __shared__ float red[2][256][9];
+    constexpr int NQN = NEXT == 1 ? 2 : 3;
+    __shared__ float red[NQN][256][9];
 #pragma unroll
     for (int j = 0; j < 8; j++) {
       red[0][t][j] = nq0[j];
       red[1][t][j] = nq1[j];
+      if (NQN == 3) red[NQN - 1][t][j] = nq2[j];
     }
     __syncthreads();
-    for (int i = t; i < 2 * C; i += 256) {
+    for (int i = t; i < NQN * C; i += 256) {
       const int q = i / C, c = i % C, cx = c >> 3, j = c & 7;
       float sum = 0.f;
       for (int k = cx; k < 256; k += C8) sum += red[q][k][j];
-      bnb_emit(reinterpret_cast<float*>(nacc), 1, blockIdx.x, q, C, c, sum);
-    }
-  }
-}
-
-extern "C" int msml_bn_fin_bwd_apply(const void* dy, const void* x, const float* scale, const float* shift,
-                                     const float* alpha, const float* save_mean, const float* save_invstd,
-                                     const double* acc, const void* residual_first, const void* add, int add_h,
-                                     int add_w, void* dx, void* dres, float* dgamma, float* dbeta, float* dalpha,
-                                     int accumulate, long M, int C, const void* next_x, const float* next_mean,
-                                     const float* next_invstd, double* next_acc, int dtype, void* stream) {
+      if (NEXT == 3) {
+        if (q != 2) bnb_emit(reinterpret_cast<float*>(nacc), 1, blockIdx.x, q, C, c, sum);
+        if (q != 1) bnb_emit(reinterpret_cast<float*>(e.acc2), 1, blockIdx.x, q >> 1, C, c, sum);
+      } else {
+        bnb_emit(reinterpret_cast<float*>(nacc), 1, blockIdx.x, q, C, c, sum);
+      }
+    }
+  }
+}
+
+static int bn_fin_bwd_apply_impl(const char* who, const void* dy, const void* x, const float* scale, const float* shift,
+                                 const float* alpha, const float* save_mean, const float* save_invstd,
+                                 const double* acc, const void* residual_first, const void* add, int add_h,
+                                 int add_w, void* dx, void* dres, float* dgamma, float* dbeta, float* dalpha,
+                                 int accumulate, long M, int C, const void* next_x, const float* next_mean,
+                                 const float* next_invstd, double* next_acc, const BnNextExtra& e, int dtype, void* stream) {
   MSML_CHECK(dy && x && dx && scale && shift && save_mean && save_invstd && acc && M > 0 && C > 0 && C % 8 == 0,
-             MSML_ERR_SHAPE, "bn_fin_bwd_apply: bad args M=%ld C=%d", M, C);
-  MSML_CHECK(256 % (C / 8) == 0, MSML_ERR_UNSUPPORTED, "bn_fin_bwd_apply: C/8 = %d must divide 256", C / 8);
+             MSML_ERR_SHAPE, "%s: bad args M=%ld C=%d", who, M, C);
+  MSML_CHECK(256 % (C / 8) == 0, MSML_ERR_UNSUPPORTED, "%s: C/8 = %d must divide 256", who, C / 8);
   const bool s2 = add_h > 0;
   MSML_CHECK(!s2 || (add && add_w > 0 && M % ((long)add_h * add_w) == 0 && M < (1L << 24)), MSML_ERR_SHAPE,
-             "bn_fin_bwd_apply: stride-2 add needs M = N*H*W < 2^24 (M=%ld H=%d W=%d)", M, add_h, add_w);
-  MSML_CHECK(!next_acc || (next_x && next_mean && next_invstd), MSML_ERR_SHAPE, "bn_fin_bwd_apply: next_* incomplete");
+             "%s: stride-2 add needs M = N*H*W < 2^24 (M=%ld H=%d W=%d)", who, M, add_h, add_w);
+  MSML_CHECK(!next_acc || (next_x && next_mean && next_invstd), MSML_ERR_SHAPE, "%s: next_* incomplete", who);
+  const int mode = !next_acc ? 0 : e.alpha ? 2 : e.acc2 ? 3 : 1;
+  MSML_CHECK(next_acc || !(e.alpha || e.acc2), MSML_ERR_SHAPE, "%s: a PReLU or second target needs next_acc", who);
+  MSML_CHECK(mode != 2 || (e.scale && e.shift && !e.acc2), MSML_ERR_SHAPE,
+             "%s: a PReLU target needs its scale and shift, and excludes a second target", who);
+  MSML_CHECK(mode != 3 || (e.x2 && e.mean2 && e.invstd2), MSML_ERR_SHAPE, "%s: next2_* incomplete", who);
   hipStream_t st = (hipStream_t)stream;
   const long n8 = M * (C / 8);
   const size_t lds = (size_t)2 * C * sizeof(float);
@@ -764,13 +803,186 @@
   (k_bn_fin_bwd_apply<DT, NEXT_, S2_>)<<<ew_grid_c(n8, C / 8), 256, lds, st>>>(                                     \
       (const DT*)dy, (const DT*)x, scale, shift, alpha, save_mean, save_invstd, acc, (double)M, dgamma, dbeta, dalpha, \
       accumulate, (const DT*)residual_first, (const DT*)add, (DT*)dx, (DT*)dres, n8, C / 8, (const DT*)next_x,      \
-      next_mean, next_invstd, next_acc, add_h, add_w);
-  MSML_DISPATCH_DTYPE(dtype, "bn_fin_bwd_apply",
-                      if (next_acc) { if (s2) { BN_FIN_LAUNCH(true, true) } else { BN_FIN_LAUNCH(true, false) } }
-                      else { if (s2) { BN_FIN_LAUNCH(false, true) } else { BN_FIN_LAUNCH(false, false) } })
+      next_mean, next_invstd, next_acc, add_h, add_w, e);
+#define BN_FIN_LAUNCH_S2(NEXT_) if (s2) { BN_FIN_LAUNCH(NEXT_, true) } else { BN_FIN_LAUNCH(NEXT_, false) }
+  MSML_DISPATCH_DTYPE(dtype, who,
+                      if (mode == 0) { BN_FIN_LAUNCH_S2(0) }
+                      else if (mode == 1) { BN_FIN_LAUNCH_S2(1) }
+                      else if (mode == 2) { BN_FIN_LAUNCH_S2(2) }
+                      else { BN_FIN_LAUNCH_S2(3) })
+#undef BN_FIN_LAUNCH_S2
 #undef BN_FIN_LAUNCH
-  MSML_LAUNCH_OK("bn_fin_bwd_apply");
+  MSML_LAUNCH_OK(who);
   return MSML_OK;
+}
+
+extern "C" int msml_bn_fin_bwd_apply(const void* dy, const void* x, const float* scale, const float* shift,
+                                     const float* alpha, const float* save_mean, const float* save_invstd,
+                                     const double* acc, const void* residual_first, const void* add, int add_h,
+                                     int add_w, void* dx, void* dres, float* dgamma, float* dbeta, float* dalpha,
+                                     int accumulate, long M, int C, const void* next_x, const float* next_mean,
+                                     const float* next_invstd, double* next_acc, int dtype, void* stream) {
+  return bn_fin_bwd_apply_impl("bn_fin_bwd_apply", dy, x, scale, shift, alpha, save_mean, save_invstd, acc, residual_first,
+                               add, add_h, add_w, dx, dres, dgamma, dbeta, dalpha, accumulate, M, C, next_x, next_mean,
+                               next_invstd, next_acc, BnNextExtra{}, dtype, stream);
+}
+
+extern "C" int msml_bn_fin_bwd_apply_next2(const void* dy, const void* x, const float* scale, const float* shift,
+                                           const float* alpha, const float* save_mean, const float* save_invstd,
+                                           const double* acc, const void* add, int add_h, int add_w, void* dx,
+                                           float* dgamma, float* dbeta, float* dalpha, int accumulate, long M, int C,
+                                           const void* next_x, const float* next_scale, const float* next_shift,
+                                           const float* next_alpha, const float* next_mean, const float* next_invstd,
+                                           double* next_acc, const void* next2_x, const float* next2_mean,
+                                           const float* next2_invstd, double* next2_acc, int dtype, void* stream) {
+  MSML_CHECK(next_acc, MSML_ERR_SHAPE, "bn_fin_bwd_apply_next2: next_acc is null");
+  BnNextExtra e{next_scale, next_shift, next_alpha, next2_x, next2_mean, next2_invstd, next2_acc};
+  return bn_fin_bwd_apply_impl("bn_fin_bwd_apply_next2", dy, x, scale, shift, alpha, save_mean, save_invstd, acc, nullptr,
+                               add, add_h, add_w, dx, nullptr, dgamma, dbeta, dalpha, accumulate, M, C, next_x, next_mean,
+                               next_invstd, next_acc, e, dtype, stream);
+}
+
+template <typename T, bool PIPE>
+__global__ void __launch_bounds__(256) k_bn_bwd_reduce2(const T* __restrict__ dy, const T* __restrict__ xa,
+                                                        const T* __restrict__ xb, const float* __restrict__ mean_a,
+                                                        const float* __restrict__ invstd_a,
+                                                        const float* __restrict__ mean_b,
+                                                        const float* __restrict__ invstd_b, long M, int C,
+                                                        double* __restrict__ acc_a, double* __restrict__ acc_b) {
+  const int c0h = (threadIdx.x % (C / 8)) * 8;
+  const Coef8 mua = ldc8(mean_a, c0h, 0.f), isa = ldc8(invstd_a, c0h, 1.f);
+  const Coef8 mub = ldc8(mean_b, c0h, 0.f), isb = ldc8(invstd_b, c0h, 1.f);
+  struct Px {
+    Vec8 g, a, b;
+  };
+  slab_reduce<3, PIPE>(M, C, reinterpret_cast<float*>(acc_a), [&](long pix, int c8) {
+    Px d;
+    d.g = load8<T>(dy + pix * C + c8 * 8);
+    d.a = load8<T>(xa + pix * C + c8 * 8);
+    d.b = load8<T>(xb + pix * C + c8 * 8);
+    return d;
+  }, [&](const Px& d, float(&q)[3][8]) {
+#pragma unroll
+    for (int j = 0; j < 8; j++) {
+      const float gg = d.g.v[j];
+      q[0][j] += gg;
+      q[1][j] += gg * ((d.a.v[j] - mua.v[j]) * isa.v[j]);
+      q[2][j] += gg * ((d.b.v[j] - mub.v[j]) * isb.v[j]);
+    }
+  }, 2, acc_b);
+}
+
+template <typename T>
+__global__ void __launch_bounds__(256) k_bn_fin_bwd_apply2(const T* __restrict__ dy, const T* __restrict__ xa,
+                                                           const T* __restrict__ xb, const float* __restrict__ scale_a,
+                                                           const float* __restrict__ mean_a, const float* __restrict__ invstd_a,
+                                                           const float* __restrict__ scale_b, const float* __restrict__ mean_b,
+                                                           const float* __restrict__ invstd_b, const double* __restrict__ acc_a,
+                                                           const double* __restrict__ acc_b, double count,
+                                                           float* __restrict__ dgamma_a, float* __restrict__ dbeta_a,
+                                                           float* __restrict__ dgamma_b, float* __restrict__ dbeta_b,
+                                                           int accumulate, T* __restrict__ dxa, T* __restrict__ dxb, long n8,
+                                                           int C8) {
+  extern __shared__ float ck[];
+  const int C = C8 * 8, t = threadIdx.x;
+  MSML_LDS_REGION(ck, 4 * C * 4);
+  for (int c = t; c < C; c += 256) {
+    double a0 = 0.0, a1 = 0.0, b0 = 0.0, b1 = 0.0;
+#pragma unroll
+    for (int r = 0; r < MSML_ACC_ROWS; r++) {
+      a0 += acc_a[(r * 3 + 0) * C + c];
+      a1 += acc_a[(r * 3 + 1) * C + c];
+      b0 += acc_b[(r * 3 + 0) * C + c];
+      b1 += acc_b[(r * 3 + 1) * C + c];
+    }
+    ck[c] = (float)(a0 / count);
+    ck[C + c] = (float)(a1 / count);
+    ck[2 * C + c] = (float)(b0 / count);
+    ck[3 * C + c] = (float)(b1 / count);
+    if (blockIdx.x == 0) {
+      if (dbeta_a) dbeta_a[c] = (accumulate ? dbeta_a[c] : 0.f) + (float)a0;
+      if (dgamma_a) dgamma_a[c] = (accumulate ? dgamma_a[c] : 0.f) + (float)a1;
+      if (dbeta_b) dbeta_b[c] = (accumulate ? dbeta_b[c] : 0.f) + (float)b0;
+      if (dgamma_b) dgamma_b[c] = (accumulate ? dgamma_b[c] : 0.f) + (float)b1;
+    }
+  }
+  __syncthreads();
+  const long tid = blockIdx.x * (long)blockDim.x + t;
+  const int c0 = (int)(tid % C8) * 8;
+  const Coef8 sca = ldc8(scale_a, c0, 1.f), mua = ldc8(mean_a, c0, 0.f), isa = ldc8(invstd_a, c0, 1.f);
+  const Coef8 scb = ldc8(scale_b, c0, 1.f), mub = ldc8(mean_b, c0, 0.f), isb = ldc8(invstd_b, c0, 1.f);
+  Coef8 k1a, k2a, k1b, k2b;
+#pragma unroll
+  for (int j = 0; j < 8; j++) {
+    k1a.v[j] = ck[c0 + j];
+    k2a.v[j] = ck[C + c0 + j];
+    k1b.v[j] = ck[2 * C + c0 + j];
+    k2b.v[j] = ck[3 * C + c0 + j];
+  }
+  for (long i = tid; i < n8; i += (long)gridDim.x * blockDim.x) {
+    const Vec8 g = load8<T>(dy + i * 8);
+    Vec8 va = load8<T>(xa + i * 8), vb = load8<T>(xb + i * 8);
+#pragma unroll
+    for (int j = 0; j < 8; j++) {
+      const float gg = g.v[j];
+      const float xha = (va.v[j] - mua.v[j]) * isa.v[j], xhb = (vb.v[j] - mub.v[j]) * isb.v[j];
+      va.v[j] = sca.v[j] * (gg - k1a.v[j] - xha * k2a.v[j]);
+      vb.v[j] = scb.v[j] * (gg - k1b.v[j] - xhb * k2b.v[j]);
+    }
+    store8<T>(dxa + i * 8, va);
+    store8<T>(dxb + i * 8, vb);
+  }
+}
+
+static int bn_bwd_dual_impl(const char* who, bool reduce, const void* dy, const void* xa, const float* scale_a,
+                            const float* mean_a, const float* invstd_a, double* acc_a, const void* xb,
+                            const float* scale_b, const float* mean_b, const float* invstd_b, double* acc_b, void* dxa,
+                            void* dxb, float* dgamma_a, float* dbeta_a, float* dgamma_b, float* dbeta_b, int accumulate,
+                            long M, int C, int dtype, void* stream) {
+  MSML_CHECK(dy && xa && xb && dxa && dxb && scale_a && mean_a && invstd_a && scale_b && mean_b && invstd_b && acc_a &&
+                 acc_b && M > 0 && C > 0 && C % 8 == 0 && C <= 2048,
+             MSML_ERR_SHAPE, "%s: bad args M=%ld C=%d", who, M, C);
+  MSML_CHECK(256 % (C / 8) == 0, MSML_ERR_UNSUPPORTED, "%s: C/8 = %d must divide 256", who, C / 8);
+  hipStream_t st = (hipStream_t)stream;
+  if (reduce) {
+    const int rows = red_rows(M, C);
+    MSML_DISPATCH_DTYPE(dtype, who,
+                        if (rows <= RED_PIPE_MAX_ROWS)
+                          (k_bn_bwd_reduce2<DT, true>)<<<rows, 256, red_lds(3, C), st>>>(
+                              (const DT*)dy, (const DT*)xa, (const DT*)xb, mean_a, invstd_a, mean_b, invstd_b, M, C, acc_a, acc_b);
+                        else
+                          (k_bn_bwd_reduce2<DT, false>)<<<rows, 256, red_lds(3, C), st>>>(
+                              (const DT*)dy, (const DT*)xa, (const DT*)xb, mean_a, invstd_a, mean_b, invstd_b, M, C, acc_a, acc_b);)
+    MSML_LAUNCH_OK("bn_bwd_reduce2");
+  }
+  const long n8 = M * (C / 8);
+  MSML_DISPATCH_DTYPE(dtype, who,
+                      (k_bn_fin_bwd_apply2<DT>)<<<ew_grid_c(n8, C / 8), 256, (size_t)4 * C * sizeof(float), st>>>(
+                          (const DT*)dy, (const DT*)xa, (const DT*)xb, scale_a, mean_a, invstd_a, scale_b, mean_b, invstd_b,
+                          acc_a, acc_b, (double)M, dgamma_a, dbeta_a, dgamma_b, dbeta_b, accumulate, (DT*)dxa, (DT*)dxb, n8,
+                          C / 8);)
+  MSML_LAUNCH_OK(who);
+  return MSML_OK;
+}
+
+extern "C" int msml_bn_fin_bwd_apply_dual(const void* dy, const void* xa, const float* scale_a, const float* mean_a,
+                                          const float* invstd_a, const double* acc_a, const void* xb,
+                                          const float* scale_b, const float* mean_b, const float* invstd_b,
+                                          const double* acc_b, void* dxa, void* dxb, float* dgamma_a, float* dbeta_a,
+                                          float* dgamma_b, float* dbeta_b, int accumulate, long M, int C, int dtype,
+                                          void* stream) {
+  return bn_bwd_dual_impl("bn_fin_bwd_apply_dual", false, dy, xa, scale_a, mean_a, invstd_a, const_cast<double*>(acc_a), xb,
+                          scale_b, mean_b, invstd_b, const_cast<double*>(acc_b), dxa, dxb, dgamma_a, dbeta_a, dgamma_b,
+                          dbeta_b, accumulate, M, C, dtype, stream);
+}
+
+extern "C" int msml_bn_act_bwd_acc_dual(const void* dy, const void* xa, const float* scale_a, const float* mean_a,
+                                        const float* invstd_a, double* acc_a, const void* xb, const float* scale_b,
+                                        const float* mean_b, const float* invstd_b, double* acc_b, void* dxa, void* dxb,
+                                        float* dgamma_a, float* dbeta_a, float* dgamma_b, float* dbeta_b, int accumulate,
+                                        long M, int C, int dtype, void* stream) {
+  return bn_bwd_dual_impl("bn_act_bwd_acc_dual", true, dy, xa, scale_a, mean_a, invstd_a, acc_a, xb, scale_b, mean_b,
+                          invstd_b, acc_b, dxa, dxb, dgamma_a, dbeta_a, dgamma_b, dbeta_b, accumulate, M, C, dtype, stream);
 }
 
 extern "C" int msml_bn_act_bwd_acc(const void* dy, const void* x, const float* scale, const float* shift,
diff --git a/msml_amd/functional.py b/msml_amd/functional.py
--- a/msml_amd/functional.py
+++ b/msml_amd/functional.py
@@ -221,13 +221,14 @@
                 call("msml_bn_fin_act_fwd", stats, float(m), gamma, beta, rmean, rvar, momentum, eps, coef[0], coef[1],
                      coef[2], coef[3], x, alpha, residual, int(res_first), y, m, c, yacc, dtype)
             ctx.training = training
+            ctx.emit = bool(emit)
             ctx.has = (gamma is not None, beta is not None, alpha is not None, residual is not None)
             ctx.res_first = bool(res_first) and residual is not None and alpha is not None
             ctx.params = (gamma, beta, alpha)
             ctx.save_for_backward(x, coef, alpha, residual if ctx.res_first else None)
             if emit:
-                ctx.mark_non_differentiable(yacc)
-                return y, yacc
+                ctx.mark_non_differentiable(yacc, coef)
+                return y, yacc, coef
             return y
         if training:
             if stats is None:
@@ -244,6 +245,7 @@
         with ops.PROFILE.rec("bn_act_fwd", 0.0, x.numel() * x.element_size() * (3 if residual is not None else 2)):
             call("msml_bn_act_fwd", x, coef[0], coef[1], alpha, residual, int(res_first), y, m, c, dtype)
         ctx.training = training
+        ctx.emit = False
         ctx.has = (gamma is not None, beta is not None, alpha is not None, residual is not None)
         ctx.res_first = bool(res_first) and residual is not None and alpha is not None
         ctx.params = (gamma, beta, alpha)
@@ -258,6 +260,10 @@
         c = x.shape[-1]
         m = x.numel() // c
         dtype = DTYPE_OF[x.dtype]
+        part = dy.__dict__.pop("_msml_bn3_partial", None) if ctx.emit else None
+        if not (torch.is_tensor(part) and part.dtype == torch.float64 and part.numel() == ops.ACC_ROWS * 3 * c
+                and not ctx.has[3] and ops.acc_applies(c, dtype)):
+            part = None
         dy = dy.contiguous()
         dx = torch.empty_like(x)
         pg = torch.empty(3, c, dtype=torch.float32, device=x.device)
@@ -274,6 +280,20 @@
             tg = [prm.grad if w else None for w, prm in zip(want, (gamma, beta, alpha_p))]
         else:
             tg = [pg[0], pg[1], pg[2] if alpha is not None else None]
+        if part is not None:
+            ops.COUNTERS["stem_partial_hits"] += 1
+            with ops.PROFILE.rec("bn_act_bwd_apply", 0.0, x.numel() * x.element_size() * 3):
+                call("msml_bn_fin_bwd_apply", dy, x, coef[0], coef[1], alpha, coef[2], coef[3], part, None, None, 0, 0, dx,
+                     None, tg[0], tg[1], tg[2], int(inplace), m, c, None, None, None, None, dtype)
+            if inplace:
+                ops.grad_ready(*[prm for w, prm in zip(want, (gamma, beta, alpha_p)) if w])
+            return (dx, None,
+                    pg[0] if want[0] and not inplace else None,
+                    pg[1] if want[1] and not inplace else None,
+                    pg[2] if want[2] and not inplace else None,
+                    None, None, None, None, None, None, None, None)
+        if ctx.emit and ops.STEM_BWD_SUMS:
+            ops.COUNTERS["stem_partial_misses"] += 1
         with ops.PROFILE.rec("bn_act_bwd", 0.0, x.numel() * x.element_size() * (5 + (3 if ctx.res_first else 0))):
             if ops.acc_applies(c, dtype):
                 call("msml_bn_act_bwd_acc", dy, x, coef[0], coef[1], alpha, coef[2], coef[3], res, None, dx, dres,
@@ -307,8 +327,10 @@
                        residual, bn.running_mean, bn.running_var, training,
                        0.1 if bn.momentum is None else bn.momentum, bn.eps, res_first, emit)
     if emit:
-        y, yacc = out
+        y, yacc, coef = out
         y._msml_stats = yacc
+        if ops.STEM_BWD_SUMS and prelu is not None and residual is None and ops.FUSE_BN_BWD:
+            y._msml_bn3 = (x.detach(), coef, prelu.weight.detach(), None, None)
         return y
     return out
 
diff --git a/msml_amd/ops.py b/msml_amd/ops.py
--- a/msml_amd/ops.py
+++ b/msml_amd/ops.py
@@ -378,8 +378,11 @@
 FM_TEE = os.environ.get("MSML_NO_FM_TEE") is None
 GCM_TEE = os.environ.get("MSML_NO_GCM_TEE") is None
 SPARSE_DOWNSAMPLE_GRAD = os.environ.get("MSML_NO_SPARSE_DOWNSAMPLE_GRAD") is None
-
-COUNTERS = {"bn3_partial_hits": 0}
+STEM_BWD_SUMS = os.environ.get("MSML_NO_STEM_BWD_SUMS") is None
+DUAL_DS_BWD = os.environ.get("MSML_NO_DUAL_DS_BWD") is None
+
+COUNTERS = {"bn3_partial_hits": 0, "stem_partial_hits": 0, "stem_partial_misses": 0,
+            "ds_partial_hits": 0}
 
 DEFER_BN_COUNTERS = False
 _PENDING_COUNTERS = []
```

Result: no change. 8692 images/sec, median of 2 (-0.3%).
